# JubSteven/POEM-v2

Hardware: AMD Instinct MI355X
Metric: samples/sec (multi-view frames) POEM-medium 8-view (higher is better)
Workload: dtype f32

## Files before the change

### poem-v2_amd/csrc/decoder.cpp

```cpp
#include "engine.h"

int build_anchor_tables(poem_handle_t h, Plan& p, hipStream_t s, bool at_create) {
  const poem_config_t& c = h->cfg;
  const int C = c.embed, Q = c.nquery;
  const bool ov = !at_create && h->overlap && h->bps_stream && h->knn_stream;
  hipStream_t sk = ov ? h->knn_stream : s;
  if (ov) {
    HIPCHK(hipEventRecord(h->ev_fork0, s));
    HIPCHK(hipStreamWaitEvent(sk, h->ev_fork0, 0));
  }
  const int bb0 = h->block_base(0);
  HIPCHK(poem_launch_canon_xyz(h->tmpl, p.canon_xyz, Q * 3, c.radius, sk));
  for (int k = 0; k < 2; ++k) {
    const int vb = bb0 + (k == 0 ? B_VS : B_VC);
    HIPCHK(poem_launch_vector_attention_tables(p.canon_xyz, h->anchor, h->anchor_idx, h->R(vb + 4), h->R(vb + 5),
                                               h->P(vb + 6), h->R(vb + 7), h->fused[0].w[5 + k], p.tab_g[k], p.tab_p[k],
                                               Q, C, sk));
  }
  if (ov) HIPCHK(hipEventRecord(h->ev_tab, sk));
  h->tables_pending = ov;
  return POEM_OK;
}

namespace {

struct DecoderRun {
  poem_handle_t h;
  Plan& p;
  const poem_config_t& c;
  const float *pt_xyz, *pt_feats;
  float *pose_aa, *betas;
  const int B, C, S, Q, BS, BQ;
  const int SP, BSP;
  const float* pt_xyz_rows;
  const bool ov;
  hipStream_t s, sb, sk;
  const bool tables;
  const bool chain;
  const float* feats;
  const float* hidden;
  int ldh = 0, hidden_mod = 0, q_batch = 0;
  const float* q0 = nullptr;
  const int *idx_s = nullptr, *idx_c = nullptr;
  const float* anchor = nullptr;
  int shared = 0;
  bool knn_issued[9] = {};
  bool wmerge = false;
  int wmask = 0;
  bool side_rest_pending = false;
  bool bps_waited[9] = {}, knn_waited[9] = {};
  bool anchor_from_y3 = false;

  DecoderRun(poem_handle_t h_, Plan& p_, const float* feats_in, const float* pt_xyz_, const float* pt_feats_, int B_, float* pose,
             float* bet, hipStream_t s_, bool template_queries)
      : h(h_), p(p_), c(h_->cfg), pt_xyz(pt_xyz_), pt_feats(pt_feats_), pose_aa(pose), betas(bet), B(B_), C(c.embed), S(c.nsample),
        Q(c.nquery), BS(B_ * c.nsample), BQ(B_ * c.nquery), SP(padded_samples(c)), BSP(B_ * padded_samples(c)), pt_xyz_rows(pt_xyz_), ov(h_->overlap && h_->bps_stream && h_->knn_stream), s(s_),
        sb(ov ? h_->bps_stream : s_), sk(ov ? h_->knn_stream : s_),
        tables(template_queries && h_->anchor_tables && h_->precision == POEM_PRECISION_FP32),
        chain(h_->chains && h_->precision == POEM_PRECISION_FP32 && poem_chain_supported(c.embed) != 0), feats(feats_in),
        hidden(nullptr) {}

  int gemm(const float* X, int ldx, int wi, int bi, const float* res, int ldr, float* Y, int ldy, int M, int N, int K, int act) {
    HIPCHK(poem_launch_gemm(X, ldx, h->P(wi), bi >= 0 ? h->R(bi) : nullptr, res, ldr, Y, ldy, M, N, K, act, s));
    return POEM_OK;
  }
  bool prof_begin() {
    const bool on = h->prof_on && (size_t)(2 * h->prof_used + 1) < h->prof_ev.size();
    if (on && hipEventRecord(h->prof_ev[2 * h->prof_used], s) != hipSuccess) return false;
    return on;
  }
  int prof_end(bool on, int kind) {
    if (on) { HIPCHK(hipEventRecord(h->prof_ev[2 * h->prof_used + 1], s)); h->prof_kind[h->prof_used++] = (char)kind; }
    return POEM_OK;
  }
  ChainArgs chain_args(int kind) const {
    ChainArgs a{};
    a.kind = kind; a.M = BQ; a.tile_p = h->chain_tile; a.eps = c.ln_eps;
    a.native_delta = h->native16 ? (long long)(h->native16 - h->packed_base) : 0;
    return a;
  }

  int fork() {
    if (!ov) return POEM_OK;
    HIPCHK(hipEventRecord(h->ev_fork, s));
    HIPCHK(hipStreamWaitEvent(sb, h->ev_fork, 0));
    HIPCHK(hipStreamWaitEvent(sk, h->ev_fork, 0));
    return POEM_OK;
  }
  int join() {
    if (!ov) return POEM_OK;
    HIPCHK(hipEventRecord(h->ev_join_bps, sb));
    HIPCHK(hipEventRecord(h->ev_join_knn, sk));
    HIPCHK(hipStreamWaitEvent(s, h->ev_join_bps, 0));
    HIPCHK(hipStreamWaitEvent(s, h->ev_join_knn, 0));
    return POEM_OK;
  }

  int basis_point_side(int i) {
    const auto& f = h->fused[i];
    const size_t seg = (size_t)BSP * C;
    float* outs[6] = {p.y1[i], p.y1[i] + seg, p.y1[i] + 2 * seg, p.y1[i] + 3 * seg, p.y1[i] + 4 * seg, p.y1[i] + 5 * seg};
    const int modes[6] = {1, 2, 1, 2, 0, 0};
    h->kv_presplit[i] = poem_gemm_split_applies(f.w[0], BSP, C, C) != 0;
    const bool anchored = tables && i == 0;
    if (!anchored && h->f1_split && C % 128 == 0) {
      HIPCHK(poem_launch_gemm_segs(pt_feats, C, f.w[0], f.b[0], BSP, C, POEM_ACT_NONE, C, 4, outs, modes, sb));
      HIPCHK(poem_launch_gemm_segs(pt_feats, C, (const float*)f.w[0] + (size_t)4 * C * C, f.b[0] + 4 * C, BSP, C, POEM_ACT_NONE, C, 2, outs + 4,
                                   modes + 4, sb));
    } else {
      HIPCHK(poem_launch_gemm_segs(pt_feats, C, f.w[0], f.b[0], BSP, C, POEM_ACT_NONE, C, anchored ? 4 : 6, outs, modes, sb));
    }
    if (ov) HIPCHK(hipEventRecord(h->ev_bps[i], sb));
    if (anchored && !side_rest_pending) return basis_point_anchor_rows(f);
    return POEM_OK;
  }
  int basis_point_anchor_rows(const poem_handle_s::Fused& f) {
    {
      HIPCHK(poem_launch_gather_anchor_rows(pt_feats, C, h->anchor_idx, SP, p.anch_x[1], B, C, p.ident, sb));
      HIPCHK(poem_launch_gemm(p.anch_x[1], C, (const float*)f.w[0] + (size_t)4 * C * C, f.b[0] + 4 * C, nullptr, 0,
                              p.anch_kv[1], 2 * C, B * 32, 2 * C, C, POEM_ACT_NONE, sb));
      if (ov) HIPCHK(hipEventRecord(h->ev_xyz[0], sb));
    }
    return POEM_OK;
  }

  bool merge_in_attention() const { return h->xattn_merge >= 0 ? h->xattn_merge != 0 : B <= 2; }

  int defer_at() const {
    return (ov && chain) ? h->bps_defer : 0;
  }
  int deferred_basis_point_side(int i, int at) {
    if (defer_at() != at || i + 1 >= c.nblocks) return POEM_OK;
    HIPCHK(hipEventRecord(h->ev_def[i], s));
    HIPCHK(hipStreamWaitEvent(sb, h->ev_def[i], 0));
    return basis_point_side(i + 1);
  }

  int neighbour_searches(int i, bool recorded = false) {
    if (knn_issued[i]) return POEM_OK;
    if (ov) {
      if (!recorded) HIPCHK(hipEventRecord(h->ev_xyz[i], s));
      HIPCHK(hipStreamWaitEvent(sk, h->ev_xyz[i], 0));
    }
    if (p.idx_ld == 32) {
      HIPCHK(poem_launch_knn(p.xyz[i], pt_xyz, p.idx_cross[i], B, Q, S, h->knn_fma, sk));
      HIPCHK(poem_launch_knn(p.xyz[i], p.xyz[i], p.idx_self[i], B, Q, Q, h->knn_fma, sk));
    } else {
      HIPCHK(poem_launch_knn_k(p.xyz[i], pt_xyz, p.idx_cross[i], B, Q, S, c.knn, p.idx_ld, h->knn_fma, sk));
      HIPCHK(poem_launch_knn_k(p.xyz[i], p.xyz[i], p.idx_self[i], B, Q, Q, h->knn_query ? h->knn_query : c.knn, p.idx_ld, h->knn_fma, sk));
    }
    if (ov) HIPCHK(hipEventRecord(h->ev_knn[i], sk));
    knn_issued[i] = true;
    return POEM_OK;
  }

  int query_projection(int i) {
    hidden = p.qeqp;
    ldh = 2 * C; hidden_mod = 0; q_batch = Q;
    q0 = p.qeqp + C;
    if (tables && i == 0) {
      const float* qe0 = p.qeqp0;
      if (h->tables_cached && h->c_qeqp0 && h->precision == POEM_PRECISION_FP32)
        qe0 = h->c_qeqp0;
      else
        HIPCHK(poem_launch_gemm_split(h->R(T_QEMB), C, h->fused[i].w[1], h->fused[i].b[1], nullptr, 0, p.qeqp0, 2 * C, Q, 2 * C, C,
                                      POEM_ACT_NONE, 2 * C, POEM_ACT_NONE, s));
      if (chain) {
        hidden = qe0; hidden_mod = Q; q0 = qe0 + C; q_batch = 0;
      } else {
        HIPCHK(poem_launch_broadcast(qe0, p.qeqp, (long)Q * 2 * C, B, s));
      }
    } else if (!(chain && i > 0)) {
      HIPCHK(poem_launch_gemm_split(feats, C, h->fused[i].w[1], h->fused[i].b[1], nullptr, 0, p.qeqp, 2 * C, BQ, 2 * C, C,
                                    POEM_ACT_NONE, 2 * C, POEM_ACT_NONE, s));
    }
    return POEM_OK;
  }

  int anchor_rows_f3(int i) {
    HIPCHK(poem_launch_gather_anchor_rows(hidden, C, h->anchor_idx, Q, p.anch_x[0], B, C, nullptr, s));
    HIPCHK(poem_launch_gemm(p.anch_x[0], C, (const float*)h->fused[i].w[2] + (size_t)C * C, h->fused[i].b[2] + C, nullptr, 0,
                            p.anch_kv[0], 2 * C, B * 32, 2 * C, C, POEM_ACT_NONE, s));
    return POEM_OK;
  }

  int cross_attentions(int i) {
    const int bb = h->block_base(i);
    if (chain) {
      const int a1 = bb + B_A1, a2 = bb + B_A2;
      if (ov && !bps_waited[i]) HIPCHK(hipStreamWaitEvent(s, h->ev_bps[i], 0));
      if (ov && (wmask & 4) && h->knn_early && i > 0 && knn_issued[i] && !knn_waited[i]) {
        HIPCHK(hipStreamWaitEvent(s, h->ev_knn[i], 0));
        knn_waited[i] = true;
      }
      const void *part_o = nullptr, *part_ml = nullptr;
      int pchunks = 0;
      float pkc2 = 0.f;
      poem_cross_attention_partials(B, Q, S, C, c.heads, p.attn_scratch, &part_o, &part_ml, &pchunks, &pkc2);
      const bool merged = merge_in_attention() && poem_cross_attention_merges(S, C, c.heads) != 0;
      const bool comb = !merged && h->chain_combine && poem_chain_combines(C, c.heads, pchunks) != 0;
      auto attention = [&](const float* q, int ldq, int qb, const float* kimg, const float* vimg) -> hipError_t {
        if (merged) return poem_launch_cross_attention_merged(q, ldq, qb, kimg, vimg, p.ctx, B, Q, S, C, c.heads, s);
        return poem_launch_cross_attention_imgq(q, ldq, qb, kimg, vimg, comb ? nullptr : p.ctx, B, Q, S, C, c.heads, p.attn_scratch, s);
      };
      auto from_partials = [&](ChainArgs& a) {
        if (!comb) return;
        a.x = nullptr; a.part_o = (const float4*)part_o; a.part_ml = (const float2*)part_ml;
        a.pc_heads = c.heads; a.pc_chunks = pchunks; a.pc_nq = Q; a.pc_kc2 = pkc2;
      };
      HIPCHK(attention(q0, 2 * C, q_batch, p.y1[i], p.y1[i] + (size_t)BSP * C));
      if (side_rest_pending) {
        side_rest_pending = false;
        if (tables && i == 0)
          if (const int rc = basis_point_anchor_rows(h->fused[0]); rc != POEM_OK) return rc;
        for (int k = 1; k < c.nblocks; ++k)
          if (const int rc = basis_point_side(k); rc != POEM_OK) return rc;
      }
      if (const int rc = deferred_basis_point_side(i, 1); rc != POEM_OK) return rc;
      ChainArgs ca = chain_args(0);
      ca.x = p.ctx; ca.ldx = C;
      from_partials(ca);
      ca.w1 = (const float4*)h->P(a1 + 6); ca.b1 = h->R(a1 + 7); ca.res = hidden; ca.ldres = ldh; ca.res_mod = hidden_mod;
      ca.ln_g = h->R(a1 + 8); ca.ln_b = h->R(a1 + 9); ca.y1 = p.h_attn; ca.ldy1 = C;
      ca.w2 = (const float4*)h->P(a2 + 0); ca.b2 = h->R(a2 + 1); ca.n2 = 1; ca.y2 = p.qp; ca.ldy2 = C;
      HIPCHK(poem_launch_chain(&ca, C, s));
      HIPCHK(attention(p.qp, C, Q, p.y1[i] + (size_t)2 * BSP * C, p.y1[i] + (size_t)3 * BSP * C));
      if (const int rc = deferred_basis_point_side(i, 2); rc != POEM_OK) return rc;
      ChainArgs cb = chain_args(0);
      cb.x = p.ctx; cb.ldx = C;
      from_partials(cb);
      cb.w1 = (const float4*)h->P(a2 + 6); cb.b1 = h->R(a2 + 7); cb.res = p.h_attn; cb.ldres = C; cb.res_mod = 0;
      cb.ln_g = h->R(a2 + 8); cb.ln_b = h->R(a2 + 9); cb.y1 = p.h_cross[i]; cb.ldy1 = C;
      anchor_from_y3 = tables && i == 0 && (h->small_batch & 2) && (long)BQ <= 16L * poem_device_cu_count();
      cb.w2 = (const float4*)h->fused[i].w[2]; cb.b2 = h->fused[i].b[2]; cb.n2 = (tables && i == 0 && !anchor_from_y3) ? 1 : 3; cb.y2 = p.y3; cb.ldy2 = 3 * C;
      HIPCHK(poem_launch_chain(&cb, C, s));
// ... 16 lines not shown
      }
      if (ov && a == 0) HIPCHK(hipStreamWaitEvent(s, h->ev_bps[i], 0));
      if (h->precision == POEM_PRECISION_SPLIT_F16X3_ALL) poem_cross_attention_split(h->kv_presplit[i] ? 2 : 1);
      if (h->precision == POEM_PRECISION_FP32 && merge_in_attention() && poem_cross_attention_merges(S, C, c.heads))
        HIPCHK(poem_launch_cross_attention_merged(qptr, ldq, Q, p.y1[i] + (size_t)(2 * a) * BSP * C, p.y1[i] + (size_t)(2 * a + 1) * BSP * C,
                                                  p.ctx, B, Q, S, C, c.heads, s));
      else
        HIPCHK(poem_launch_cross_attention_img(qptr, ldq, p.y1[i] + (size_t)(2 * a) * BSP * C, p.y1[i] + (size_t)(2 * a + 1) * BSP * C,
                                               p.ctx, B, Q, S, C, c.heads, p.attn_scratch, s));
      const int rc = gemm(p.ctx, C, ab + 6, ab + 7, hidden, ldh, p.att, C, BQ, C, C, POEM_ACT_NONE);
      if (rc != POEM_OK) return rc;
      HIPCHK(poem_launch_layernorm(p.att, h->R(ab + 8), h->R(ab + 9), hout, BQ, C, c.ln_eps, s));
      hidden = hout;
      ldh = C;
    }
    if (tables && i == 0) {
      HIPCHK(poem_launch_gemm(hidden, C, h->fused[i].w[2], h->fused[i].b[2], nullptr, 0, p.y3, 3 * C, BQ, C, C, POEM_ACT_NONE, s));
      return anchor_rows_f3(i);
    }
    HIPCHK(poem_launch_gemm_split(hidden, C, h->fused[i].w[2], h->fused[i].b[2], nullptr, 0, p.y3, 3 * C, BQ, 3 * C, C, POEM_ACT_NONE,
                                  3 * C, POEM_ACT_NONE, s));
    return POEM_OK;
  }

  int vector_self(int i) {
    const int vsb = h->block_base(i) + B_VS;
    const float* xyz = p.xyz[i];
    if (ov && i > 0 && !knn_waited[i]) HIPCHK(hipStreamWaitEvent(s, h->ev_knn[i], 0));
    const bool prof = prof_begin();
    const int kq = shared ? 32 : (h->knn_query ? h->knn_query : c.knn);
    if (h->precision != POEM_PRECISION_FP32) {
      if (kq != 32) return POEM_E_UNSUPPORTED;
      const auto& sw = h->split[2 * i];
      HIPCHK(poem_launch_vector_attention_split(xyz, xyz, anchor, idx_s, shared, p.y3, p.y3 + C, p.y3 + 2 * C, Q, h->R(vsb + 4),
                                                h->R(vsb + 5), sw.w[0], h->R(vsb + 7), sw.w[1], sw.w[2], sw.scales, p.rs, B, Q, C,
                                                3 * C, 3 * C, 3 * C, s));
    } else if (tables && i == 0) {
      if (ov && h->tables_pending) HIPCHK(hipStreamWaitEvent(s, h->ev_tab, 0));
      if (anchor_from_y3)
        HIPCHK(poem_launch_vector_attention_anchored(h->anchor_idx, p.y3, p.y3 + C, p.y3 + 2 * C, Q, h->P(vsb + 10), p.tab_g[0], p.tab_p[0],
                                                     p.rs, B, Q, C, 3 * C, 3 * C, 3 * C, s));
      else {
      if (ov) HIPCHK(hipStreamWaitEvent(s, h->ev_xyz[0], 0));
      HIPCHK(poem_launch_vector_attention_anchored(p.ident, p.y3, p.anch_kv[0], p.anch_kv[0] + C, 32, h->P(vsb + 10), p.tab_g[0],
                                                   p.tab_p[0], p.rs, B, Q, C, 3 * C, 2 * C, 2 * C, s));
      }
    } else if (!shared && p.idx_ld != 32) {
      HIPCHK(poem_launch_vector_attention_k(xyz, xyz, idx_s, kq, p.idx_ld, p.y3, p.y3 + C, p.y3 + 2 * C, Q, h->R(vsb + 4), h->R(vsb + 5),
                                            h->P(vsb + 6), h->R(vsb + 7), h->fused[i].w[5], h->R(vsb + 9), h->P(vsb + 10), h->R(vsb + 11),
                                            p.rs, B, Q, C, 3 * C, 3 * C, 3 * C, 1, s));
    } else {
      poem_vecattn_one_query_blocks(h->va_p1);
      poem_vecattn_valid_neighbours(kq);
      const hipError_t ve = poem_launch_vector_attention(xyz, xyz, anchor, idx_s, shared, p.y3, p.y3 + C, p.y3 + 2 * C, Q, h->R(vsb + 4),
                                                         h->R(vsb + 5), h->P(vsb + 6), h->R(vsb + 7), h->fused[i].w[5], h->R(vsb + 9),
                                                         h->P(vsb + 10), h->R(vsb + 11), p.rs, B, Q, C, 3 * C, 3 * C, 3 * C, 1, s);
      poem_vecattn_valid_neighbours(32);
      poem_vecattn_one_query_blocks(0);
      HIPCHK(ve);
    }
    if (const int rc = prof_end(prof, tables && i == 0 ? 1 : 0); rc != POEM_OK) return rc;
    if (chain) {
      ChainArgs cc = chain_args(1);
      cc.x = p.rs; cc.ldx = C;
      cc.w1 = (const float4*)h->P(vsb + 2); cc.b1 = h->R(vsb + 3); cc.res = hidden; cc.ldres = C; cc.res_mod = 0;
      cc.y1 = p.f_self[i]; cc.ldy1 = C;
      cc.w2 = (const float4*)h->fused[i].w[4]; cc.b2 = h->fused[i].b[4]; cc.n2 = 1; cc.y2 = p.qc; cc.ldy2 = C;
      HIPCHK(poem_launch_chain(&cc, C, s));
      return POEM_OK;
    }
    if (const int rc = gemm(p.rs, C, vsb + 2, vsb + 3, hidden, C, p.f_self[i], C, BQ, C, C, POEM_ACT_NONE); rc != POEM_OK) return rc;
    HIPCHK(poem_launch_gemm(p.f_self[i], C, h->fused[i].w[4], h->fused[i].b[4], nullptr, 0, p.qc, C, BQ, C, C, POEM_ACT_NONE, s));
    return POEM_OK;
  }

  int vector_cross(int i) {
    const int vcb = h->block_base(i) + B_VC;
    const float* xyz = p.xyz[i];
    if (ov && (wmask & 2) && i == 0 && defer_at() == 0)
      for (int k = 1; k < c.nblocks; ++k) {
        HIPCHK(hipStreamWaitEvent(s, h->ev_bps[k], 0));
        bps_waited[k] = true;
      }
    const bool prof = prof_begin();
    const int kc = shared ? 32 : c.knn;
    if (h->precision != POEM_PRECISION_FP32) {
      if (kc != 32) return POEM_E_UNSUPPORTED;
      const auto& sw = h->split[2 * i + 1];
      HIPCHK(poem_launch_vector_attention_split(xyz, pt_xyz_rows, anchor, idx_c, shared, p.qc, p.y1[i] + 4 * (size_t)BSP * C,
                                                p.y1[i] + 5 * (size_t)BSP * C, SP, h->R(vcb + 4), h->R(vcb + 5), sw.w[0],
                                                h->R(vcb + 7), sw.w[1], sw.w[2], sw.scales, p.rc, B, Q, C, C, C, C, s));
    } else if (tables && i == 0) {
      if (ov) HIPCHK(hipStreamWaitEvent(s, h->ev_xyz[0], 0));
      HIPCHK(poem_launch_vector_attention_anchored(p.ident, p.qc, p.anch_kv[1], p.anch_kv[1] + C, 32, h->P(vcb + 10), p.tab_g[1],
                                                   p.tab_p[1], p.rc, B, Q, C, C, 2 * C, 2 * C, s));
    } else if (!shared && p.idx_ld != 32) {
      HIPCHK(poem_launch_vector_attention_k(xyz, pt_xyz_rows, idx_c, kc, p.idx_ld, p.qc, p.y1[i] + 4 * (size_t)BSP * C, p.y1[i] + 5 * (size_t)BSP * C,
                                            SP, h->R(vcb + 4), h->R(vcb + 5), h->P(vcb + 6), h->R(vcb + 7), h->fused[i].w[6], h->R(vcb + 9),
                                            h->P(vcb + 10), h->R(vcb + 11), p.rc, B, Q, C, C, C, C, 1, s));
    } else {
      poem_vecattn_one_query_blocks(h->va_p1);
      poem_vecattn_valid_neighbours(kc);
      const hipError_t ve = poem_launch_vector_attention(xyz, pt_xyz_rows, anchor, idx_c, shared, p.qc, p.y1[i] + 4 * (size_t)BSP * C,
                                                         p.y1[i] + 5 * (size_t)BSP * C, SP, h->R(vcb + 4), h->R(vcb + 5), h->P(vcb + 6),
                                                         h->R(vcb + 7), h->fused[i].w[6], h->R(vcb + 9), h->P(vcb + 10), h->R(vcb + 11), p.rc, B,
                                                         Q, C, C, C, C, 1, s);
      poem_vecattn_valid_neighbours(32);
      poem_vecattn_one_query_blocks(0);
      HIPCHK(ve);
    }
    return prof_end(prof, tables && i == 0 ? 1 : 0);
  }

  int parametric_tail(int i) {
    const int bb = h->block_base(i);
    HIPCHK(poem_launch_q3_flatten(feats, h->R(bb + B_FLAT_W), h->R(bb + B_FLAT_B), p.q3t, B, Q, C, s));
    HIPCHK(poem_launch_narrow_linear(p.q3t, C, h->R(bb + B_MANO_W), h->R(bb + B_MANO_B), nullptr, p.par, B, C, 106, s));
    HIPCHK(poem_launch_rot6d_to_aa(p.par, pose_aa, betas, B, s));
    if (h->mano_table) HIPCHK(poem_launch_mano_lbs(pose_aa, betas, h->mano_table, p.mano_verts, p.mano_joints, B, h->mano_center, s));
    return POEM_OK;
  }

  int tail(int i, bool* done) {
    const int bb = h->block_base(i), vcb = bb + B_VC;
    const float* xyz = p.xyz[i];
    const bool last = i == c.nblocks - 1;
    const bool feats_dead = last && !c.parametric && !h->taps;
    *done = feats_dead;
    if (chain) {
      ChainArgs cd = chain_args(2);
      cd.x = p.rc; cd.ldx = C;
      cd.w1 = (const float4*)h->P(vcb + 2); cd.b1 = h->R(vcb + 3); cd.res = p.f_self[i]; cd.ldres = C; cd.res_mod = 0;
      cd.y1 = p.f_cross[i]; cd.ldy1 = C;
      cd.wf4 = (const float4*)h->fused[i].w[3]; cd.bf4 = h->fused[i].b[3];
      cd.wreg2 = h->R(bb + B_REG2_W); cd.breg2 = h->R(bb + B_REG2_B); cd.xyz_in = xyz; cd.xyz_out = p.xyz[i + 1];
      HIPCHK(poem_launch_chain(&cd, C, s));
      if (feats_dead) return POEM_OK;
      const bool early = ov && h->knn_early && !last;
      const bool d2_first = early && h->d2_first != 0;
      if (early && d2_first) HIPCHK(hipEventRecord(h->ev_xyz[i + 1], s));
      if (early && !d2_first)
        if (const int rc = neighbour_searches(i + 1); rc != POEM_OK) return rc;
      ChainArgs ce = chain_args(3);
      ce.x = p.f_cross[i]; ce.ldx = C;
      ce.wf4 = (const float4*)h->fused[i].w[3]; ce.bf4 = h->fused[i].b[3];
      ce.wout = (const float4*)h->P(bb + B_OUT_W); ce.bout = h->R(bb + B_OUT_B);
      ce.ln2_g = h->R(bb + B_LN_W); ce.ln2_b = h->R(bb + B_LN_B); ce.y3 = p.feats[i]; ce.ldy3 = C;
      if (!last) {
        ce.w2 = (const float4*)h->fused[i + 1].w[1]; ce.b2 = h->fused[i + 1].b[1]; ce.n2 = 2; ce.y2 = p.qeqp; ce.ldy2 = 2 * C;
      }
      HIPCHK(poem_launch_chain(&ce, C, s));
      if (early && d2_first)
        if (const int rc = neighbour_searches(i + 1, true); rc != POEM_OK) return rc;
      feats = p.feats[i];
      return c.parametric && last ? parametric_tail(i) : POEM_OK;
    }
    if (const int rc = gemm(p.rc, C, vcb + 2, vcb + 3, p.f_self[i], C, p.f_cross[i], C, BQ, C, C, POEM_ACT_NONE); rc != POEM_OK) return rc;
    if (feats_dead) {
      HIPCHK(poem_launch_gemm(p.f_cross[i], C, h->fused[i].w[3], h->fused[i].b[3], nullptr, 0, p.y4, 5 * C, BQ, C, C, POEM_ACT_RELU, s));
      HIPCHK(poem_launch_narrow_linear(p.y4, 5 * C, h->R(bb + B_REG2_W), h->R(bb + B_REG2_B), xyz, p.xyz[i + 1], BQ, C, 3, s));
      return POEM_OK;
    }
    HIPCHK(poem_launch_gemm_split(p.f_cross[i], C, h->fused[i].w[3], h->fused[i].b[3], nullptr, 0, p.y4, 5 * C, BQ, 5 * C, C,
                                  POEM_ACT_RELU, C, POEM_ACT_GELU, s));
    HIPCHK(poem_launch_narrow_linear(p.y4, 5 * C, h->R(bb + B_REG2_W), h->R(bb + B_REG2_B), xyz, p.xyz[i + 1], BQ, C, 3, s));
    if (const int rc = gemm(p.y4 + C, 5 * C, bb + B_OUT_W, bb + B_OUT_B, p.f_cross[i], C, p.ffo, C, BQ, C, 4 * C, POEM_ACT_NONE); rc != POEM_OK)
      return rc;
    HIPCHK(poem_launch_layernorm(p.ffo, h->R(bb + B_LN_W), h->R(bb + B_LN_B), p.feats[i], BQ, C, c.ln_eps, s));
    feats = p.feats[i];
    return c.parametric && last ? parametric_tail(i) : POEM_OK;
  }

  int run() {
    if (SP != S) {
      if (h->precision != POEM_PRECISION_FP32) return POEM_E_UNSUPPORTED;
      HIPCHK(poem_launch_pad_rows(pt_feats, p.feat_pad, B, S, SP, C, s));
      HIPCHK(poem_launch_pad_rows(pt_xyz, p.xyz_pad, B, S, SP, 3, s));
      pt_feats = p.feat_pad;
      pt_xyz_rows = p.xyz_pad;
    }
    int rc = fork();
    if (rc != POEM_OK) return rc;
    wmask = (ov && chain) ? (h->wait_merge >= 0 ? h->wait_merge : 3) : 0;
    wmerge = wmask != 0;
    side_rest_pending = (wmask & 1) && defer_at() == 0;
    if (ov)
      for (int i = 0; i < ((defer_at() || side_rest_pending) ? 1 : c.nblocks); ++i)
        if ((rc = basis_point_side(i)) != POEM_OK) return rc;
    for (int i = 0; i < c.nblocks; ++i) {
      idx_s = idx_c = h->anchor_idx;
      anchor = h->anchor;
      shared = 1;
      if (i > 0) {
        if ((rc = neighbour_searches(i)) != POEM_OK) return rc;
        idx_s = p.idx_self[i]; idx_c = p.idx_cross[i]; anchor = nullptr; shared = 0;
      }
      if (!ov && (rc = basis_point_side(i)) != POEM_OK) return rc;
      bool done = false;
      if ((rc = query_projection(i)) != POEM_OK || (rc = cross_attentions(i)) != POEM_OK || (rc = vector_self(i)) != POEM_OK ||
          (rc = vector_cross(i)) != POEM_OK || (rc = tail(i, &done)) != POEM_OK)
        return rc;
      if (done) break;
    }
    return join();
  }
};

}

int run_decoder(poem_handle_t h, Plan& p, const float* feats_in, const float* pt_xyz, const float* pt_feats, int B, float* pose_aa,
                float* betas, hipStream_t s, bool template_queries) {
  DecoderRun run(h, p, feats_in, pt_xyz, pt_feats, B, pose_aa, betas, s, template_queries);
  return run.run();
}
```

### poem-v2_amd/csrc/engine.h

```cpp
#pragma once
#include "../../include/poem_hip.h"
#include "launchers.h"

#include <hip/hip_runtime.h>

#include <algorithm>
#include <cstdio>
#include <cstdlib>
#include <cstring>
#include <map>
#include <string>
#include <vector>

extern thread_local int g_last_hip_error;

#define HIPCHK(expr)                                 \
  do {                                               \
    (void)hipGetLastError();                         \
    hipError_t e_ = (expr);                          \
    if (e_ != hipSuccess) {                          \
      g_last_hip_error = (int)e_;                    \
      return POEM_E_LAUNCH;                          \
    }                                                \
  } while (0)
// ... 15 lines not shown
enum {
  T_INPROJ_W = 0, T_INPROJ_B, T_ADAPT_W, T_ADAPT_B, T_M00_W, T_M00_B, T_M02_W, T_M02_B, T_M10_W, T_M10_B, T_M12_W,
  T_M12_B, T_QEMB, T_HEAD_COUNT
};
enum {
  B_EMB_W = 0, B_EMB_B,
  B_A1 = 2,
  B_A2 = 12,
  B_VS = 22,
  B_VC = 37,
  B_REG0_W = 52, B_REG0_B, B_REG2_W, B_REG2_B, B_INT_W, B_INT_B, B_OUT_W, B_OUT_B, B_LN_W, B_LN_B,
  B_COUNT = 62,
  B_FLAT_W = 62, B_FLAT_B, B_MANO_W, B_MANO_B, B_COUNT_PARAM = 66
};

static inline int petr_slot(const poem_config_t& c) { return T_HEAD_COUNT + c.nblocks * (c.parametric ? B_COUNT_PARAM : B_COUNT); }
static inline size_t pe_views(int max_views) { return (size_t)max_views * (max_views + 1) / 2; }
std::vector<TensorSpec> tensor_table(const poem_config_t& c);
int check_config(const poem_config_t* c);

struct poem_handle_s {
  poem_config_t cfg;
  std::vector<TensorSpec> specs;
  std::vector<const float*> raw;
  std::vector<const void*> packed;
  const float* bps = nullptr;
  const float* anchor = nullptr;
  const int32_t* anchor_idx = nullptr;
  const float* tmpl = nullptr;
  float* pe_table = nullptr;
  struct Fused { const void* w[7]; const float* b[7]; };
  std::vector<Fused> fused;
  struct SplitW { const void* w[3]; const float* scales; };
  std::vector<SplitW> split;
  void* split_mem = nullptr;
  int precision = 0;
  bool kv_presplit[8] = {};
  const char* packed_base = nullptr;
  size_t packed_size = 0;
  char* native16 = nullptr;
  char* gemm_split = nullptr;
  float* gemm_scales = nullptr;
  bool taps = false;
  struct Tap { const void* p; int64_t elems; };
  std::map<std::string, Tap> tapmap;
  std::vector<hipEvent_t> prof_ev;
  int prof_used = 0;
  std::vector<char> prof_kind;
  bool prof_on = false;
  hipStream_t bps_stream = nullptr, knn_stream = nullptr;
  hipEvent_t ev_fork = nullptr, ev_join_bps = nullptr, ev_join_knn = nullptr, ev_tab = nullptr, ev_fork0 = nullptr;
  bool anchor_tables = true;
  bool chains = true;
  bool fused_sampling = true;
  bool tables_first = true;
  bool chain_combine = true;
  int xattn_merge = -1;
  bool knn_early = true;
  bool graphs = true;
  bool graph_broken = false;
  hipStream_t cap_stream = nullptr;
  int stream_device = 0;
  struct GraphEntry { std::vector<int64_t> key; hipGraphExec_t exec; uint64_t stamp; uint64_t shape; hipStream_t last_stream = nullptr; bool launched = false; };
  std::vector<GraphEntry> graph_cache;
  std::vector<std::vector<int64_t>> graph_seen;
  bool graph_eager = false;
  uint64_t graph_clock = 0;
  static constexpr size_t GRAPH_CAP = 12;
  int64_t graph_captures = 0, graph_instantiations = 0, graph_replays = 0, plain_forwards = 0, layout_uploads = 0;
  int small_batch = 3;
  int group_xcd = 1;
  int group_min_views = 0;
  const float* mano_table = nullptr;
  int mano_center = 9;
  int knn_query = 0;
  int knn_fma = 0;
  int chain_tile = 0;
  bool tables_cached = true;
  bool tables_pending = false;
  float* tab_mem = nullptr;
  float *c_canon_xyz = nullptr, *c_tab_g[2] = {}, *c_tab_p[2] = {};
  float* c_qeqp0 = nullptr;
  hipEvent_t ev_bps[8] = {}, ev_xyz[8] = {}, ev_knn[8] = {}, ev_def[8] = {};
  int bps_defer = 0;
  bool f1_split = true;
  int va_p1 = -1;
  int d2_first = 1;
  int wait_merge = -1;
  bool overlap = true;
  static constexpr int IDX_CAP = 32768;
  int32_t* idx_dev = nullptr;
  std::vector<int32_t> idx_host;
  int block_base(int b) const { return T_HEAD_COUNT + b * (cfg.parametric ? B_COUNT_PARAM : B_COUNT); }
  const float* R(int idx) const { return raw[idx]; }
  const void* P(int idx) const { return packed[idx]; }
};

struct Arena {
  char* base;
  size_t off = 0;
  explicit Arena(void* b) : base((char*)b) {}
  template <typename T>
  T* take(size_t n) {
    off = align_up(off, 256);
    T* p = base ? (T*)(base + off) : nullptr;
    off += n * sizeof(T);
    return p;
  }
};

struct Plan {
  int32_t *offs, *view_sample, *pe_index, *idx_self[8], *idx_cross[8];
  float *x, *uv, *g, *h1, *h2, *mm, *mh, *y, *bps_feat, *centre, *pt_xyz, *xyz[9];
  float *xt, *ptab, *q1;
  float *petr_f, *petr_h, *petr_tab;
  float *feats0, *qp, *ctx, *att, *h_attn, *y3, *rs, *qc, *rc, *y4, *ffo;
  float *y1[8];
  float *qeqp;
  float *h_cross[8], *f_self[8], *f_cross[8], *feats[8];
  float *q3t, *par, *attn_scratch, *g_pose, *g_betas;
  float *mano_verts, *mano_joints;
  float *canon_xyz, *tab_g[2], *tab_p[2];
  float *anch_x[2], *anch_kv[2], *qeqp0;
  int32_t* ident;
  float *feat_pad, *xyz_pad;
  int idx_ld;
  size_t bytes;
};

inline int padded_samples(const poem_config_t& c) { return (c.nsample + 31) / 32 * 32; }

inline int neighbour_ld(const poem_config_t& c, int knn_query) { return (c.knn > 32 || knn_query > 32) ? 64 : 32; }

Plan make_plan(const poem_config_t& c, int B, int BN, void* base, int idx_ld);
void register_taps(poem_handle_t h, const Plan& p, int B, int BN, bool sampling);

int poem_process_switches();
void poem_park_graph_exec(hipGraphExec_t e, uint64_t shape, int device, hipStream_t last_stream, bool launched);
hipGraphExec_t poem_reuse_graph_exec(hipGraph_t graph, uint64_t shape, int device);

int build_anchor_tables(poem_handle_t h, Plan& p, hipStream_t s, bool at_create = false);
int run_decoder(poem_handle_t h, Plan& p, const float* feats_in, const float* pt_xyz, const float* pt_feats, int B, float* pose_aa,
                float* betas, hipStream_t s, bool template_queries = false);
```

### poem-v2_amd/csrc/forward.cpp

```cpp
#include "engine.h"

namespace {

struct SplitContext {
  bool set = false;
  explicit SplitContext(poem_handle_t h) {
    if (h->precision != POEM_PRECISION_SPLIT_F16X3_ALL) return;
    set = true;
    poem_gemm_split_context(h->packed_base, h->packed_size, h->gemm_split, h->gemm_scales);
    poem_cross_attention_split(1);
    const int dh = h->cfg.embed / h->cfg.heads;
    poem_gemm_split_images(dh == 32 || dh == 64);
  }
  ~SplitContext() {
    if (!set) return;
    poem_gemm_split_context(nullptr, 0, nullptr, nullptr);
    poem_cross_attention_split(0);
    poem_gemm_split_images(0);
  }
};

struct HeadRun {
  poem_handle_t h;
  const poem_config_t& c;
// ... 76 lines not shown
      const int ps = petr_slot(c), K0 = 3 * c.depth_num;
      HIPCHK(poem_launch_frustum_features(cam_intr, cam_extr, p.petr_f, BN, c.feat_h, c.feat_w, c.depth_num, c.lid != 0, c.depth_start,
                                          c.depth_end, c.position_range, img_w, img_h, s));
      HIPCHK(poem_launch_conv1x1_ex(p.petr_f, h->P(ps), h->R(ps + 1), nullptr, nullptr, p.petr_h, nullptr, BN, K0, 2 * C, HW, 1, s));
      HIPCHK(poem_launch_conv1x1_ex(p.petr_h, h->P(ps + 2), h->R(ps + 3), h->pe_table, p.pe_index, p.petr_tab, nullptr, BN, 2 * C, C, HW, 0, s));
      table = p.petr_tab;
      table_index = nullptr;
    }
    HIPCHK(poem_launch_conv1x1(mlvl_feat, h->P(T_INPROJ_W), h->R(T_INPROJ_B), table, table_index,
                               (fused_fe && !h->taps) ? nullptr : p.x, fused_fe ? p.xt : nullptr, BN, c.in_channels, C, HW, s));
    if (fused_fe && (h->small_batch & 1)) {
      HIPCHK(poem_launch_input_tables(h->bps, reference_joints, h->tmpl, p.view_sample, cam_intr, cam_extr, p.ptab, p.ptab + (size_t)plan_views * S * 4, p.centre, p.pt_xyz,
                                      p.xyz[0], BN, B, S, Q, c.feat_h, c.feat_w, img_w, img_h, c.radius, s));
      return POEM_OK;
    }
    HIPCHK(poem_launch_prep_xyz(reference_joints, h->bps, h->tmpl, p.centre, p.pt_xyz, p.xyz[0], B, S, Q, c.radius, s));
    if (fused_fe) {
      float* inv = p.uv + (size_t)BN * S * 2;
      HIPCHK(poem_launch_invert_extr(cam_extr, inv, BN, s));
      HIPCHK(poem_launch_project_table(h->bps, p.centre, p.view_sample, cam_intr, inv, p.ptab, p.ptab + (size_t)plan_views * S * 4, nullptr, BN, C, c.feat_h, c.feat_w, S,
                                       img_w, img_h, s));
    } else {
      HIPCHK(poem_launch_project_uv(h->bps, p.centre, p.view_sample, cam_intr, cam_extr, p.uv + (size_t)BN * S * 2, p.uv, BN, c.feat_h,
                                    c.feat_w, S, img_w, img_h, s));
    }
    return POEM_OK;
  }

  int sampling(hipStream_t st) {
    if (fused_fe) {
      SampleMergeArgs sm{};
      sm.xt = p.xt; sm.tab = (const float4*)p.ptab; sm.tabo = (const uint2*)(p.ptab + (size_t)plan_views * S * 4);
      sm.view_sample = p.view_sample; sm.offs = p.offs;
      sm.w0 = (const float4*)h->P(T_M00_W); sm.b0 = h->R(T_M00_B); sm.w1 = (const float4*)h->P(T_M02_W); sm.b1 = h->R(T_M02_B);
      sm.h2 = p.h2; sm.q1 = p.q1; sm.S = S; sm.hw = HW; sm.h2_tiled = 1;
      sm.views = plan_views; sm.B = B; sm.views_dev = p.offs + B;
      const bool group_ok = h->group_min_views >= 0 && (S / C) % 8 == 0;
      sm.group_min_views = group_ok ? (h->group_min_views > 0 ? h->group_min_views : 2 * poem_device_cu_count() / ((C / (C == 512 ? 32 : 64)) * (S / C / 8)))
                                    : 0x7fffffff;
      if (h->tables_first && h->tables_pending) HIPCHK(hipStreamWaitEvent(st, h->ev_tab, 0));
      MergeTailArgs mt{};
      mt.h2 = p.h2; mt.q1 = p.q1; mt.offs = p.offs;
      mt.w0 = (const float4*)h->P(T_M10_W); mt.b0 = h->R(T_M10_B); mt.w1 = (const float4*)h->P(T_M12_W); mt.b1 = h->R(T_M12_B);
      mt.out = p.bps_feat; mt.B = B; mt.S = S; mt.h2_tiled = 1;
      mt.group_min_views = sm.group_min_views; mt.views_dev = sm.views_dev; mt.views = sm.views;
      sm.xcd_order = h->group_xcd;
      if (group_ok && plan_views >= sm.group_min_views) {
        SampleGroupArgs sg{};
        sg.sm = sm; sg.w2 = mt.w0; sg.b2 = mt.b0; sg.w3 = mt.w1; sg.b3 = mt.b1; sg.out = p.bps_feat;
        HIPCHK(poem_launch_sample_group(&sg, C, st));
      }
      HIPCHK(poem_launch_sample_merge(&sm, C, st));
      HIPCHK(poem_launch_merge_tail(&mt, C, st));
      return POEM_OK;
    }
    auto gemm = [&](const float* X, int ldx, int wi, int bi, float* Y, int ldy, int M, int N, int K, int act) -> int {
      HIPCHK(poem_launch_gemm(X, ldx, h->P(wi), h->R(bi), nullptr, 0, Y, ldy, M, N, K, act, st));
      return POEM_OK;
    };
    HIPCHK(poem_launch_grid_sample(p.x, p.uv, p.g, BN, C, c.feat_h, c.feat_w, S, st));
    int rc = gemm(p.g, C, T_M00_W, T_M00_B, p.h1, C, BN * S, C, C, POEM_ACT_RELU);
    if (rc == POEM_OK) rc = gemm(p.h1, C, T_M02_W, T_M02_B, p.h2, C / 2, BN * S, C / 2, C, POEM_ACT_NONE);
    if (rc != POEM_OK) return rc;
    HIPCHK(poem_launch_merge_reduce(p.h2, p.offs, p.mm, B, S, C / 2, st));
    rc = gemm(p.mm, C / 2, T_M10_W, T_M10_B, p.mh, C / 2, BS, C / 2, C / 2, POEM_ACT_RELU);
    if (rc == POEM_OK) rc = gemm(p.mh, C / 2, T_M12_W, T_M12_B, p.y, C, BS, C, C / 2, POEM_ACT_NONE);
    if (rc != POEM_OK) return rc;
    HIPCHK(poem_launch_merge_finalize(p.g, p.y, p.offs, p.bps_feat, B, S, C, st));
    return POEM_OK;
  }

  int body(hipStream_t st, float* pose_dst, float* betas_dst) {
    if (const int rc = sampling(st); rc != POEM_OK) return rc;
    if (prof_fe) HIPCHK(hipEventRecord(h->prof_ev[2 * prof_slot + 1], st));
    if (!(h->anchor_tables && h->precision == POEM_PRECISION_FP32 && (h->small_batch & 1)))
      HIPCHK(poem_launch_broadcast(h->R(T_QEMB), p.feats0, (long)Q * C, B, st));
    return run_decoder(h, p, p.feats0, p.pt_xyz, p.bps_feat, B, pose_dst, betas_dst, st, true);
  }

  int replay(void* workspace, float* pose_aa, float* betas) {
    if (!h->graphs || h->graph_broken || h->prof_on || h->tables_pending || !h->cap_stream) return 0;
    const std::vector<int64_t> key = {B, plan_views, fused_fe ? -1 : BN, (int64_t)(uintptr_t)workspace, h->precision, h->anchor_tables, h->chains,
                                      h->fused_sampling, h->tables_first, h->chain_combine, h->knn_early, h->overlap, h->chain_tile,
                                      h->tables_cached, h->knn_fma, h->knn_query, h->taps, c.parametric, h->xattn_merge, h->small_batch, h->bps_defer, poem_process_switches(), h->f1_split, h->va_p1, h->group_min_views, h->group_xcd, h->d2_first, h->wait_merge,
                                      (int64_t)(uintptr_t)h->mano_table, h->mano_center};
    poem_handle_s::GraphEntry* hit = nullptr;
    for (auto& g : h->graph_cache)
      if (g.key == key) { hit = &g; break; }
    if (!hit) {
      if (!h->graph_eager) {
        bool seen = false;
        for (auto& k : h->graph_seen) seen = seen || k == key;
        if (!seen) {
          if (h->graph_seen.size() >= 64) h->graph_seen.erase(h->graph_seen.begin());
          h->graph_seen.push_back(key);
          return 0;
        }
      }
      hipGraph_t graph = nullptr;
      hipGraphExec_t exec = nullptr;
      POEM_TRACE("capture begin h=%p B=%d cached=%zu", (void*)h, B, h->graph_cache.size());
      bool ok = hipStreamBeginCapture(h->cap_stream, hipStreamCaptureModeRelaxed) == hipSuccess;
      if (ok) {
        const int rc = body(h->cap_stream, p.g_pose, p.g_betas);
        POEM_TRACE("capture body rc=%d", rc);
        const hipError_t e = hipStreamEndCapture(h->cap_stream, &graph);
        POEM_TRACE("capture end e=%d graph=%p", (int)e, (void*)graph);
        ok = rc == POEM_OK && e == hipSuccess && graph != nullptr;
      }
      ++h->graph_captures;
      if (ok) {
        exec = poem_reuse_graph_exec(graph, graph_shape_of(c, key), h->stream_device);
        if (!exec) {
          ok = hipGraphInstantiate(&exec, graph, nullptr, nullptr, 0) == hipSuccess;
          ++h->graph_instantiations;
        }
      }
      POEM_TRACE("instantiate ok=%d exec=%p", (int)ok, (void*)exec);
      if (graph) (void)hipGraphDestroy(graph);
      POEM_TRACE("graph destroyed");
      if (!ok) {
        (void)hipGetLastError();
        h->graph_broken = true;
        return 0;
      }
      if (h->graph_cache.size() >= poem_handle_s::GRAPH_CAP) {
        size_t lru = 0;
        for (size_t i = 1; i < h->graph_cache.size(); ++i)
          if (h->graph_cache[i].stamp < h->graph_cache[lru].stamp) lru = i;
        poem_park_graph_exec(h->graph_cache[lru].exec, h->graph_cache[lru].shape, h->stream_device, h->graph_cache[lru].last_stream,
                             h->graph_cache[lru].launched);
        h->graph_cache.erase(h->graph_cache.begin() + lru);
      }
      h->graph_cache.push_back({key, exec, 0, graph_shape_of(c, key), nullptr, false});
      hit = &h->graph_cache.back();
    }
    hit->stamp = ++h->graph_clock;
    POEM_TRACE("graph launch exec=%p", (void*)hit->exec);
    HIPCHK(hipGraphLaunch(hit->exec, s));
    hit->last_stream = s; hit->launched = true;
    ++h->graph_replays;
    POEM_TRACE("graph launched");
    if (c.parametric) {
      HIPCHK(hipMemcpyAsync(pose_aa, p.g_pose, (size_t)B * 48 * sizeof(float), hipMemcpyDeviceToDevice, s));
      HIPCHK(hipMemcpyAsync(betas, p.g_betas, (size_t)B * 10 * sizeof(float), hipMemcpyDeviceToDevice, s));
    }
    return 1;
  }

  static uint64_t graph_shape_of(const poem_config_t& c, const std::vector<int64_t>& key) {
    uint64_t v = 1469598103934665603ull;
    auto mix = [&](uint64_t x) { v = (v ^ x) * 1099511628211ull; };
    mix((uint64_t)c.embed); mix((uint64_t)c.nblocks); mix((uint64_t)c.heads); mix((uint64_t)c.nsample); mix((uint64_t)c.nquery);
    mix((uint64_t)c.in_channels); mix((uint64_t)c.feat_h * 65536u + (uint64_t)c.feat_w); mix((uint64_t)c.max_views);
    for (size_t i = 0; i < key.size(); ++i)
      if (i != 3) mix((uint64_t)key[i]);
    return v ? v : 1;
  }
};

}

extern "C" {

int poem_head_forward(poem_handle_t h, const float* mlvl_feat, const float* cam_intr, const float* cam_extr,
                      const int32_t* view_offsets_host, int batch, const float* reference_joints, int img_w, int img_h,
                      float* out_xyz, float* pose_aa, float* betas, void* workspace, size_t workspace_bytes,
// ... 71 lines not shown
```

### poem-v2_amd/csrc/gemm.hip

```cpp
#include "common.h"
#include <algorithm>
#include <cstdlib>

typedef _Float16 h8 __attribute__((ext_vector_type(8)));
#ifndef POEM_GS_WAVES
#define POEM_GS_WAVES 12
#endif
#define POEM_GEMM_SX 16.0f
__global__ __launch_bounds__(256) void pack_split_tiles_kernel(const float* __restrict__ W, int N, int K,
                                                              h8* __restrict__ img, float* __restrict__ scales,
                                                              int scale_stride) {
  __shared__ float red[256];
  const int nt = blockIdx.x, KC = K / 16;
  float m = 0.f;
  for (int i = threadIdx.x; i < 32 * K; i += 256) {
    const int row = 32 * nt + i / K;
    if (row < N) m = fmaxf(m, fabsf(W[(size_t)row * K + i % K]));
  }
  red[threadIdx.x] = m;
  __syncthreads();
  for (int o = 128; o > 0; o >>= 1) {
    if ((int)threadIdx.x < o) red[threadIdx.x] = fmaxf(red[threadIdx.x], red[threadIdx.x + o]);
    __syncthreads();
  }
// ... 160 lines not shown
      float4* yp = reinterpret_cast<float4*>(Y) + (size_t)(mt0 + i) * KCO * 64 + lane;
      const float4* rp = reinterpret_cast<const float4*>(R) + (size_t)(mt0 + i) * KCO * 64 + lane;
#pragma unroll
      for (int n = 0; n < NT; ++n) {
#pragma unroll
        for (int g = 0; g < 4; ++g) {
          const int c0 = (cg * NT + n) * 32 + 8 * g + 4 * h;
          const int kco = (cg * NT + n) * 4 + g;
          float4 v = make_float4(acc[i][n][4 * g], acc[i][n][4 * g + 1], acc[i][n][4 * g + 2], acc[i][n][4 * g + 3]);
          if (bias) {
            const float4 bb = *reinterpret_cast<const float4*>(bias + c0);
            v.x += bb.x; v.y += bb.y; v.z += bb.z; v.w += bb.w;
          }
          if (act == 1) { v.x = relu_nan(v.x); v.y = relu_nan(v.y); v.z = relu_nan(v.z); v.w = relu_nan(v.w); }
          if (act == 2) { v.x = gelu_erf(v.x); v.y = gelu_erf(v.y); v.z = gelu_erf(v.z); v.w = gelu_erf(v.w); }
          if (R) {
            const float4 rr = rp[(size_t)kco * 64];
            v.x += rr.x; v.y += rr.y; v.z += rr.z; v.w += rr.w;
          }
          yp[(size_t)kco * 64] = v;
        }
      }
    }
  } else {
#pragma unroll
    for (int n = 0; n < NT; ++n) {
      const int col = (cg * NT + n) * 32 + r;
      if (col >= N) continue;
      const float bv = bias ? bias[col] : 0.f;
#pragma unroll
      for (int i = 0; i < MT; ++i) {
#pragma unroll
        for (int e = 0; e < 16; ++e) {
          const int row = (mt0 + i) * 32 + mfma_row(e, h);
          if (row < M) {
            float v = acc[i][n][e] + bv;
            if (act == 1) v = relu_nan(v);
            if (act == 2) v = gelu_erf(v);
            if (R) v += R[(size_t)row * ldr + col];
            Y[(size_t)row * ldy + col] = v;
          }
        }
      }
    }
  }
}

template <int MT, int NT>
static hipError_t launch_gemm2_t(const float* X, int ldx, const void* Wp, const float* bias, const float* R, int ldr,
                                 float* Y, int ldy, int M, int N, int K, int act, int in_pa, int out_pa, hipStream_t s) {
  const int ntiles = (N + 31) / 32, mtiles = (M + 31) / 32;
  const int rgroups = (mtiles + MT - 1) / MT;
  dim3 grid((unsigned)((rgroups + 3) / 4), (unsigned)(ntiles / NT)), block(256);
#define POEM_G2(IP, OP)                                                                                              \
  hipLaunchKernelGGL((gemm2_kernel<MT, NT, IP, OP>), grid, block, 0, s, X, ldx, (const float4*)Wp, bias, R, ldr, Y, \
                     ldy, M, N, K, act)
  if (in_pa && out_pa) POEM_G2(true, true);
  else if (in_pa) POEM_G2(true, false);
  else if (out_pa) POEM_G2(false, true);
  else POEM_G2(false, false);
#undef POEM_G2
  return hipGetLastError();
}

extern "C" hipError_t poem_launch_gemm2(const float* X, int ldx, const void* Wp, const float* bias, const float* R,
                                        int ldr, float* Y, int ldy, int M, int N, int K, int act, int in_pa, int out_pa,
                                        hipStream_t s) {
  const int ntiles = (N + 31) / 32, mtiles = (M + 31) / 32;
  const bool big = (long)((mtiles + 1) / 2) * (ntiles / 4) >= 768;
  if (ntiles % 4 == 0) {
    if (big) return launch_gemm2_t<2, 4>(X, ldx, Wp, bias, R, ldr, Y, ldy, M, N, K, act, in_pa, out_pa, s);
    return launch_gemm2_t<1, 2>(X, ldx, Wp, bias, R, ldr, Y, ldy, M, N, K, act, in_pa, out_pa, s);
  }
  if (ntiles % 2 == 0) return launch_gemm2_t<1, 2>(X, ldx, Wp, bias, R, ldr, Y, ldy, M, N, K, act, in_pa, out_pa, s);
  return launch_gemm2_t<1, 1>(X, ldx, Wp, bias, R, ldr, Y, ldy, M, N, K, act, in_pa, out_pa, s);
}

struct PanelSegs {
  float* ptr[6];
  int mode[6];
  int seg_cols;
  int split_images;
  int xcd_map;
};

template <int MT, int NT, int SKC, int OMODE>
__device__ __forceinline__ void kslab_body(const float* __restrict__ X, int ldx, const float4* __restrict__ Wp,
                                           const float* __restrict__ bias, const float* __restrict__ R, int ldr,
                                           float* __restrict__ Y, int ldy, int M, int K, int pact, int cb, int rb, int ycol0) {
  constexpr int FRAGS = NT * SKC;
  constexpr int PER = FRAGS / 8;
  static_assert(FRAGS % 8 == 0, "a slab is dealt to the eight waves");
  extern __shared__ __attribute__((aligned(16))) float4 ws[];
  const int tid = threadIdx.x, lane = tid & 63, wv = tid >> 6, r = lane & 31, h = lane >> 5;
  const int KC = K >> 3, nslab = KC / SKC;
  const int mt0 = (rb * 8 + wv) * MT;
  const float4* wsrc = Wp + (size_t)(cb * NT) * KC * 64 + lane;
  const __amdgpu_buffer_rsrc_t xrs = frag_rsrc(X, 0xffffffffu);
  unsigned xo[MT];
#pragma unroll
  for (int i = 0; i < MT; ++i) xo[i] = (unsigned)min((mt0 + i) * 32 + r, M - 1) * (unsigned)(ldx * 4) + 16u * h;
  f32x16 acc[MT][NT];
#pragma unroll
  for (int i = 0; i < MT; ++i)
#pragma unroll
    for (int n = 0; n < NT; ++n) acc[i][n] = zero16();

  float4 stage[PER];
#define KS_FETCH(SL)                                                                                     \
  _Pragma("unroll") for (int j = 0; j < PER; ++j) {                                                      \
    const int f_ = wv * PER + j;                                                                         \
    stage[j] = wsrc[((size_t)(f_ / SKC) * KC + (size_t)(SL) * SKC + f_ % SKC) * 64];                      \
  }
#define KS_COMMIT(BUF)                                                                                   \
  _Pragma("unroll") for (int j = 0; j < PER; ++j) ws[((BUF) * FRAGS + wv * PER + j) * 64 + lane] = stage[j];
  KS_FETCH(0)
  KS_COMMIT(0)
  __syncthreads();
  float4 a0[MT], a1[MT], a2[MT], a3[MT];
#define KS_LOADA(A, KCI) { const int kq_ = min((KCI), KC - 1); _Pragma("unroll") for (int i = 0; i < MT; ++i) A[i] = frag_load(xrs, (int)xo[i], kq_ * 32); }
#define KS_MMA(A, WB, KL)                                                                                \
  {                                                                                                      \
    float4 b_[NT];                                                                                       \
    _Pragma("unroll") for (int n = 0; n < NT; ++n) b_[n] = (WB)[(n * SKC + (KL)) * 64 + lane];            \
    _Pragma("unroll") for (int t = 0; t < 4; ++t)                                                        \
      _Pragma("unroll") for (int n = 0; n < NT; ++n)                                                     \
        _Pragma("unroll") for (int i = 0; i < MT; ++i)                                                   \
          acc[i][n] = OMODE == 1 ? mfma32((&b_[n].x)[t], (&A[i].x)[t], acc[i][n]) : mfma32((&A[i].x)[t], (&b_[n].x)[t], acc[i][n]); \
  }
  KS_LOADA(a0, 0) KS_LOADA(a1, 1) KS_LOADA(a2, 2)
  static_assert(SKC % 4 == 0, "the ring is unrolled by four");
  for (int sl = 0; sl < nslab; ++sl) {
    const float4* wb = ws + (sl & 1) * FRAGS * 64;
    KS_FETCH(min(sl + 1, nslab - 1))
    __builtin_amdgcn_sched_barrier(0);
    const int kc0 = sl * SKC;
    for (int kl = 0; kl < SKC; kl += 4) {
      KS_LOADA(a3, kc0 + kl + 3)
      __builtin_amdgcn_sched_barrier(0);
      KS_MMA(a0, wb, kl)
      __builtin_amdgcn_sched_barrier(0);
      KS_LOADA(a0, kc0 + kl + 4)
      __builtin_amdgcn_sched_barrier(0);
      KS_MMA(a1, wb, kl + 1)
      __builtin_amdgcn_sched_barrier(0);
      KS_LOADA(a1, kc0 + kl + 5)
      __builtin_amdgcn_sched_barrier(0);
      KS_MMA(a2, wb, kl + 2)
      __builtin_amdgcn_sched_barrier(0);
      KS_LOADA(a2, kc0 + kl + 6)
      __builtin_amdgcn_sched_barrier(0);
      KS_MMA(a3, wb, kl + 3)
      __builtin_amdgcn_sched_barrier(0);
    }
    if (sl + 1 < nslab) { KS_COMMIT((sl + 1) & 1) }
    __syncthreads();
  }
#undef KS_FETCH
#undef KS_COMMIT
#undef KS_LOADA
#undef KS_MMA
  const int col0 = cb * NT * 32;
  if (OMODE == 1) {
#pragma unroll
    for (int i = 0; i < MT; ++i) {
      if ((mt0 + i) * 32 >= M) break;
// ... 36 lines not shown
    const int col = col0 + n * 32 + r, ycol = ycol0 + n * 32 + r;
    const float bv = bias ? bias[col] : 0.f;
#pragma unroll
    for (int i = 0; i < MT; ++i) {
      const int row0 = (mt0 + i) * 32 + 4 * h;
      if (row0 >= M) continue;
      float v[16];
#pragma unroll
      for (int e = 0; e < 16; ++e) {
        v[e] = acc[i][n][e] + bv;
        if (pact == 1) v[e] = relu_nan(v[e]);
        if (pact == 2) v[e] = gelu_erf(v[e]);
      }
      if (row0 + 28 < M) {
        float* yl = Y + (size_t)row0 * ldy + ycol;
        if (R) {
          const float* rl = R + (size_t)row0 * ldr + col;
          float rr[16];
#pragma unroll
          for (int e = 0; e < 16; ++e) rr[e] = rl[(size_t)((e & 3) + 8 * (e >> 2)) * ldr];
#pragma unroll
          for (int e = 0; e < 16; ++e) yl[(size_t)((e & 3) + 8 * (e >> 2)) * ldy] = v[e] + rr[e];
        } else {
#pragma unroll
          for (int e = 0; e < 16; ++e) yl[(size_t)((e & 3) + 8 * (e >> 2)) * ldy] = v[e];
        }
      } else {
#pragma unroll
        for (int e = 0; e < 16; ++e) {
          const int row = row0 + (e & 3) + 8 * (e >> 2);
          if (row < M) Y[(size_t)row * ldy + ycol] = v[e] + (R ? R[(size_t)row * ldr + col] : 0.f);
        }
      }
    }
  }
}

template <int MT, int NT, int SKC>
__global__ __launch_bounds__(512, 2) void gemm_kslab_kernel(const float* __restrict__ X, int ldx, const float4* __restrict__ Wp,
                                                            const float* __restrict__ bias, const float* __restrict__ R, int ldr,
                                                            float* __restrict__ Y, int ldy, int M, int N, int K, int act,
                                                            int act_split, int act2, PanelSegs segs) {
  const int ncb = N / (32 * NT);
  const int nb = (int)gridDim.x;
  const int lb = (nb & 7) == 0 ? (int)(blockIdx.x & 7) * (nb >> 3) + (int)(blockIdx.x >> 3) : (int)blockIdx.x;
  const int cb = lb % ncb, rb = lb / ncb;
  const int col0 = cb * NT * 32;
  const int pact = (col0 >= act_split) ? act2 : act;
  if (segs.seg_cols == 0) {
    kslab_body<MT, NT, SKC, 0>(X, ldx, Wp, bias, R, ldr, Y, ldy, M, K, pact, cb, rb, col0);
    return;
  }
  const int sidx = col0 / segs.seg_cols, ycol0 = col0 - sidx * segs.seg_cols, mode = segs.mode[sidx];
  float* ys = segs.ptr[sidx];
  if (mode == 1) kslab_body<MT, NT, SKC, 1>(X, ldx, Wp, bias, nullptr, 0, ys, segs.seg_cols, M, K, pact, cb, rb, ycol0);
  else if (mode == 2) kslab_body<MT, NT, SKC, 2>(X, ldx, Wp, bias, nullptr, 0, ys, segs.seg_cols, M, K, pact, cb, rb, ycol0);
  else kslab_body<MT, NT, SKC, 0>(X, ldx, Wp, bias, nullptr, 0, ys, segs.seg_cols, M, K, pact, cb, rb, ycol0);
}

static bool kslab_applies(const float* X, int ldx, int M, int N, int K, int act_split) {
  return K >= 512 && K % 128 == 0 && N % 64 == 0 && (act_split >= N || act_split % 64 == 0) && !((uintptr_t)X & 15) && ldx % 4 == 0 &&
         (unsigned long long)M * ldx * 4ull < (1ull << 32) && M >= 512;
}

static hipError_t launch_gemm_kslab(const float* X, int ldx, const void* Wp, const float* bias, const float* R, int ldr, float* Y,
                                    int ldy, int M, int N, int K, int act, int act_split, int act2, const PanelSegs& segs, hipStream_t s) {
  constexpr int NT = 2, SKC = 16;
  const int mtiles = (M + 31) / 32, ncb = N / (32 * NT);
  const bool mt2 = (long)((mtiles + 15) / 16) * ncb >= 2 * poem_device_cus();
  const size_t lds = (size_t)2 * NT * SKC * 1024;
  if (mt2) {
    auto kern = gemm_kslab_kernel<2, NT, SKC>;
    hipLaunchKernelGGL(kern, dim3((unsigned)(((mtiles + 15) / 16) * ncb)), dim3(512), lds, s, X, ldx, (const float4*)Wp, bias, R, ldr, Y, ldy,
                       M, N, K, act, act_split, act2, segs);
  } else {
    auto kern = gemm_kslab_kernel<1, NT, SKC>;
    hipLaunchKernelGGL(kern, dim3((unsigned)(((mtiles + 7) / 8) * ncb)), dim3(512), lds, s, X, ldx, (const float4*)Wp, bias, R, ldr, Y, ldy,
                       M, N, K, act, act_split, act2, segs);
  }
  return hipGetLastError();
}


template <int NT, int MT, bool GELU, int OMODE, bool SPLIT = false>
__device__ __forceinline__ void panel_rows(const float* __restrict__ X, int ldx, const float4* __restrict__ wl,
                                           const float* __restrict__ bias, const float* __restrict__ R, int ldr,
                                           float* __restrict__ Y, int ldy, int M, int K, int pact, int col0, int ycol0,
                                           int bip, int blocks_in_panel, const float* __restrict__ tile_scales = nullptr,
                                           int scale_stride = 0, int split_images = 0, int part = 0, int nparts = 1) {
  constexpr int NWV = (SPLIT && !GELU) ? POEM_GS_WAVES : 8;
  const int KC = K >> 3;
  const int tid = threadIdx.x, lane = tid & 63, wv = tid >> 6, r = lane & 31, h = lane >> 5;
  const int mtiles = (M + 31) / 32;
  const int rgroups = (mtiles + MT - 1) / MT;
  const __amdgpu_buffer_rsrc_t xrs = frag_rsrc(X, 0xffffffffu);
  float bv[NT];
#pragma unroll
  for (int n = 0; n < NT; ++n) bv[n] = (bias && OMODE != 1) ? bias[col0 + n * 32 + r] : 0.f;
  const size_t lane_yo = (size_t)(4 * h) * ldy + r, lane_ro = (size_t)(4 * h) * ldr + r;
  const int rg_lo = (int)((long)rgroups * part / nparts), rg_hi = (int)((long)rgroups * (part + 1) / nparts);
#ifndef POEM_PANEL_LAB
#define POEM_PANEL_LAB 0
#endif
#ifdef POEM_PANEL_SKEW
  if (wv >= NWV / 2) { const long long t0_ = wall_clock64(); while (wall_clock64() - t0_ < POEM_PANEL_SKEW) __builtin_amdgcn_s_sleep(32); }
#endif
  for (int rg = rg_lo + bip * NWV + wv; rg < rg_hi; rg += blocks_in_panel * NWV) {
#if POEM_PANEL_LAB & 4
    __builtin_amdgcn_s_setprio(0);
#endif
    const int mt0 = rg * MT;
    unsigned xo[MT];
#pragma unroll
    for (int i = 0; i < MT; ++i) xo[i] = (unsigned)min((mt0 + i) * 32 + r, M - 1) * (unsigned)(ldx * 4) + 16u * h;
    f32x16 acc[MT][NT];
#pragma unroll
    for (int i = 0; i < MT; ++i)
#pragma unroll
      for (int n = 0; n < NT; ++n) acc[i][n] = zero16();
    if constexpr (SPLIT) {
      const int KC16 = K >> 4;
      const h8* wl8 = reinterpret_cast<const h8*>(wl);
      unsigned xo8[MT];
#pragma unroll
      for (int i = 0; i < MT; ++i) xo8[i] = (unsigned)min((mt0 + i) * 32 + r, M - 1) * (unsigned)(ldx * 4) + 32u * h;
      float4 ra[2][MT][2];
#define POEM_LOADA8(S, KCI) { const int kq_ = min((KCI), KC16 - 1); _Pragma("unroll") for (int i = 0; i < MT; ++i) { \
        ra[S][i][0] = frag_load(xrs, (int)xo8[i], kq_ * 64); ra[S][i][1] = frag_load(xrs, (int)xo8[i], kq_ * 64 + 16); } }
      POEM_LOADA8(0, 0)
      h8 bh_next = wl8[lane], bl_next = wl8[64 + lane];
      for (int kc = 0; kc < KC16; ++kc) {
        const int cur = kc & 1;
        if (cur == 0) { POEM_LOADA8(1, kc + 1) } else { POEM_LOADA8(0, kc + 1) }
        h8 ah[MT], al[MT];
#pragma unroll
        for (int i = 0; i < MT; ++i) {
          const float4 lo4 = cur == 0 ? ra[0][i][0] : ra[1][i][0], hi4 = cur == 0 ? ra[0][i][1] : ra[1][i][1];
          const float xv[8] = {lo4.x, lo4.y, lo4.z, lo4.w, hi4.x, hi4.y, hi4.z, hi4.w};
#pragma unroll
          for (int t = 0; t < 8; ++t) {
#if defined(POEM_GS_LAB) && POEM_GS_LAB == 1
            ah[i][t] = __builtin_bit_cast(_Float16, (unsigned short)__float_as_uint(xv[t]));
            al[i][t] = ah[i][t];
#else
            const float v = __builtin_amdgcn_fmed3f(xv[t] * POEM_GEMM_SX, -60000.f, 60000.f);
            ah[i][t] = (_Float16)v;
            al[i][t] = (_Float16)(v - (float)ah[i][t]);
#endif
          }
        }
        __builtin_amdgcn_sched_barrier(0);
#pragma unroll
        for (int n = 0; n < NT; ++n) {
          const int nn = n + 1 < NT ? n + 1 : 0, kn = n + 1 < NT ? kc : min(kc + 1, KC16 - 1);
          const h8 bh = bh_next, bl = bl_next;
          bh_next = wl8[((size_t)(nn * KC16 + kn) * 2 + 0) * 64 + lane];
          bl_next = wl8[((size_t)(nn * KC16 + kn) * 2 + 1) * 64 + lane];
          __builtin_amdgcn_sched_barrier(0);
#define POEM_MMA8(XA, WB)                                                                                      \
          _Pragma("unroll") for (int i = 0; i < MT; ++i)                                                       \
            acc[i][n] = OMODE == 1 ? __builtin_amdgcn_mfma_f32_32x32x16_f16(WB, XA[i], acc[i][n], 0, 0, 0)     \
                                   : __builtin_amdgcn_mfma_f32_32x32x16_f16(XA[i], WB, acc[i][n], 0, 0, 0);
#if defined(POEM_GS_LAB) && POEM_GS_LAB == 2
#pragma unroll
          for (int i = 0; i < MT; ++i) acc[i][n][0] += (float)al[i][0] * (float)bh[0] + (float)ah[i][1] * (float)bl[1];
#else
          POEM_MMA8(al, bh) POEM_MMA8(ah, bh) POEM_MMA8(ah, bl)
#endif
#undef POEM_MMA8
          __builtin_amdgcn_sched_barrier(0);
        }
      }
#undef POEM_LOADA8
#pragma unroll
      for (int n = 0; n < NT; ++n) {
        const float inv = 1.0f / (tile_scales[(size_t)(col0 / 32 + n) * scale_stride] * POEM_GEMM_SX);
#pragma unroll
        for (int i = 0; i < MT; ++i)
#pragma unroll
          for (int e = 0; e < 16; ++e) acc[i][n][e] *= inv;
      }
    } else {
    float4 a0[MT], a1[MT], b0[NT], b1[NT];
#define POEM_LOADA(A, KCI) { const int kq_ = min((KCI), KC - 1); _Pragma("unroll") for (int i = 0; i < MT; ++i) A[i] = frag_load(xrs, (int)xo[i], kq_ * 32); }
#define POEM_LOADB(B, KCI) { const int kq_ = min((KCI), KC - 1); _Pragma("unroll") for (int n = 0; n < NT; ++n) B[n] = wl[(n * KC + kq_) * 64 + lane]; }
#define POEM_MMA(A, B)                                                          \
  _Pragma("unroll") for (int t = 0; t < 4; ++t) {                               \
    _Pragma("unroll") for (int n = 0; n < NT; ++n) {                            \
      const float bw = (&B[n].x)[t];                                            \
      _Pragma("unroll") for (int i = 0; i < MT; ++i)                            \
        acc[i][n] = OMODE == 1 ? mfma32(bw, (&A[i].x)[t], acc[i][n]) : mfma32((&A[i].x)[t], bw, acc[i][n]); \
    }                                                                           \
  }
    POEM_LOADA(a0, 0) POEM_LOADB(b0, 0)
    int kc = 0;
    for (; kc + 1 < KC; kc += 2) {
      POEM_LOADA(a1, kc + 1) POEM_LOADB(b1, kc + 1)
// ... 41 lines not shown
              vprev = v;
            } else {
#if POEM_PANEL_LAB & 1
              asm volatile("" :: "v"(v.x), "v"(v.y), "v"(v.z), "v"(v.w));
#else
              yp[(size_t)(n * 4 + g) * 64] = v;
#endif
            }
          }
      }
      continue;
    }
#pragma unroll
    for (int i = 0; i < MT; ++i) {
      const int trow0 = (mt0 + i) * 32;
      if (trow0 >= M) break;
      float* yl = Y + (size_t)trow0 * ldy + (size_t)ycol0 + lane_yo;
      const float* rl = R ? R + (size_t)trow0 * ldr + (size_t)col0 + lane_ro : nullptr;
      const bool full = trow0 + 32 <= M;
#pragma unroll
      for (int n = 0; n < NT; ++n) {
        float v[16];
        if (GELU && pact == 2) {
#pragma unroll
          for (int e = 0; e < 16; ++e) v[e] = gelu_erf(acc[i][n][e] + bv[n]);
        } else if (pact == 1) {
#pragma unroll
          for (int e = 0; e < 16; e += 2) {
            const f32x2 t = f32x2{acc[i][n][e], acc[i][n][e + 1]} + f32x2{bv[n], bv[n]};
            v[e] = relu_nan(t[0]); v[e + 1] = relu_nan(t[1]);
          }
        } else {
#pragma unroll
          for (int e = 0; e < 16; e += 2) {
            const f32x2 t = f32x2{acc[i][n][e], acc[i][n][e + 1]} + f32x2{bv[n], bv[n]};
            v[e] = t[0]; v[e + 1] = t[1];
          }
        }
        if (OMODE == 2) {
          float4* yp = reinterpret_cast<float4*>(Y) + ((size_t)(mt0 + i) * (ldy >> 5) + (ycol0 >> 5) + n) * 256 + lane;
          if (SPLIT && split_images) {
#pragma unroll
            for (int c = 0; c < 2; ++c) {
              h8 hi, lo;
              split_pair(make_float4(v[8 * c], v[8 * c + 1], v[8 * c + 2], v[8 * c + 3]),
                         make_float4(v[8 * c + 4], v[8 * c + 5], v[8 * c + 6], v[8 * c + 7]), hi, lo);
              yp[(size_t)(2 * c) * 64] = __builtin_bit_cast(float4, hi);
              yp[(size_t)(2 * c + 1) * 64] = __builtin_bit_cast(float4, lo);
            }
          } else {
#pragma unroll
          for (int g = 0; g < 4; ++g) {
#if POEM_PANEL_LAB & 1
            asm volatile("" :: "v"(v[4 * g]), "v"(v[4 * g + 1]), "v"(v[4 * g + 2]), "v"(v[4 * g + 3]));
#else
            yp[(size_t)g * 64] = make_float4(v[4 * g], v[4 * g + 1], v[4 * g + 2], v[4 * g + 3]);
#endif
          }
          }
        } else if (full) {
          if (rl) {
            float rr[16];
#pragma unroll
            for (int e = 0; e < 16; ++e) rr[e] = rl[(size_t)((e & 3) + 8 * (e >> 2)) * ldr + n * 32];
            __builtin_amdgcn_sched_barrier(0);
#pragma unroll
            for (int e = 0; e < 16; ++e) yl[(size_t)((e & 3) + 8 * (e >> 2)) * ldy + n * 32] = v[e] + rr[e];
          } else {
#pragma unroll
            for (int e = 0; e < 16; ++e) yl[(size_t)((e & 3) + 8 * (e >> 2)) * ldy + n * 32] = v[e];
          }
        } else {
#pragma unroll
          for (int e = 0; e < 16; ++e) {
            const int ro = (e & 3) + 8 * (e >> 2);
            if (trow0 + ro + 4 * h < M) yl[(size_t)ro * ldy + n * 32] = v[e] + (rl ? rl[(size_t)ro * ldr + n * 32] : 0.f);
          }
        }
      }
    }
  }
}

template <int NT, int MT, bool GELU, bool SPLIT = false>
__global__ __launch_bounds__((SPLIT && !GELU) ? POEM_GS_WAVES * 64 : 512, 2) void gemm_panel_kernel(const float* __restrict__ X, int ldx,
                                                            const float4* __restrict__ Wp, const float* __restrict__ bias,
                                                            const float* __restrict__ R, int ldr, float* __restrict__ Y,
                                                            int ldy, int M, int N, int K, int act, int act_split, int act2,
                                                            PanelSegs segs, const float* __restrict__ tile_scales = nullptr,
                                                            int scale_stride = 0) {
  constexpr int NWV = (SPLIT && !GELU) ? POEM_GS_WAVES : 8;
  const int KC = K >> 3;
  extern __shared__ __attribute__((aligned(16))) float4 wl[];
  const int tid = threadIdx.x;
  const int panels = N / (32 * NT);
  const int xm = segs.xcd_map;
  const int lb = xm ? (int)(blockIdx.x >> 3) : (int)blockIdx.x;
  const int panel = lb % panels, bip = lb / panels;
  const int blocks_in_panel = xm ? (int)(gridDim.x >> 3) / panels : ((int)gridDim.x - panel + panels - 1) / panels;
  const int part = xm ? (int)(blockIdx.x & 7) : 0, nparts = xm ? 8 : 1;
  {
    const float4* src = Wp + (size_t)panel * NT * KC * 64;
    for (int i = tid; i < NT * KC * 64; i += NWV * 64) wl[i] = src[i];
    float* lb = reinterpret_cast<float*>(wl + NT * KC * 64);
    if (tid < NT * 32) lb[tid] = bias ? bias[panel * NT * 32 + tid] : 0.f;
  }
  __syncthreads();
  const int col0 = panel * NT * 32;
  const int pact = (col0 >= act_split) ? act2 : act;
  if (segs.seg_cols == 0) {
    panel_rows<NT, MT, GELU, 0, SPLIT>(X, ldx, wl, bias, R, ldr, Y, ldy, M, K, pact, col0, col0, bip, blocks_in_panel,
                                       tile_scales, scale_stride, 0, part, nparts);
    return;
  }
  const int sidx = col0 / segs.seg_cols;
  const int ycol0 = col0 - sidx * segs.seg_cols;
  float* ys = segs.ptr[sidx];
  const int mode = segs.mode[sidx];
  if (!GELU && mode == 1)
    panel_rows<NT, MT, false, 1, SPLIT>(X, ldx, wl, bias, nullptr, 0, ys, segs.seg_cols, M, K, pact, col0, ycol0, bip,
                                        blocks_in_panel, tile_scales, scale_stride, segs.split_images, part, nparts);
  else if (!GELU && mode == 2)
    panel_rows<NT, MT, false, 2, SPLIT>(X, ldx, wl, bias, nullptr, 0, ys, segs.seg_cols, M, K, pact, col0, ycol0, bip,
                                        blocks_in_panel, tile_scales, scale_stride, segs.split_images, part, nparts);
  else
    panel_rows<NT, MT, GELU, 0, SPLIT>(X, ldx, wl, bias, nullptr, 0, ys, segs.seg_cols, M, K, pact, col0, ycol0, bip,
                                       blocks_in_panel, tile_scales, scale_stride, 0, part, nparts);
}

static int poem_num_cus() { return poem_device_cus(); }
static std::atomic<int> g_kslab{1};
extern "C" void poem_gemm_kslab(int on) { g_kslab = on; }
static std::atomic<int> g_panel_narrow{1};
extern "C" void poem_gemm_panel_narrow(int on) { g_panel_narrow = on; }
static std::atomic<int> g_panel_xcd_map{1};
extern "C" void poem_gemm_xcd_map(int on) { g_panel_xcd_map = on; }

template <int NT, int MT, bool GELU, bool SPLIT = false>
static hipError_t launch_panel_t(const float* X, int ldx, const void* Wp, const float* bias, const float* R, int ldr,
                                 float* Y, int ldy, int M, int N, int K, int act, int act_split, int act2,
                                 const PanelSegs& segs, hipStream_t s, const float* tile_scales = nullptr,
                                 int scale_stride = 0) {
  const size_t lds = (size_t)NT * (K / 8) * 64 * 16 + (size_t)NT * 32 * sizeof(float);
  auto kern = gemm_panel_kernel<NT, MT, GELU, SPLIT>;
  static std::atomic<unsigned long long> optin{0};
  if (hipError_t e = poem_optin_lds(reinterpret_cast<const void*>(kern), 128 * 1024 + 512, optin); e != hipSuccess) return e;
  const int panels = N / (32 * NT);
  const int grid = std::max(poem_num_cus(), panels);
  PanelSegs sg = segs;
  const int mtiles = (M + 31) / 32;
  sg.xcd_map = g_panel_xcd_map && grid % 8 == 0 && (grid / 8) % panels == 0 && mtiles >= 8 * ((grid / 8) / panels) * 8 * MT;
  hipLaunchKernelGGL(kern, dim3(grid), dim3((SPLIT && !GELU) ? POEM_GS_WAVES * 64 : 512), lds, s, X, ldx, (const float4*)Wp, bias, R,
                     ldr, Y, ldy, M, N, K, act, act_split, act2, sg, tile_scales, scale_stride);
  return hipGetLastError();
}

static hipError_t launch_gemm_split_impl(const float* X, int ldx, const void* Wp, const float* bias, const float* R,
                                         int ldr, float* Y, int ldy, int M, int N, int K, int act, int act_split,
                                         int act2, const PanelSegs& segs, hipStream_t s) {
  const bool seg = segs.seg_cols > 0;
  const bool in_split_mode = g_explicit_split.img || (g_split_ctx.packed && (const char*)Wp >= g_split_ctx.packed &&
                                                      (const char*)Wp < g_split_ctx.packed + g_split_ctx.bytes);
  int NT = 0;
  const long wave_slots = 8L * poem_num_cus(), row_tiles = (M + 31) / 32;
  for (int c : {4, 2, 1})
    if (N % (32 * c) == 0 && (size_t)c * K * 128 <= 128 * 1024 && (act_split >= N || act_split % (32 * c) == 0) &&
        (!seg || segs.seg_cols % (32 * c) == 0)) {
      NT = c;
      if (row_tiles * (N / (32 * c)) >= wave_slots || !g_panel_narrow || K > 256 || in_split_mode) break;
    }
  const bool split_mode = in_split_mode;
  if (NT <= 1 && !split_mode && g_kslab && kslab_applies(X, ldx, M, N, K, act_split) && (!seg || (segs.seg_cols % 64 == 0 && M % 32 == 0)))
    return launch_gemm_kslab(X, ldx, Wp, bias, R, ldr, Y, ldy, M, N, K, act, act_split, act2, segs, s);
  if (!seg && NT == 1 && N >= 64 && K >= 512 && !(act_split < N && act2 != act)) NT = 0;
  if (NT == 0 || K % 8 || ((uintptr_t)X & 15) || ldx % 4 || (unsigned long long)M * ldx * 4ull >= (1ull << 32)) {
    if (seg || (act_split < N && act2 != act) || g_explicit_split.img) return hipErrorInvalidValue;
    return poem_launch_gemm2(X, ldx, Wp, bias, R, ldr, Y, ldy, M, N, K, act, 0, 0, s);
  }
  const int mtiles = (M + 31) / 32, panels = N / (32 * NT);
  const int wpp = std::max(1, std::max(poem_num_cus(), panels) / panels) * 8;
  auto cost = [&](int mt) { return (long)(((mtiles + mt - 1) / mt + wpp - 1) / wpp) * mt; };
  const bool mt2_default = 5 * cost(2) <= 6 * cost(1);
  const bool mt2 = mt2_default;
  const bool gelu = act == 2 || (act_split < N && act2 == 2);
  if (seg && gelu) return hipErrorInvalidValue;
  const float* tsc = nullptr;
  int tstride = 0;
  const void* Wsplit = nullptr;
  if (g_explicit_split.img) {
    Wsplit = g_explicit_split.img; tsc = g_explicit_split.scales; tstride = 1;
  } else if (g_split_ctx.packed && (const char*)Wp >= g_split_ctx.packed && (const char*)Wp < g_split_ctx.packed + g_split_ctx.bytes) {
    const size_t off = (const char*)Wp - g_split_ctx.packed;
    Wsplit = g_split_ctx.split + off; tsc = g_split_ctx.scales + off / 256; tstride = K / 2;
  }
  if (g_explicit_split.img && K % 16) return hipErrorInvalidValue;
  if (Wsplit && K % 16 == 0 && (unsigned long long)M * ldx * 4ull + 64ull < (1ull << 32)) {
#ifdef POEM_LAB
    static const int force_mt = getenv("POEM_GS_MT") ? atoi(getenv("POEM_GS_MT")) : 1;
#else
    constexpr int force_mt = 1;
#endif
    const bool mt2 = force_mt == 2;
    (void)mt2_default;
#define POEM_PANEL_S(NTV)                                                                                                \
    if (gelu)                                                                                                            \
      return mt2 ? launch_panel_t<NTV, 2, true, true>(X, ldx, Wsplit, bias, R, ldr, Y, ldy, M, N, K, act, act_split, act2, segs, s, tsc, tstride)   \
                 : launch_panel_t<NTV, 1, true, true>(X, ldx, Wsplit, bias, R, ldr, Y, ldy, M, N, K, act, act_split, act2, segs, s, tsc, tstride);  \
    return mt2 ? launch_panel_t<NTV, 2, false, true>(X, ldx, Wsplit, bias, R, ldr, Y, ldy, M, N, K, act, act_split, act2, segs, s, tsc, tstride)    \
               : launch_panel_t<NTV, 1, false, true>(X, ldx, Wsplit, bias, R, ldr, Y, ldy, M, N, K, act, act_split, act2, segs, s, tsc, tstride)
    if (NT == 4) { POEM_PANEL_S(4); }
    if (NT == 2) { POEM_PANEL_S(2); }
    POEM_PANEL_S(1);
#undef POEM_PANEL_S
  }
#define POEM_PANEL(NTV)                                                                                                  \
  if (gelu)                                                                                                              \
    return mt2 ? launch_panel_t<NTV, 2, true>(X, ldx, Wp, bias, R, ldr, Y, ldy, M, N, K, act, act_split, act2, segs, s)   \
               : launch_panel_t<NTV, 1, true>(X, ldx, Wp, bias, R, ldr, Y, ldy, M, N, K, act, act_split, act2, segs, s);  \
  return mt2 ? launch_panel_t<NTV, 2, false>(X, ldx, Wp, bias, R, ldr, Y, ldy, M, N, K, act, act_split, act2, segs, s)    \
             : launch_panel_t<NTV, 1, false>(X, ldx, Wp, bias, R, ldr, Y, ldy, M, N, K, act, act_split, act2, segs, s)
  if (NT == 4) { POEM_PANEL(4); }
  if (NT == 2) { POEM_PANEL(2); }
  POEM_PANEL(1);
#undef POEM_PANEL
}

extern "C" hipError_t poem_launch_gemm_split(const float* X, int ldx, const void* Wp, const float* bias, const float* R,
                                             int ldr, float* Y, int ldy, int M, int N, int K, int act, int act_split,
                                             int act2, hipStream_t s) {
  PanelSegs none{};
  return launch_gemm_split_impl(X, ldx, Wp, bias, R, ldr, Y, ldy, M, N, K, act, act_split, act2, none, s);
}

extern "C" hipError_t poem_launch_gemm_segs(const float* X, int ldx, const void* Wp, const float* bias, int M, int K,
                                            int act, int seg_cols, int nsegs, float* const* outs, const int* modes,
                                            hipStream_t s) {
  if (nsegs < 1 || nsegs > 6 || seg_cols % 32 || M % 32) return hipErrorInvalidValue;
  PanelSegs segs{};
  segs.seg_cols = seg_cols;
  segs.split_images = g_split_images;
  for (int i = 0; i < nsegs; ++i) { segs.ptr[i] = outs[i]; segs.mode[i] = modes[i]; }
  const int N = seg_cols * nsegs;
  return launch_gemm_split_impl(X, ldx, Wp, bias, nullptr, 0, nullptr, 0, M, N, K, act, N, act, segs, s);
}

extern "C" hipError_t poem_launch_gemm(const float* X, int ldx, const void* Wp, const float* bias, const float* R,
                                       int ldr, float* Y, int ldy, int M, int N, int K, int act, hipStream_t s) {
  return poem_launch_gemm_split(X, ldx, Wp, bias, R, ldr, Y, ldy, M, N, K, act, N, act, s);
}

__global__ __launch_bounds__(256) void layernorm_kernel(const float* __restrict__ x, const float* __restrict__ g,
                                                        const float* __restrict__ b, float* __restrict__ y, int rows,
                                                        int cols, float eps) {
  const int lane = threadIdx.x & 63;
  const int row = blockIdx.x * 4 + (threadIdx.x >> 6);
  if (row >= rows) return;
  const float* xr = x + (size_t)row * cols;
  float s = 0.f;
  for (int c = lane; c < cols; c += 64) s += xr[c];
#pragma unroll
  for (int o = 32; o > 0; o >>= 1) s += __shfl_xor(s, o, 64);
  const float mean = s / (float)cols;
  float v = 0.f;
  for (int c = lane; c < cols; c += 64) { float d = xr[c] - mean; v += d * d; }
#pragma unroll
  for (int o = 32; o > 0; o >>= 1) v += __shfl_xor(v, o, 64);
  const float rstd = 1.0f / sqrtf(v / (float)cols + eps);
  float* yr = y + (size_t)row * cols;
  for (int c = lane; c < cols; c += 64) yr[c] = (xr[c] - mean) * rstd * g[c] + b[c];
}

extern "C" hipError_t poem_launch_layernorm(const float* x, const float* g, const float* b, float* y, int rows,
                                            int cols, float eps, hipStream_t s) {
  hipLaunchKernelGGL(layernorm_kernel, dim3((rows + 3) / 4), dim3(256), 0, s, x, g, b, y, rows, cols, eps);
  return hipGetLastError();
}

__global__ __launch_bounds__(256) void narrow_linear_kernel(const float* __restrict__ x, int ldx,
                                                            const float* __restrict__ w, const float* __restrict__ b,
                                                            const float* __restrict__ base, float* __restrict__ out,
                                                            int rows, int K, int N, int npb) {
  const int lane = threadIdx.x & 63;
  const int row = blockIdx.x * 4 + (threadIdx.x >> 6);
  if (row >= rows) return;
  const float* xr = x + (size_t)row * ldx;
  for (int n = blockIdx.y * npb, ne = min(N, n + npb); n < ne; ++n) {
    float s = 0.f;
    for (int c = lane; c < K; c += 64) s = fmaf(xr[c], w[(size_t)n * K + c], s);
#pragma unroll
    for (int o = 32; o > 0; o >>= 1) s += __shfl_xor(s, o, 64);
    if (lane == 0) out[(size_t)row * N + n] = (base ? base[(size_t)row * N + n] : 0.f) + (s + (b ? b[n] : 0.f));
  }
}

extern "C" hipError_t poem_launch_narrow_linear(const float* x, int ldx, const float* w, const float* b,
                                                const float* base, float* out, int rows, int K, int N,
                                                hipStream_t s) {
  const int npb = (long)((rows + 3) / 4) * N <= 65535 && (rows + 3) / 4 < 2048 ? 1 : N;
  hipLaunchKernelGGL(narrow_linear_kernel, dim3((rows + 3) / 4, (N + npb - 1) / npb), dim3(256), 0, s, x, ldx, w, b, base, out, rows, K, N, npb);
  return hipGetLastError();
}
```

### poem-v2_amd/csrc/handle.cpp

```cpp
#include "engine.h"

#include <atomic>
thread_local int g_last_hip_error = 0;

static std::atomic<int> g_proc_switches{15};
int poem_process_switches() { return g_proc_switches.load(); }

#include <mutex>
namespace {
struct CaptureKit {
  hipStream_t cap = nullptr, bps = nullptr, knn = nullptr;
  hipEvent_t ev[5 + 32] = {};
};
std::mutex g_pool_mutex;
std::map<int, std::vector<CaptureKit>> g_kit_pool;
struct ParkedExec { hipGraphExec_t exec; uint64_t shape; int device; hipEvent_t done; };
std::vector<ParkedExec> g_parked_execs;
std::map<int, std::vector<hipEvent_t>> g_idle_done_events;
int64_t g_exec_reuses = 0, g_exec_update_failures = 0, g_exec_busy_skips = 0;

hipEvent_t done_event_locked(hipStream_t last_stream, bool launched, int device, bool* ok) {
  *ok = true;
  if (!launched) return nullptr;
  int cur = -1;
  const bool switched = hipGetDevice(&cur) == hipSuccess && cur != device && hipSetDevice(device) == hipSuccess;
  hipEvent_t ev = nullptr;
  auto& idle = g_idle_done_events[device];
  if (!idle.empty()) { ev = idle.back(); idle.pop_back(); }
  else if (hipEventCreateWithFlags(&ev, hipEventDisableTiming) != hipSuccess) { (void)hipGetLastError(); ev = nullptr; }
  if (ev && hipEventRecord(ev, last_stream) != hipSuccess) {
    (void)hipGetLastError();
    idle.push_back(ev);
    ev = nullptr;
  }
  if (!ev) {
    *ok = hipDeviceSynchronize() == hipSuccess;
    (void)hipGetLastError();
  }
  if (switched) (void)hipSetDevice(cur);
  return ev;
}

hipEvent_t** kit_event_slots(poem_handle_t h, hipEvent_t** out) {
  int n = 0;
  out[n++] = &h->ev_fork; out[n++] = &h->ev_join_bps; out[n++] = &h->ev_join_knn; out[n++] = &h->ev_tab; out[n++] = &h->ev_fork0;
  for (int i = 0; i < 8; ++i) { out[n++] = &h->ev_bps[i]; out[n++] = &h->ev_xyz[i]; out[n++] = &h->ev_knn[i]; out[n++] = &h->ev_def[i]; }
  return out;
}

bool take_kit(poem_handle_t h) {
  int dev = 0;
  if (hipGetDevice(&dev) != hipSuccess) return false;
  h->stream_device = dev;
  hipEvent_t* slots[5 + 32];
  kit_event_slots(h, slots);
  {
    std::lock_guard<std::mutex> lock(g_pool_mutex);
    auto& pool = g_kit_pool[dev];
    if (!pool.empty()) {
      const CaptureKit k = pool.back();
      pool.pop_back();
      h->cap_stream = k.cap; h->bps_stream = k.bps; h->knn_stream = k.knn;
      for (int i = 0; i < 5 + 32; ++i) *slots[i] = k.ev[i];
      return true;
    }
  }
  bool ok = hipStreamCreateWithFlags(&h->bps_stream, hipStreamNonBlocking) == hipSuccess &&
            hipStreamCreateWithFlags(&h->knn_stream, hipStreamNonBlocking) == hipSuccess &&
            hipStreamCreateWithFlags(&h->cap_stream, hipStreamNonBlocking) == hipSuccess;
  for (int i = 0; i < 5 + 32; ++i) ok = ok && hipEventCreateWithFlags(slots[i], hipEventDisableTiming) == hipSuccess;
  return ok;
}

void return_kit(poem_handle_t h) {
  hipEvent_t* slots[5 + 32];
  kit_event_slots(h, slots);
  bool whole = h->cap_stream && h->bps_stream && h->knn_stream;
  for (int i = 0; i < 5 + 32; ++i) whole = whole && *slots[i] != nullptr;
  if (!whole) {
    if (h->cap_stream) (void)hipStreamDestroy(h->cap_stream);
    if (h->bps_stream) (void)hipStreamDestroy(h->bps_stream);
    if (h->knn_stream) (void)hipStreamDestroy(h->knn_stream);
    for (int i = 0; i < 5 + 32; ++i) if (*slots[i]) (void)hipEventDestroy(*slots[i]);
  } else {
    CaptureKit k;
    k.cap = h->cap_stream; k.bps = h->bps_stream; k.knn = h->knn_stream;
    for (int i = 0; i < 5 + 32; ++i) k.ev[i] = *slots[i];
    std::lock_guard<std::mutex> lock(g_pool_mutex);
    g_kit_pool[h->stream_device].push_back(k);
  }
  h->cap_stream = h->bps_stream = h->knn_stream = nullptr;
  for (int i = 0; i < 5 + 32; ++i) *slots[i] = nullptr;
}

void park_execs(poem_handle_t h) {
  std::lock_guard<std::mutex> lock(g_pool_mutex);
  for (auto& g : h->graph_cache) {
    bool ok = true;
    hipEvent_t ev = done_event_locked(g.last_stream, g.launched, h->stream_device, &ok);
    g_parked_execs.push_back({g.exec, ok ? g.shape : 0, h->stream_device, ev});
  }
  h->graph_cache.clear();
}
}

void poem_park_graph_exec(hipGraphExec_t e, uint64_t shape, int device, hipStream_t last_stream, bool launched) {
  std::lock_guard<std::mutex> lock(g_pool_mutex);
  bool ok = true;
  hipEvent_t ev = done_event_locked(last_stream, launched, device, &ok);
  g_parked_execs.push_back({e, ok ? shape : 0, device, ev});
}

hipGraphExec_t poem_reuse_graph_exec(hipGraph_t graph, uint64_t shape, int device) {
  ParkedExec cand{nullptr, 0, 0, nullptr};
  {
    std::lock_guard<std::mutex> lock(g_pool_mutex);
    for (size_t i = g_parked_execs.size(); i-- > 0;) {
      ParkedExec& pe = g_parked_execs[i];
      if (pe.shape != shape || pe.device != device) continue;
      if (pe.done) {
        if (hipEventQuery(pe.done) != hipSuccess) { (void)hipGetLastError(); ++g_exec_busy_skips; continue; }
        g_idle_done_events[pe.device].push_back(pe.done);
        pe.done = nullptr;
      }
      cand = pe;
      g_parked_execs.erase(g_parked_execs.begin() + i);
      break;
    }
  }
  if (!cand.exec) return nullptr;
  hipGraphNode_t err_node = nullptr;
  hipGraphExecUpdateResult res = hipGraphExecUpdateSuccess;
  const hipError_t e = hipGraphExecUpdate(cand.exec, graph, &err_node, &res);
  std::lock_guard<std::mutex> lock(g_pool_mutex);
  if (e == hipSuccess && res == hipGraphExecUpdateSuccess) {
    ++g_exec_reuses;
    return cand.exec;
  }
  (void)hipGetLastError();
  POEM_TRACE("exec update refused e=%d res=%d", (int)e, (int)res);
  ++g_exec_update_failures;
  g_parked_execs.insert(g_parked_execs.begin(), {cand.exec, 0, cand.device, nullptr});
  return nullptr;
}

std::vector<TensorSpec> tensor_table(const poem_config_t& c) {
  const int C = c.embed, Q = c.nquery;
  std::vector<TensorSpec> t;
  auto lin = [&](int o, int i, bool pack, bool bias = true) {
    t.push_back({o, i, pack});
    if (bias) t.push_back({o, 1, false});
  };
  lin(C, c.in_channels, true);
  lin(C, 3 * C / 2, true);
  lin(C, C, true);
  lin(C / 2, C, true);
  lin(C / 2, C / 2, true);
  lin(C, C / 2, true);
  t.push_back({Q, C, false});
  for (int b = 0; b < c.nblocks; ++b) {
    lin(C, C, true);
    for (int a = 0; a < 2; ++a) {
      lin(C, C, true); lin(C, C, true); lin(C, C, true); lin(C, C, true);
      t.push_back({C, 1, false}); t.push_back({C, 1, false});
    }
    for (int a = 0; a < 2; ++a) {
      lin(C, C, true); lin(C, C, true);
      lin(C, 3, false);
      lin(C, C, true); lin(C, C, true); lin(C, C, true);
      lin(C, C, true, false); lin(C, C, true, false); lin(C, C, true, false);
    }
    lin(C, C, true);
    lin(3, C, false);
    lin(4 * C, C, true);
    lin(C, 4 * C, true);
// ... 245 lines not shown
  h->pe_table = (float*)cur;
  cur += align_up(pe_views(cfg->max_views) * C * hw * 4, 256);
  float* sine = (float*)cur;
  rc = poem_pe_table_ex(h->P(T_ADAPT_W), h->R(T_ADAPT_B), C, cfg->feat_h, cfg->feat_w, cfg->max_views, cfg->pe_normalize != 0, sine,
                        h->pe_table, stream);
  if (rc != POEM_OK) { poem_destroy(h); return rc; }
  {
    if (!take_kit(h)) { poem_destroy(h); return POEM_E_LAUNCH; }
  }
  {
    const size_t tf = poem_vector_attention_table_floats(cfg->nquery, C);
    const size_t cx = align_up((size_t)cfg->nquery * 3, 64);
    const size_t qf = align_up((size_t)cfg->nquery * 2 * C, 64);
    if (hipMalloc((void**)&h->tab_mem, (cx + 4 * tf + qf) * sizeof(float)) != hipSuccess) {
      g_last_hip_error = (int)hipGetLastError(); poem_destroy(h); return POEM_E_LAUNCH;
    }
    h->c_canon_xyz = h->tab_mem;
    Plan tp{};
    tp.canon_xyz = h->c_canon_xyz;
    for (int k = 0; k < 2; ++k) {
      tp.tab_g[k] = h->c_tab_g[k] = h->tab_mem + cx + (size_t)(2 * k) * tf;
      tp.tab_p[k] = h->c_tab_p[k] = h->tab_mem + cx + (size_t)(2 * k + 1) * tf;
    }
    rc = build_anchor_tables(h, tp, s, true);
    if (rc != POEM_OK) { poem_destroy(h); return rc; }
    h->c_qeqp0 = h->tab_mem + cx + 4 * tf;
    if (poem_launch_gemm_split(h->R(T_QEMB), C, h->fused[0].w[1], h->fused[0].b[1], nullptr, 0, h->c_qeqp0, 2 * C, cfg->nquery, 2 * C, C,
                               POEM_ACT_NONE, 2 * C, POEM_ACT_NONE, s) != hipSuccess) {
      g_last_hip_error = (int)hipGetLastError(); poem_destroy(h); return POEM_E_LAUNCH;
    }
  }
  *out = h;
  return POEM_OK;
}

void poem_destroy(poem_handle_t h) {
  if (!h) return;
  POEM_TRACE("destroy h=%p graphs=%zu", (void*)h, h->graph_cache.size());
  for (auto e : h->prof_ev) (void)hipEventDestroy(e);
  if (h->tab_mem) (void)hipFree(h->tab_mem);
  if (h->split_mem) (void)hipFree(h->split_mem);
  if (h->gemm_split) (void)hipFree(h->gemm_split);
  if (h->native16) (void)hipFree(h->native16);
  if (h->gemm_scales) (void)hipFree(h->gemm_scales);
  park_execs(h);
  return_kit(h);
  delete h;
}

int poem_set_overlap(poem_handle_t h, int enable) {
  if (!h) return POEM_E_ARG;
  h->overlap = enable != 0;
  return POEM_OK;
}

int poem_set_chains(poem_handle_t h, int enable) {
  if (!h) return POEM_E_ARG;
  h->chains = enable != 0;
  return POEM_OK;
}

int poem_set_option(poem_handle_t h, const char* name, int value) {
  if (!h || !name) return POEM_E_ARG;
  const std::string k(name);
  if (k == "overlap") h->overlap = value != 0;
  else if (k == "anchor_tables") h->anchor_tables = value != 0;
  else if (k == "chains") h->chains = value != 0;
  else if (k == "knn_early") h->knn_early = value != 0;
  else if (k == "fused_sampling") h->fused_sampling = value != 0;
  else if (k == "chain_combine") h->chain_combine = value != 0;
  else if (k == "xattn_merge") { if (value < -1 || value > 1) return POEM_E_ARG; h->xattn_merge = value; }
  else if (k == "tables_first") h->tables_first = value != 0;
  else if (k == "tables_cached") h->tables_cached = value != 0;
  else if (k == "knn_fma") h->knn_fma = value != 0;
  else if (k == "knn_query") {
    if (value < 0 || value > 64 || value > h->cfg.nquery) return POEM_E_ARG;
    if (h->precision != POEM_PRECISION_FP32 && value != 0 && value != 32) return POEM_E_UNSUPPORTED;
    h->knn_query = value;
  }
  else if (k == "graphs") h->graphs = value != 0;
  else if (k == "graph_eager") h->graph_eager = value != 0;
  else if (k == "gemm_xcd_map") { poem_gemm_xcd_map(value != 0); g_proc_switches.fetch_and(~1); g_proc_switches.fetch_or(value ? 1 : 0); }
  else if (k == "f1_split") h->f1_split = value != 0;
  else if (k == "xattn_half") { poem_cross_attention_half(value != 0); g_proc_switches.fetch_and(~4); g_proc_switches.fetch_or(value ? 4 : 0); }
  else if (k == "xattn_tail") { poem_cross_attention_tail_halves(value != 0); g_proc_switches.fetch_and(~8); g_proc_switches.fetch_or(value ? 8 : 0); }
  else if (k == "wait_merge") { if (value < -1 || value > 7) return POEM_E_ARG; h->wait_merge = value; }
  else if (k == "d2_first") { if (value < 0 || value > 1) return POEM_E_ARG; h->d2_first = value; }
  else if (k == "va_p1") { if (value < -1 || value > 2) return POEM_E_ARG; h->va_p1 = value; }
  else if (k == "gemm_kslab") { poem_gemm_kslab(value != 0); g_proc_switches.fetch_and(~2); g_proc_switches.fetch_or(value ? 2 : 0); }
  else if (k == "small_batch") h->small_batch = value;
  else if (k == "group_xcd") h->group_xcd = value != 0;
  else if (k == "group_min_views") { if (value < -1) return POEM_E_ARG; h->group_min_views = value; }
  else if (k == "bps_defer") { if (value < 0 || value > 3) return POEM_E_ARG; h->bps_defer = value; }
  else if (k == "chain_tile") { if (value < 0 || value > 3) return POEM_E_ARG; h->chain_tile = value; }
  else return POEM_E_ARG;
  return POEM_OK;
}

int poem_graph_stats(poem_handle_t h, int64_t* out, int n) {
  if (!h || !out || n < 9) return POEM_E_ARG;
  out[0] = (int64_t)h->graph_cache.size();
  out[1] = h->graph_captures; out[2] = h->graph_instantiations; out[3] = h->graph_replays; out[4] = h->plain_forwards;
  out[5] = h->layout_uploads;
  std::lock_guard<std::mutex> lock(g_pool_mutex);
  out[6] = (int64_t)g_parked_execs.size(); out[7] = g_exec_reuses; out[8] = g_exec_update_failures;
  if (n >= 10) out[9] = g_exec_busy_skips;
  return POEM_OK;
}

int poem_attach_mano(poem_handle_t h, const void* table, int center_idx) {
  if (!h || center_idx < -1 || center_idx > 20) return POEM_E_ARG;
  if (table && !h->cfg.parametric) return POEM_E_UNSUPPORTED;
  h->mano_table = (const float*)table;
  h->mano_center = center_idx;
  return POEM_OK;
}

int poem_set_anchor_tables(poem_handle_t h, int enable) {
  if (!h) return POEM_E_ARG;
  h->anchor_tables = enable != 0;
  return POEM_OK;
}

int poem_set_precision(poem_handle_t h, int mode) {
  if (!h || mode < POEM_PRECISION_FP32 || mode > POEM_PRECISION_SPLIT_F16X3_ALL) return POEM_E_ARG;
  if (mode != POEM_PRECISION_FP32 && (!h->split_mem || !h->gemm_split)) return POEM_E_UNSUPPORTED;
  if (mode != POEM_PRECISION_FP32 && (h->cfg.knn != 32 || (h->knn_query && h->knn_query != 32)))
    return POEM_E_UNSUPPORTED;
  if (mode != POEM_PRECISION_FP32 && h->cfg.nsample % 32)
    return POEM_E_UNSUPPORTED;
  h->precision = mode;
  return POEM_OK;
}

int poem_enable_taps(poem_handle_t h, int enable) {
  if (!h) return POEM_E_ARG;
  h->taps = enable != 0;
  return POEM_OK;
}

int64_t poem_tap(poem_handle_t h, const char* name, void* dst, int64_t dst_elems, void* stream) {
  if (!h || !name) return POEM_E_ARG;
  auto it = h->tapmap.find(name);
  if (it == h->tapmap.end()) return POEM_E_ARG;
  if (dst) {
    if (dst_elems < it->second.elems) return POEM_E_ARG;
    HIPCHK(hipMemcpyAsync(dst, it->second.p, (size_t)it->second.elems * 4, hipMemcpyDeviceToDevice, (hipStream_t)stream));
  }
  return it->second.elems;
}
int poem_profile_enable(poem_handle_t h, int max_launches) {
  if (!h || max_launches < 0) return POEM_E_ARG;
  for (auto e : h->prof_ev) (void)hipEventDestroy(e);
  h->prof_ev.clear();
  h->prof_used = 0;
  h->prof_on = max_launches > 0;
  h->prof_kind.assign((size_t)max_launches, 0);
  for (int i = 0; i < 2 * max_launches; ++i) {
    hipEvent_t e;
    HIPCHK(hipEventCreate(&e));
    h->prof_ev.push_back(e);
  }
  return POEM_OK;
}

static int profile_sum(poem_handle_t h, int kind, int* launches, float* total_ms) {
// ... 33 lines not shown
```

### poem-v2_amd/csrc/knn.hip

```cpp
#include "common.h"
#include <algorithm>

#define POEM_KNN_SURV_CAP 128
#define POEM_KNN_SURV_CAP_K 256

namespace {

typedef float knn2 __attribute__((ext_vector_type(2)));

template <bool FMA>
__device__ __forceinline__ knn2 knn_dist2(knn2 qx, knn2 qy, knn2 qz, knn2 sx, knn2 sy, knn2 sz) {
#pragma clang fp contract(off)
  const knn2 dx = qx - sx, dy = qy - sy, dz = qz - sz;
  const knn2 xx = dx * dx;
  if (FMA) return __builtin_elementwise_fma(dz, dz, __builtin_elementwise_fma(dy, dy, xx));
  const knn2 yy = dy * dy, zz = dz * dz;
  return (xx + yy) + zz;
}
template <bool FMA>
__device__ __forceinline__ float knn_dist(float qx, float qy, float qz, float sx, float sy, float sz) {
  const knn2 d = knn_dist2<FMA>(knn2{qx, qx}, knn2{qy, qy}, knn2{qz, qz}, knn2{sx, sx}, knn2{sy, sy}, knn2{sz, sz});
  return d[0];
}

// ... 104 lines not shown

}

template <int QPB, bool FMA, bool WIDE>
__device__ __forceinline__ void knn_block(const float* qxyz, const float* sxyz, int* idx, int NQ, int NS, int G, int K, int ld) {
  constexpr int CAP = WIDE ? POEM_KNN_SURV_CAP_K : POEM_KNN_SURV_CAP, LM = WIDE ? 128 : 64;
  extern __shared__ __attribute__((aligned(16))) float sp[];
  const int NSP = (NS + 127) & ~127, pairs = NSP >> 7;
  const int lane = threadIdx.x & 63, wv = threadIdx.x >> 6;
  const int b = blockIdx.x / G, g = blockIdx.x % G;
  float *px = sp, *py = sp + NSP, *pz = sp + 2 * NSP;
  float2* surv = reinterpret_cast<float2*>(sp + 3 * NSP) + wv * CAP;
  float* lmin = sp + 3 * NSP + QPB * CAP * 2 + wv * LM;
  int* counter = reinterpret_cast<int*>(sp + 3 * NSP + QPB * CAP * 2 + QPB * LM);
  {
    const float* src = sxyz + (size_t)b * NS * 3;
    for (int i = threadIdx.x; i < NS * 3; i += QPB * 64) {
      const int c = i / 3, k = i - 3 * c;
      sp[k * NSP + c] = src[i];
    }
    for (int i = NS + threadIdx.x; i < NSP; i += QPB * 64) px[i] = py[i] = pz[i] = INFINITY;
    if (threadIdx.x == 0) *counter = 0;
  }
  __syncthreads();
  const int q_lo = g * NQ / G, q_hi = (g + 1) * NQ / G;
  for (;;) {
    int qi = 0;
    if (lane == 0) qi = atomicAdd(counter, 1);
    qi = q_lo + __builtin_amdgcn_readfirstlane(qi);
    if (qi >= q_hi) break;
    const long wid = (long)b * NQ + qi;
    const float* qp = qxyz + wid * 3;
    const float qx = qp[0], qy = qp[1], qz = qp[2];
    knn_query<FMA, WIDE>(px, py, pz, surv, lmin, qx, qy, qz, pairs, NS, lane, idx + wid * ld, K);
  }
}

template <int QPB, bool FMA>
__global__ __launch_bounds__(QPB * 64) void knn_kernel(const float* __restrict__ qxyz, const float* __restrict__ sxyz,
                                                       int* __restrict__ idx, int B, int NQ, int NS, int G) {
  knn_block<QPB, FMA, false>(qxyz, sxyz, idx, NQ, NS, G, 32, 32);
}
template <int QPB, bool FMA>
__global__ __launch_bounds__(QPB * 64) void knn_kernel_k(const float* __restrict__ qxyz, const float* __restrict__ sxyz,
                                                         int* __restrict__ idx, int B, int NQ, int NS, int G, int K, int ld) {
  knn_block<QPB, FMA, true>(qxyz, sxyz, idx, NQ, NS, G, K, ld);
}

template <bool WIDE>
static hipError_t knn_launch(const float* qxyz, const float* sxyz, int* idx, int B, int NQ, int NS, int K, int ld, int fma,
                             hipStream_t s) {
  constexpr int QPB = 16, CAP = WIDE ? POEM_KNN_SURV_CAP_K : POEM_KNN_SURV_CAP, LM = WIDE ? 128 : 64;
  if (B <= 0 || NQ <= 0 || NS <= 0) return hipErrorInvalidValue;
  const int NSP = (NS + 127) & ~127;
  const size_t lds = ((size_t)3 * NSP + (size_t)QPB * CAP * 2 + QPB * LM + 4) * sizeof(float);
  if (lds > 160 * 1024) return hipErrorInvalidValue;
  auto kern = [fma] {
    if constexpr (WIDE) return fma ? knn_kernel_k<QPB, true> : knn_kernel_k<QPB, false>;
    else return fma ? knn_kernel<QPB, true> : knn_kernel<QPB, false>;
  }();
  static std::atomic<unsigned long long> optin[2];
  if (lds > 64 * 1024)
    if (hipError_t e = poem_optin_lds(reinterpret_cast<const void*>(kern), 160 * 1024, optin[fma ? 1 : 0]); e != hipSuccess) return e;
  const int cus = poem_device_cus();
  int G = (cus + B - 1) / B;
  G = std::max(1, std::min(G, (NQ + QPB - 1) / QPB));
  if ((long)G * NQ >= (1l << 31)) return hipErrorInvalidValue;
  const dim3 grid((unsigned)(B * G)), block(QPB * 64);
  if constexpr (WIDE) hipLaunchKernelGGL(kern, grid, block, lds, s, qxyz, sxyz, idx, B, NQ, NS, G, K, ld);
  else hipLaunchKernelGGL(kern, grid, block, lds, s, qxyz, sxyz, idx, B, NQ, NS, G);
  return hipGetLastError();
}

extern "C" hipError_t poem_launch_knn(const float* qxyz, const float* sxyz, int* idx, int B, int NQ, int NS, int fma,
                                      hipStream_t s) {
  return knn_launch<false>(qxyz, sxyz, idx, B, NQ, NS, 32, 32, fma, s);
}
extern "C" hipError_t poem_launch_knn_k(const float* qxyz, const float* sxyz, int* idx, int B, int NQ, int NS, int K, int ld,
                                        int fma, hipStream_t s) {
  if (K < 1 || K > 64 || K > NS || ld < K) return hipErrorInvalidValue;
  return K == 32 && ld == 32 ? knn_launch<false>(qxyz, sxyz, idx, B, NQ, NS, 32, 32, fma, s)
                             : knn_launch<true>(qxyz, sxyz, idx, B, NQ, NS, K, ld, fma, s);
}
```

### poem-v2_amd/csrc/launchers.h

```cpp
#pragma once
#include <hip/hip_runtime.h>

#include "chain.h"
#include "loss.h"
#include "merge.h"

extern "C" {
hipError_t poem_launch_pack_linear(const float* w, int N, int K, void* out, hipStream_t s);
hipError_t poem_launch_gemm(const float* X, int ldx, const void* Wp, const float* bias, const float* R, int ldr,
                            float* Y, int ldy, int M, int N, int K, int act, hipStream_t s);
hipError_t poem_launch_gemm2(const float* X, int ldx, const void* Wp, const float* bias, const float* R, int ldr,
                             float* Y, int ldy, int M, int N, int K, int act, int in_pa, int out_pa, hipStream_t s);
hipError_t poem_launch_unpack_rows(const void* pa, int N, int K, float* out, hipStream_t s);
hipError_t poem_launch_layernorm(const float* x, const float* g, const float* b, float* y, int rows, int cols,
                                 float eps, hipStream_t s);
hipError_t poem_launch_narrow_linear(const float* x, int ldx, const float* w, const float* b, const float* base,
                                     float* out, int rows, int K, int N, hipStream_t s);
hipError_t poem_launch_sine_pe(float* out, int F, int H, int W, int max_views, int normalize, hipStream_t s);
hipError_t poem_launch_frustum_features(const float* intr, const float* extr, float* out, int views, int H, int W, int D, int lid,
                                        double depth_start, double depth_end, const double* position_range, int img0, int img1,
                                        hipStream_t s);
hipError_t poem_launch_conv1x1_ex(const float* feat, const void* Wp, const float* bias, const float* table, const int* pe_index,
                                  float* x, float* xt, int views, int K, int C, int hw, int relu, hipStream_t s);
int poem_sample_merge_supported(int C, int S, int hw);
hipError_t poem_launch_project_table(const float* bps, const float* centre, const int* view_sample, const float* intr,
                                     const float* inv_extr, void* tabw, void* tabo, float* uv, int views, int C, int fh, int fw, int S,
                                     int img_w, int img_h, hipStream_t s);
hipError_t poem_launch_view_layout(const ViewLayoutArgs* a, hipStream_t s);
hipError_t poem_launch_input_tables(const float* bps, const float* ref_joints, const float* tmpl, const int* view_sample,
                                    const float* intr, const float* extr, void* tabw, void* tabo, float* centre, float* pt_xyz, float* query_xyz,
                                    int views, int B, int S, int Q, int fh, int fw, int img_w, int img_h, float radius, hipStream_t s);
hipError_t poem_launch_sample_merge(const SampleMergeArgs* a, int C, hipStream_t s);
hipError_t poem_launch_sample_group(const SampleGroupArgs* a, int C, hipStream_t s);
int poem_device_cu_count(void);
hipError_t poem_launch_merge_tail(const MergeTailArgs* a, int C, hipStream_t s);
hipError_t poem_launch_invert_extr(const float* extr, float* inv, int views, hipStream_t s);
hipError_t poem_launch_conv1x1(const float* feat, const void* Wp, const float* bias, const float* table,
                               const int* pe_index, float* x, float* xt, int views, int K, int C, int hw, hipStream_t s);
hipError_t poem_launch_project_sample(const float* x, const float* bps, const float* centre, const int* view_sample,
                                      const float* intr, const float* extr, float* inv_scratch, float* uv, float* g,
                                      int views, int C, int fh, int fw, int S, int img_w, int img_h, hipStream_t s);
hipError_t poem_launch_project_uv(const float* bps, const float* centre, const int* view_sample, const float* intr,
                                  const float* extr, float* inv_scratch, float* uv, int views, int fh, int fw, int S, int img_w,
                                  int img_h, hipStream_t s);
hipError_t poem_launch_grid_sample(const float* x, const float* uv, float* g, int views, int C, int fh, int fw, int S, hipStream_t s);
hipError_t poem_launch_grid_sample_ex(const float* x, const float* uv, float* g, int views, int C, int fh, int fw, int S, int staged,
                                      hipStream_t s);
hipError_t poem_launch_merge_reduce(const float* h2, const int* offs, float* m, int B, int S, int HALF, hipStream_t s);
hipError_t poem_launch_merge_finalize(const float* g, const float* y, const int* offs, float* out, int B, int S, int C,
                                      hipStream_t s);
hipError_t poem_launch_cross_attention(const float* q, const float* k, const float* v, float* ctx, int B, int NQ, int NK,
                                       int C, int heads, int ldkv, float* scratch, hipStream_t s);
size_t poem_cross_attention_scratch_floats(int B, int NQ, int NK, int C, int heads, int with_images);
hipError_t poem_launch_cross_attention_img(const float* q, int ldq, const void* kimg, const void* vimg, float* ctx, int B,
                                           int NQ, int NK, int C, int heads, float* scratch, hipStream_t s);
hipError_t poem_launch_gemm_segs(const float* X, int ldx, const void* Wp, const float* bias, int M, int K, int act,
                                 int seg_cols, int nsegs, float* const* outs, const int* modes, hipStream_t s);
hipError_t poem_launch_cross_attention_imgq(const float* q, int ldq, int q_batch_rows, const void* kimg, const void* vimg,
                                            float* ctx, int B, int NQ, int NK, int C, int heads, float* scratch, hipStream_t s);
int poem_chain_supported(int C);
int poem_chain_combines(int C, int heads, int chunks);
void poem_cross_attention_partials(int B, int NQ, int NK, int C, int heads, float* scratch, const void** part_o,
                                   const void** part_ml, int* chunks, float* kc2);
hipError_t poem_launch_chain(const ChainArgs* a, int C, hipStream_t s);
hipError_t poem_launch_native16(const void* packed, void* native, size_t bytes, hipStream_t s);
int poem_chain16_wants_native(int C);
hipError_t poem_launch_knn(const float* qxyz, const float* sxyz, int* idx, int B, int NQ, int NS, int fma, hipStream_t s);
hipError_t poem_launch_knn_k(const float* qxyz, const float* sxyz, int* idx, int B, int NQ, int NS, int K, int ld, int fma,
                             hipStream_t s);
hipError_t poem_launch_vector_attention(const float* query_xyz, const float* src_xyz, const float* anchor_xyz,
                                        const int* idx, int shared_idx, const float* q, const float* k, const float* v,
                                        int nsrc, const float* wd1, const float* bd1, const void* wd2, const float* bd2,
                                        const void* wg1, const float* bg1, const void* wg2, const float* bg2, float* out,
                                        int B, int Q, int C, int ldq, int ldk, int ldv, int composed, hipStream_t s);
hipError_t poem_launch_vector_attention_k(const float* query_xyz, const float* src_xyz, const int* idx, int K, int ld,
                                          const float* q, const float* k, const float* v, int nsrc, const float* wd1,
                                          const float* bd1, const void* wd2, const float* bd2, const void* wg1, const float* bg1,
                                          const void* wg2, const float* bg2, float* out, int B, int Q, int C, int ldq, int ldk,
                                          int ldv, int composed, hipStream_t s);
size_t poem_vector_attention_table_floats(int Q, int C);
hipError_t poem_launch_vector_attention_tables(const float* query_xyz, const float* anchor_xyz, const int* idx,
                                               const float* wd1, const float* bd1, const void* wd2, const float* bd2,
                                               const void* wg1d2, float* tab_g, float* tab_p, int Q, int C, hipStream_t s);
hipError_t poem_launch_vector_attention_anchored(const int* idx, const float* qg, const float* kg, const float* v, int nsrc,
                                                 const void* wg2, const float* tab_g, const float* tab_p, float* out, int B,
                                                 int Q, int C, int ldq, int ldk, int ldv, hipStream_t s);
hipError_t poem_launch_gather_anchor_rows(const float* src, int ld, const int* idx, int NS, float* dst, int B, int C,
                                          int* ident, hipStream_t s);
hipError_t poem_launch_pad_rows(const float* src, float* dst, int B, int S, int SP, int W, hipStream_t s);
hipError_t poem_launch_canon_xyz(const float* tmpl, float* out, int n, float radius, hipStream_t s);
hipError_t poem_launch_pack_split(const float* w, int C, void* img, float* scale_out, hipStream_t s);
hipError_t poem_launch_pack_split_tiles(const float* w, int N, int K, void* img, float* scales, int scale_stride, hipStream_t s);
void poem_gemm_split_context(const void* packed, size_t bytes, const void* split, const float* scales);
void poem_gemm_split_explicit(const void* img, const float* scales);
void poem_cross_attention_split(int on);
void poem_cross_attention_masked_form(int on);
void poem_cross_attention_half(int on);
void poem_cross_attention_tail_halves(int on);
int poem_cross_attention_merges(int NK, int C, int heads);
int poem_cross_attention_fits(int B, int NK, int C);
hipError_t poem_launch_cross_attention_merged_rm(const float* q, const float* k, const float* v, float* ctx, int B, int NQ, int NK,
                                                 int C, int heads, float* scratch, hipStream_t s);
hipError_t poem_launch_cross_attention_merged(const float* q, int ldq, int q_batch_rows, const void* kimg, const void* vimg, float* ctx,
                                              int B, int NQ, int NK, int C, int heads, hipStream_t s);
int poem_gemm_split_applies(const void* Wp, int M, int ldx, int K);
void poem_gemm_split_images(int on);
void poem_gemm_xcd_map(int on);
void poem_gemm_kslab(int on);
void poem_vecattn_one_query_blocks(int on);
void poem_vecattn_valid_neighbours(int k);
hipError_t poem_launch_vector_attention_split(const float* query_xyz, const float* src_xyz, const float* anchor_xyz,
                                              const int* idx, int shared_idx, const float* q, const float* k,
                                              const float* v, int nsrc, const float* wd1, const float* bd1,
                                              const void* wd2, const float* bd2, const void* wg1, const void* wg2,
                                              const float* scales, float* out, int B, int Q, int C, int ldq,
                                              int ldk, int ldv, hipStream_t s);
hipError_t poem_launch_dlt(const float* uv, const float* intr, const float* mat, const int* offs, float* out, int B, int J,
                           int invert, hipStream_t s);
hipError_t poem_launch_dlt_confidence(const float* uv, const float* conf, const float* intr, const float* mat,
                                      const int* offs, float* out, int* sel_count, int B, int J, int invert, int mode,
                                      double threshold, hipStream_t s);
hipError_t poem_launch_pa_epe(const float* pred, const float* gt, float* out, int B, int P, hipStream_t s);
hipError_t poem_launch_pck_accumulate(const float* pred, const float* gt, int B, int P, double vmin, double vmax, int steps,
                                      unsigned int* counts, double* sum, unsigned int* n, float* dist_out, hipStream_t s);
hipError_t poem_launch_mano_to_openpose(const float* jreg, const float* verts, float* joints, int B, int nverts,
                                        hipStream_t s);
hipError_t poem_launch_warp_affine(const unsigned char* src, const long long* src_off, const int* src_hw,
                                   const double* minv, const double* gain, float* out_f32, unsigned char* out_u8, int views,
                                   int OH, int OW, hipStream_t s);
hipError_t poem_launch_heatmap_uv(const float* hmap, float* uv, int maps, int hh, int hw, float img_w, float img_h,
                                  hipStream_t s);
hipError_t poem_launch_heatmap_uv_conf(const float* hmap, float* uv, float* conf, int maps, int hh, int hw, float img_w,
                                       float img_h, hipStream_t s);
size_t poem_conv3x3_packed_floats(int Cout, int Cin);
hipError_t poem_launch_upcat_conv3x3(const float* a_half, int Ca, const float* b_full, int Cb, const void* wp, const float* scale,
                                     const float* shift, float* out, int views, int Cout, int H, int W, int relu, long out_ns,
                                     int out_cs, int out_rs, int out_off, hipStream_t s);
hipError_t poem_launch_pack_conv3x3(const float* w, int Cout, int Cin, void* out, hipStream_t s);
hipError_t poem_launch_conv3x3(const float* in, const void* wp, const float* scale, const float* shift, const float* res,
                               float* out, int views, int Cin, int Cout, int H, int W, int stride, int relu, long out_ns,
                               int out_cs, int out_rs, int out_off, hipStream_t s);
hipError_t poem_launch_conv3x3_ex(const float* in, const void* wp, const float* scale, const float* shift, const float* res,
                                  long res_ns, int res_cs, int res_rs, int res_off, int res_pre, float* out, int views, int Cin,
                                  int Cout, int H, int W, int stride, int relu, long out_ns, int out_cs, int out_rs, int out_off,
                                  hipStream_t s);
size_t poem_conv1x1_packed_floats(int Cout, int Cin);
hipError_t poem_launch_pack_conv1x1(const float* w, int Cout, int Cin, void* out, hipStream_t s);
hipError_t poem_launch_conv1x1_nchw(const float* in, long in_ns, int in_cs, int in_rs, int in_off, const void* wp,
                                    const float* shift, const float* res, long res_ns, int res_cs, int res_rs, int res_off,
                                    float* out, long out_ns, int out_cs, int out_rs, int out_off, int views, int Cin, int Cout,
                                    int H, int W, int relu, hipStream_t s);
hipError_t poem_launch_hrnet_fuse(const float* const* ptrs, const long* ns, const int* cs, const int* rs, const int* off,
// ... 50 lines not shown
```

### poem-v2_amd/csrc/plan.cpp

```cpp
#include "engine.h"

Plan make_plan(const poem_config_t& c, int B, int BN, void* base, int idx_ld) {
  Plan p{};
  p.idx_ld = idx_ld;
  Arena a(base);
  const size_t C = c.embed, S = c.nsample, Q = c.nquery, HW = (size_t)c.feat_h * c.feat_w;
  const size_t BS = (size_t)B * S, BQ = (size_t)B * Q, VS = (size_t)BN * S;
  const size_t SP = (size_t)padded_samples(c), BSP = (size_t)B * SP;
  p.offs = a.take<int32_t>(B + 1);
  p.view_sample = a.take<int32_t>(BN);
  p.pe_index = a.take<int32_t>(BN);
  p.x = a.take<float>((size_t)BN * C * HW);
  p.uv = a.take<float>(VS * 2 + (size_t)BN * 16);
  p.h2 = a.take<float>(VS * C / 2);
  p.bps_feat = a.take<float>(BS * C);
  const size_t front = a.off;
  p.g = a.take<float>(VS * C);
  p.h1 = a.take<float>(VS * C);
  p.mm = a.take<float>(BS * C / 2);
  p.mh = a.take<float>(BS * C / 2);
  p.y = a.take<float>(BS * C);
  const size_t end_ops = a.off;
  a.off = front;
  p.xt = a.take<float>((size_t)BN * C * HW);
  p.ptab = a.take<float>(VS * 8);
  p.q1 = a.take<float>(BS * C);
  a.off = std::max(a.off, end_ops);
  p.centre = a.take<float>((size_t)B * 3);
  p.pt_xyz = a.take<float>(BS * 3);
  for (int i = 0; i <= c.nblocks; ++i) p.xyz[i] = nullptr;
  float* xyz_all = a.take<float>((size_t)(c.nblocks + 1) * BQ * 3);
  for (int i = 0; i <= c.nblocks; ++i) p.xyz[i] = xyz_all ? xyz_all + (size_t)i * BQ * 3 : nullptr;
  p.feats0 = a.take<float>(BQ * C);
  p.qeqp = a.take<float>(BQ * C * 2);
  p.qp = a.take<float>(BQ * C);
  p.ctx = a.take<float>(BQ * C);
  p.att = a.take<float>(BQ * C);
  p.h_attn = a.take<float>(BQ * C);
  p.y3 = a.take<float>(BQ * C * 3);
  p.rs = a.take<float>(BQ * C);
  p.qc = a.take<float>(BQ * C);
  p.rc = a.take<float>(BQ * C);
  p.y4 = a.take<float>(BQ * C * 5);
  p.ffo = a.take<float>(BQ * C);
  for (int i = 0; i < c.nblocks; ++i) {
    p.h_cross[i] = a.take<float>(BQ * C);
    p.f_self[i] = a.take<float>(BQ * C);
    p.f_cross[i] = a.take<float>(BQ * C);
    p.feats[i] = a.take<float>(BQ * C);
    p.idx_self[i] = a.take<int32_t>(BQ * idx_ld);
    p.idx_cross[i] = a.take<int32_t>(BQ * idx_ld);
    p.y1[i] = a.take<float>(BSP * C * 6);
  }
  p.q3t = a.take<float>((size_t)B * C);
  p.par = a.take<float>((size_t)B * 106);
  p.g_pose = a.take<float>((size_t)B * 48);
  p.g_betas = a.take<float>((size_t)B * 10);
  p.mano_verts = a.take<float>((size_t)B * 778 * 3);
  p.mano_joints = a.take<float>((size_t)B * 21 * 3);
  p.attn_scratch = a.take<float>(poem_cross_attention_scratch_floats(B, (int)Q, (int)S, (int)C, c.heads, 0) + 4);
  p.canon_xyz = a.take<float>(Q * 3);
  for (int k = 0; k < 2; ++k) {
    p.anch_x[k] = a.take<float>((size_t)B * 32 * C);
    p.anch_kv[k] = a.take<float>((size_t)B * 32 * C * 2);
  }
  p.qeqp0 = a.take<float>(Q * C * 2);
  p.ident = a.take<int32_t>(32);
  for (int k = 0; k < 2; ++k) {
    p.tab_g[k] = a.take<float>(poem_vector_attention_table_floats((int)Q, (int)C));
    p.tab_p[k] = a.take<float>(poem_vector_attention_table_floats((int)Q, (int)C));
  }
  if (c.petr_embedding) {
    p.petr_f = a.take<float>((size_t)BN * 3 * c.depth_num * HW);
    p.petr_h = a.take<float>((size_t)BN * 2 * C * HW);
    p.petr_tab = a.take<float>((size_t)BN * C * HW);
  }
  p.feat_pad = p.xyz_pad = nullptr;
  if (SP != S) {
    p.feat_pad = a.take<float>(BSP * C);
    p.xyz_pad = a.take<float>(BSP * 3);
  }
  p.bytes = align_up(a.off, 256);
  return p;
}
void register_taps(poem_handle_t h, const Plan& p, int B, int BN, bool sampling) {
  const poem_config_t& c = h->cfg;
  const int64_t C = c.embed, S = c.nsample, Q = c.nquery, HW = c.feat_h * c.feat_w;
  const int64_t BS = B * S, BQ = B * Q;
  h->tapmap.clear();
  if (!h->taps) return;
  auto put = [&](const std::string& k, const void* ptr, int64_t n) { h->tapmap[k] = {ptr, n}; };
  if (sampling) {
    put("x", p.x, (int64_t)BN * C * HW);
    if (!(h->fused_sampling && h->precision == POEM_PRECISION_FP32 && poem_sample_merge_supported((int)C, (int)S, (int)HW)))
      put("g", p.g, (int64_t)BN * C * S);
    put("bps_feat", p.bps_feat, BS * C);
    put("pt_xyz", p.pt_xyz, BS * 3);
  }
  put("query_xyz", p.xyz[0], BQ * 3);
  for (int i = 0; i < c.nblocks; ++i) {
    const std::string pre = "b" + std::to_string(i) + ".";
    put(pre + "h_cross", p.h_cross[i], BQ * C);
    put(pre + "f_self", p.f_self[i], BQ * C);
    put(pre + "f_cross", p.f_cross[i], BQ * C);
    put(pre + "feats", p.feats[i], BQ * C);
    put(pre + "xyz", p.xyz[i + 1], BQ * 3);
    if (i > 0) {
      put(pre + "idx_self", p.idx_self[i], BQ * p.idx_ld);
      put(pre + "idx_cross", p.idx_cross[i], BQ * p.idx_ld);
    }
  }
}

extern "C" {

size_t poem_workspace_bytes(poem_handle_t h, int batch, int total_views) {
  if (!h || batch <= 0 || total_views < batch || h->cfg.nblocks > 8) return 0;
  return make_plan(h->cfg, batch, total_views, nullptr, neighbour_ld(h->cfg, h->knn_query)).bytes;
}
}
```

### poem-v2_amd/csrc/vecattn.hip

```cpp
#include "common.h"
#ifndef POEM_VA_XCD_SAMPLES
#define POEM_VA_XCD_SAMPLES 1
#endif
#include <algorithm>
#include <cstdlib>

#ifdef POEM_VA_DBG
__device__ long long va_dbg[64 * 4 * 8];
#define VA_STAMP(k) do { if (item >= 6000 && item < 6064 && lane == 0) va_dbg[((item - 6000) * 4 + wv) * 8 + (k)] = clock64(); } while (0)
#else
#define VA_STAMP(k) do { } while (0)
#endif

struct VecAttnArgs {
  const float* query_xyz;
  const float* src_xyz;
  const float* anchor_xyz;
  const int* idx;
  int shared_idx;
  const float* q;
  const float* k;
  const float* v;
  int NS;
  const float* wd1;
  const float* bd1;
  const float4* wd2;
  const float* bd2;
  const float4* wg1;
  const float* bg1;
  const float4* wg2;
  const float* bg2;
  float* out;
  int B, Q;
  int ldq, ldk, ldv;
  int stagger;
  int composed;
  float4* tab_g;
  float4* tab_p;
  int kvalid;
  int ldidx;
};

__device__ unsigned int va_cu_slot[8 * 256];

template <int C, int P, int NW, int TPW, bool FLIP, bool INIT0 = true>
__device__ __forceinline__ void chain_gemm(const float4* __restrict__ Wp, const float* __restrict__ X,
                                           f32x16 (&acc)[TPW][P], int wv, int lane) {
  constexpr int KC = C / 8;
  constexpr int XS = 32 * P;
  const int j = lane & 31, h = lane >> 5;
  const __amdgpu_buffer_rsrc_t wrs = frag_rsrc(Wp, (unsigned)(C * C * 4));
  const int wbase = __builtin_amdgcn_readfirstlane(wv) * TPW * KC * 1024;
  const int loff = lane * 16;
  const float* xc = X + (4 * h) * XS + j;
  float4 a0[TPW], a1[TPW];
#define VA_LOADW(A, KCI)                                                                  \
  {                                                                                       \
    const int kq_ = min((KCI), KC - 1);                                                   \
    _Pragma("unroll") for (int tp = 0; tp < TPW; ++tp) A[tp] = frag_load(wrs, loff, wbase + (tp * KC + kq_) * 1024); \
  }
#define VA_READX(XR, KCI, T)                                                              \
  {                                                                                       \
    const int kq_ = min((KCI), KC - 1);                                                   \
    _Pragma("unroll") for (int p = 0; p < P; ++p) XR[p] = xc[(kq_ * 8 + (T)) * XS + 32 * p]; \
  }
#define VA_MMA(A, T, XR, INIT)                                                            \
  _Pragma("unroll") for (int tp = 0; tp < TPW; ++tp) {                                    \
    const float av = (&A[tp].x)[T];                                                       \
    _Pragma("unroll") for (int p = 0; p < P; ++p) {                                       \
      const f32x16 c_ = (INIT) ? zero16() : acc[tp][p];                                   \
      acc[tp][p] = FLIP ? mfma32(XR[p], av, c_) : mfma32(av, XR[p], c_);                  \
    }                                                                                     \
  }
  float x0[P], x1[P], x2[P], x3[P];
#define VA_CHUNK4(A, KCI, INIT)                                                             \
  VA_MMA(A, 0, x0, INIT) __builtin_amdgcn_sched_barrier(0); VA_READX(x0, (KCI) + 1, 0) __builtin_amdgcn_sched_barrier(0);  \
  VA_MMA(A, 1, x1, false) __builtin_amdgcn_sched_barrier(0); VA_READX(x1, (KCI) + 1, 1) __builtin_amdgcn_sched_barrier(0); \
  VA_MMA(A, 2, x2, false) __builtin_amdgcn_sched_barrier(0); VA_READX(x2, (KCI) + 1, 2) __builtin_amdgcn_sched_barrier(0); \
  VA_MMA(A, 3, x3, false) __builtin_amdgcn_sched_barrier(0); VA_READX(x3, (KCI) + 1, 3) __builtin_amdgcn_sched_barrier(0);
  if constexpr (TPW <= 2) {
  static_assert(KC % 4 == 0, "C must be a multiple of 32");
  float4 a2[TPW], a3[TPW];
  VA_LOADW(a0, 0)
  VA_READX(x0, 0, 0) VA_READX(x1, 0, 1) VA_READX(x2, 0, 2) VA_READX(x3, 0, 3)
  VA_LOADW(a1, 1)
  VA_LOADW(a2, 2)
  __builtin_amdgcn_sched_barrier(0);
#define VA_GROUP(KC0, INIT)                                                   \
  VA_LOADW(a3, (KC0) + 3) __builtin_amdgcn_sched_barrier(0); VA_CHUNK4(a0, (KC0), INIT)      \
  VA_LOADW(a0, (KC0) + 4) __builtin_amdgcn_sched_barrier(0); VA_CHUNK4(a1, (KC0) + 1, false) \
  VA_LOADW(a1, (KC0) + 5) __builtin_amdgcn_sched_barrier(0); VA_CHUNK4(a2, (KC0) + 2, false) \
  VA_LOADW(a2, (KC0) + 6) __builtin_amdgcn_sched_barrier(0); VA_CHUNK4(a3, (KC0) + 3, false)
  VA_GROUP(0, INIT0)
  for (int kc = 4; kc < KC; kc += 4) { VA_GROUP(kc, false) }
#undef VA_GROUP
  } else {
  VA_LOADW(a0, 0)
  VA_READX(x0, 0, 0) VA_READX(x1, 0, 1) VA_READX(x2, 0, 2) VA_READX(x3, 0, 3)
  VA_LOADW(a1, 1)
  __builtin_amdgcn_sched_barrier(0);
  VA_CHUNK4(a0, 0, INIT0)
  VA_LOADW(a0, 2)
  __builtin_amdgcn_sched_barrier(0);
  VA_CHUNK4(a1, 1, false)
  for (int kc = 2; kc < KC; kc += 2) {
    VA_LOADW(a1, kc + 1)
    __builtin_amdgcn_sched_barrier(0);
    VA_CHUNK4(a0, kc, false)
    VA_LOADW(a0, kc + 2)
    __builtin_amdgcn_sched_barrier(0);
    VA_CHUNK4(a1, kc + 1, false)
  }
  }
#undef VA_CHUNK4
#undef VA_LOADW
#undef VA_READX
#undef VA_MMA
}

template <int C, int P, int NW, int MINW, bool COMP, int MODE = 0>
__global__ __launch_bounds__(NW * 64, MINW) void vecattn_kernel(VecAttnArgs A) {
  static_assert(MODE == 0 || MODE == 4 || COMP, "table modes exist for the composed form only");
  constexpr bool MASK = MODE == 3;
  constexpr bool WIDE = MODE == 4;
  constexpr int NTILE = C / 32;
  constexpr int TPW = C / 32 / NW;
  constexpr int XS = 32 * P;
  constexpr int NT = NW * 64;
  extern __shared__ __attribute__((aligned(16))) float smem[];
  float* X = smem;
  float* dl = smem + C * XS;
  int* sidx = reinterpret_cast<int*>(dl + P * 32 * 3);
  int* voffs = sidx + P * 32;
  float* qs = reinterpret_cast<float*>(voffs + P * 32);

  const int tid = threadIdx.x, lane = tid & 63, wv = tid >> 6, j = lane & 31, h = lane >> 5;
  const int groups = (A.Q + P - 1) / P;
  const int total = A.B * groups;
  const float inv_sqrt_c = 1.0f / sqrtf((float)C);

  if (A.stagger > 0) {
    if (tid == 0) {
      const unsigned hw = __builtin_amdgcn_s_getreg(4 | (0 << 6) | (31 << 11));
      const unsigned xcc = __builtin_amdgcn_s_getreg(20 | (0 << 6) | (3 << 11));
      const unsigned key = ((xcc & 7u) << 8) | ((hw >> 8) & 0xffu);
      sidx[0] = (int)atomicInc(&va_cu_slot[key], 1u);
    }
    __syncthreads();
    if (sidx[0] & 1) {
      const long long t0 = clock64();
      while (clock64() - t0 < (long long)A.stagger) __builtin_amdgcn_s_sleep(64);
    }
  }

  for (int item = blockIdx.x; item < total; item += gridDim.x) {
  int b = item / groups, ig = item % groups;
  if ((MODE == 0 || MODE == 3 || WIDE) && POEM_VA_XCD_SAMPLES && gridDim.x == (unsigned)total && (total & 7) == 0) {
    const int it = (item & 7) * (total >> 3) + (item >> 3);
    b = it / groups; ig = it % groups;
  }
  if (MODE == 2) {
    if (groups % 8 == 0) {
      const int r = item >> 3;
      ig = (r / A.B) * 8 + (item & 7);
      b = r % A.B;
    } else {
      ig = item / A.B;
      b = item % A.B;
    }
  }
  const int i0 = ig * P;
  float wmx[TPW * P], wsum[TPW * P], wres[TPW * P];
  const int nch = WIDE ? (A.kvalid + 31) >> 5 : 1;
  int ch = 0;
va_chunk:
  __syncthreads();

  VA_STAMP(0);
  if (tid < 32 * P) {
    const int p = tid >> 5, jj = tid & 31;
    const int qi = min(i0 + p, A.Q - 1);
#ifdef POEM_VA_NOLOADS0
    const int id = (qi * 37 + jj * 101) % A.NS;
    dl[tid * 3 + 0] = 0.01f * (float)jj; dl[tid * 3 + 1] = 0.02f * (float)(qi & 7); dl[tid * 3 + 2] = 0.03f;
    (void)0;
#else
    const int id = WIDE ? A.idx[((size_t)b * A.Q + qi) * A.ldidx + min(32 * ch + jj, A.kvalid - 1)]
                        : A.shared_idx ? A.idx[jj] : A.idx[((size_t)b * A.Q + qi) * 32 + jj];
    if (MODE != 2) {
      const float* qx = A.query_xyz + ((size_t)b * A.Q + qi) * 3;
      const float* nx = A.anchor_xyz ? A.anchor_xyz + jj * 3 : A.src_xyz + ((size_t)b * A.NS + id) * 3;
      dl[tid * 3 + 0] = qx[0] - nx[0];
      dl[tid * 3 + 1] = qx[1] - nx[1];
      dl[tid * 3 + 2] = qx[2] - nx[2];
    }
#endif
    sidx[tid] = id;
    voffs[tid] = (int)((unsigned)id * (unsigned)(A.ldv * 4));
  }
  if (MODE != 1)
  for (int f = tid; f < P * C / 4; f += NT) {
    const int p = f / (C / 4), c4 = f % (C / 4);
    const int qi = min(i0 + p, A.Q - 1);
    reinterpret_cast<float4*>(qs)[f] = *reinterpret_cast<const float4*>(A.q + ((size_t)b * A.Q + qi) * A.ldq + 4 * c4);
  }
  __syncthreads();
  if (MODE != 2) {
    float db0[P], db1[P];
#pragma unroll
    for (int p = 0; p < P; ++p) {
      db0[p] = dl[(p * 32 + j) * 3 + h];
      db1[p] = h == 0 ? dl[(p * 32 + j) * 3 + 2] : 0.f;
    }
#pragma unroll
    for (int tp = 0; tp < TPW; ++tp) {
      const int crow = (wv * TPW + tp) * 32 + j;
      const float wa0 = A.wd1[crow * 3 + h];
      const float wa1 = h == 0 ? A.wd1[crow * 3 + 2] : 0.f;
      const int cbase = (wv * TPW + tp) * 32 + 4 * h;
#pragma unroll
      for (int p = 0; p < P; ++p) {
        f32x16 hh = zero16();
        hh = mfma32(wa0, db0[p], hh);
        hh = mfma32(wa1, db1[p], hh);
#pragma unroll
        for (int g = 0; g < 4; ++g) {
          const float4 bb = *reinterpret_cast<const float4*>(A.bd1 + cbase + 8 * g);
#pragma unroll
          for (int e = 0; e < 4; e += 2) {
            const int i = 4 * g + e;
            const f32x2 v = f32x2{hh[i], hh[i + 1]} + f32x2{(&bb.x)[e], (&bb.x)[e + 1]};
            X[((wv * TPW + tp) * 32 + mfma_row(i, h)) * XS + 32 * p + j] = fmaxf(v[0], 0.f);
            X[((wv * TPW + tp) * 32 + mfma_row(i + 1, h)) * XS + 32 * p + j] = fmaxf(v[1], 0.f);
          }
        }
      }
    }
    __syncthreads();
  }

  f32x16 acc[TPW][P], pos[TPW][P];

  if (MODE != 1)
#pragma unroll
  for (int tp = 0; tp < TPW; ++tp) {
    const int cbase = (wv * TPW + tp) * 32 + 4 * h;
#pragma unroll
    for (int p = 0; p < P; ++p) {
      const float* krow = A.k + ((size_t)b * A.NS + sidx[p * 32 + j]) * A.ldk + cbase;
#pragma unroll
      for (int g = 0; g < 4; ++g) {
        const float4 kk = *reinterpret_cast<const float4*>(krow + 8 * g);
#pragma unroll
        for (int e = 0; e < 4; ++e) (COMP ? acc : pos)[tp][p][4 * g + e] = (&kk.x)[e];
      }
    }
  }
  __builtin_amdgcn_sched_barrier(0);

  VA_STAMP(1);
  if (MODE == 2) {
    const float4* tg = A.tab_g + ((size_t)ig * NTILE + wv * TPW) * (P * 4 * 64) + lane;
    const float4* tq = A.tab_p + ((size_t)ig * NTILE + wv * TPW) * (P * 4 * 64) + lane;
    float4 gf[TPW][P][4];
#pragma unroll
    for (int tp = 0; tp < TPW; ++tp)
#pragma unroll
      for (int p = 0; p < P; ++p)
#pragma unroll
        for (int g = 0; g < 4; ++g) gf[tp][p][g] = tg[((tp * P + p) * 4 + g) * 64];
#pragma unroll
    for (int tp = 0; tp < TPW; ++tp)
#pragma unroll
      for (int p = 0; p < P; ++p)
#pragma unroll
        for (int g = 0; g < 4; ++g) {
          const float4 t = tq[((tp * P + p) * 4 + g) * 64];
#pragma unroll
          for (int e = 0; e < 4; ++e) pos[tp][p][4 * g + e] = (&t.x)[e];
        }
#pragma unroll
    for (int tp = 0; tp < TPW; ++tp) {
      const int cbase = (wv * TPW + tp) * 32 + 4 * h;
#pragma unroll
      for (int g = 0; g < 4; ++g)
#pragma unroll
        for (int p = 0; p < P; ++p) {
          const float4 qq = *reinterpret_cast<const float4*>(qs + p * C + cbase + 8 * g);
#pragma unroll
          for (int e = 0; e < 4; e += 2) {
            const int i = 4 * g + e;
            const f32x2 tv = (f32x2{(&qq.x)[e], (&qq.x)[e + 1]} - f32x2{acc[tp][p][i], acc[tp][p][i + 1]}) +
                             f32x2{(&gf[tp][p][g].x)[e], (&gf[tp][p][g].x)[e + 1]};
            X[((wv * TPW + tp) * 32 + mfma_row(i, h)) * XS + 32 * p + j] = fmaxf(tv[0], 0.f);
            X[((wv * TPW + tp) * 32 + mfma_row(i + 1, h)) * XS + 32 * p + j] = fmaxf(tv[1], 0.f);
          }
        }
    }
    __syncthreads();
  } else if (COMP) {
    chain_gemm<C, P, NW, TPW, true>(A.wd2, X, pos, wv, lane);
    VA_STAMP(2);
#pragma unroll
    for (int tp = 0; tp < TPW; ++tp) {
      const float bch = A.bd2[(wv * TPW + tp) * 32 + j];
      const f32x2 bb2 = {bch, bch};
#pragma unroll
      for (int p = 0; p < P; ++p)
#pragma unroll
        for (int i = 0; i < 16; i += 2) {
          const f32x2 pv = f32x2{pos[tp][p][i], pos[tp][p][i + 1]} + bb2;
          pos[tp][p][i] = pv[0]; pos[tp][p][i + 1] = pv[1];
        }
    }
    if (MODE != 1) {
#pragma unroll
      for (int tp = 0; tp < TPW; ++tp) {
        const int cbase = (wv * TPW + tp) * 32 + 4 * h;
#pragma unroll
        for (int g = 0; g < 4; ++g)
#pragma unroll
          for (int p = 0; p < P; ++p) {
            const float4 qq = *reinterpret_cast<const float4*>(qs + p * C + cbase + 8 * g);
#pragma unroll
            for (int e = 0; e < 4; e += 2) {
              const int i = 4 * g + e;
              const f32x2 tv = f32x2{(&qq.x)[e], (&qq.x)[e + 1]} - f32x2{acc[tp][p][i], acc[tp][p][i + 1]};
              acc[tp][p][i] = tv[0]; acc[tp][p][i + 1] = tv[1];
            }
          }
      }
    }
// ... 8 lines not shown
      for (int tp = 0; tp < TPW; ++tp)
#pragma unroll
        for (int p = 0; p < P; ++p)
#pragma unroll
          for (int g = 0; g < 4; ++g) {
            tg[((tp * P + p) * 4 + g) * 64] = float4{acc[tp][p][4 * g], acc[tp][p][4 * g + 1], acc[tp][p][4 * g + 2], acc[tp][p][4 * g + 3]};
            tq[((tp * P + p) * 4 + g) * 64] = float4{pos[tp][p][4 * g], pos[tp][p][4 * g + 1], pos[tp][p][4 * g + 2], pos[tp][p][4 * g + 3]};
          }
      continue;
    }
#pragma unroll
    for (int tp = 0; tp < TPW; ++tp)
#pragma unroll
      for (int p = 0; p < P; ++p)
#pragma unroll
        for (int i = 0; i < 16; ++i)
          X[((wv * TPW + tp) * 32 + mfma_row(i, h)) * XS + 32 * p + j] = fmaxf(acc[tp][p][i], 0.f);
    __syncthreads();
  } else {
  chain_gemm<C, P, NW, TPW, false>(A.wd2, X, acc, wv, lane);
  VA_STAMP(2);
#pragma unroll
  for (int tp = 0; tp < TPW; ++tp) {
    const int cbase = (wv * TPW + tp) * 32 + 4 * h;
#pragma unroll
    for (int g = 0; g < 4; ++g) {
      const float4 bb = *reinterpret_cast<const float4*>(A.bd2 + cbase + 8 * g);
#pragma unroll
      for (int p = 0; p < P; ++p) {
        const float4 qq = *reinterpret_cast<const float4*>(qs + p * C + cbase + 8 * g);
#pragma unroll
        for (int e = 0; e < 4; e += 2) {
          const int i = 4 * g + e;
          const f32x2 pv = f32x2{acc[tp][p][i], acc[tp][p][i + 1]} + f32x2{(&bb.x)[e], (&bb.x)[e + 1]};
          const f32x2 tv = (f32x2{(&qq.x)[e], (&qq.x)[e + 1]} - f32x2{pos[tp][p][i], pos[tp][p][i + 1]}) + pv;
          acc[tp][p][i] = tv[0]; acc[tp][p][i + 1] = tv[1];
          pos[tp][p][i] = pv[0]; pos[tp][p][i + 1] = pv[1];
        }
      }
    }
  }
  __syncthreads();
#pragma unroll
  for (int tp = 0; tp < TPW; ++tp)
#pragma unroll
    for (int p = 0; p < P; ++p)
#pragma unroll
      for (int i = 0; i < 16; ++i) {
        X[((wv * TPW + tp) * 32 + mfma_row(i, h)) * XS + 32 * p + j] = acc[tp][p][i];
      }
  __syncthreads();

  VA_STAMP(3);
  chain_gemm<C, P, NW, TPW, false>(A.wg1, X, acc, wv, lane);
  VA_STAMP(4);
  __syncthreads();
#pragma unroll
  for (int tp = 0; tp < TPW; ++tp) {
    const int cbase = (wv * TPW + tp) * 32 + 4 * h;
#pragma unroll
    for (int g = 0; g < 4; ++g) {
      const float4 bb = *reinterpret_cast<const float4*>(A.bg1 + cbase + 8 * g);
#pragma unroll
      for (int p = 0; p < P; ++p)
#pragma unroll
        for (int e = 0; e < 4; e += 2) {
          const int i = 4 * g + e;
          const f32x2 v = f32x2{acc[tp][p][i], acc[tp][p][i + 1]} + f32x2{(&bb.x)[e], (&bb.x)[e + 1]};
          X[((wv * TPW + tp) * 32 + mfma_row(i, h)) * XS + 32 * p + j] = fmaxf(v[0], 0.f);
          X[((wv * TPW + tp) * 32 + mfma_row(i + 1, h)) * XS + 32 * p + j] = fmaxf(v[1], 0.f);
        }
    }
  }
  __syncthreads();
  }

  VA_STAMP(5);
  chain_gemm<C, P, NW, TPW, true>(A.wg2, X, acc, wv, lane);
  VA_STAMP(6);
  if (!COMP) __syncthreads();

  float* scr = X + wv * (32 * 33);
  const float k2 = inv_sqrt_c * 1.44269504088896340736f;
  const __amdgpu_buffer_rsrc_t vrs = frag_rsrc(A.v + (size_t)b * A.NS * A.ldv, 0xffffffffu);
  float vgb[2][16];
#define VA_GATHER(Q)                                                                                          \
  {                                                                                                           \
    const int tp_ = (Q) / P, p_ = (Q) % P, cch_ = (wv * TPW + tp_) * 32 + j;                                  \
    _Pragma("unroll") for (int i = 0; i < 16; ++i)                                                            \
      vgb[(Q) & 1][i] = __builtin_bit_cast(float, __builtin_amdgcn_raw_buffer_load_b32(vrs, voffs[p_ * 32 + mfma_row(i, h)] + cch_ * 4, 0, 0)); \
  }
  VA_GATHER(0)
#pragma unroll
  for (int q = 0; q < TPW * P; ++q) {
    const int tp = q / P, p = q % P;
    const int cch = (wv * TPW + tp) * 32 + j;
    {
      if (!COMP) {
#pragma unroll
        for (int i = 0; i < 16; ++i) scr[j * 33 + mfma_row(i, h)] = pos[tp][p][i];
      }
      if (q + 1 < TPW * P) VA_GATHER(q + 1)
      __builtin_amdgcn_sched_barrier(0);
      const float (&vg)[16] = vgb[q & 1];
      asm volatile("s_waitcnt lgkmcnt(0)" ::: "memory");
      float pt[16];
#pragma unroll
      for (int i = 0; i < 16; ++i) pt[i] = COMP ? pos[tp][p][i] : scr[mfma_row(i, h) * 33 + j];
      f32x16& a = acc[tp][p];
      if (MASK) {
#pragma unroll
        for (int i = 0; i < 16; ++i)
          if (mfma_row(i, h) >= A.kvalid) a[i] = -INFINITY;
      }
      if (WIDE) {
#pragma unroll
        for (int i = 0; i < 16; ++i)
          if (32 * ch + mfma_row(i, h) >= A.kvalid) a[i] = -INFINITY;
      }
      float mx = fmaxf(fmaxf(a[0], a[1]), a[2]);
#pragma unroll
      for (int i = 3; i < 15; i += 2) mx = fmaxf(fmaxf(mx, a[i]), a[i + 1]);
      mx = half_max(fmaxf(mx, a[15]));
      const float nb = -mx * k2;
      const f32x2 k2v = {k2, k2}, nbv = {nb, nb};
      f32x2 sum2 = {0.f, 0.f}, res2 = {0.f, 0.f};
      asm volatile("s_waitcnt lgkmcnt(0)" ::: "memory");
#pragma unroll
      for (int i = 0; i < 16; i += 2) {
        f32x2 e = __builtin_elementwise_fma(f32x2{a[i], a[i + 1]}, k2v, nbv);
        e[0] = __builtin_amdgcn_exp2f(e[0]);
        e[1] = __builtin_amdgcn_exp2f(e[1]);
        const f32x2 val = f32x2{vg[i], vg[i + 1]} + f32x2{pt[i], pt[i + 1]};
        sum2 += e;
        res2 = __builtin_elementwise_fma(e, val, res2);
      }
      const float sum = half_sum(sum2[0] + sum2[1]);
      const float res = half_sum(res2[0] + res2[1]);
      if (WIDE) {
        if (ch == 0) {
          wmx[q] = mx; wsum[q] = sum; wres[q] = res;
        } else {
          const float m = fmaxf(wmx[q], mx), nm = -m * k2;
          const float so = __builtin_amdgcn_exp2f(__builtin_fmaf(wmx[q], k2, nm)), sn = __builtin_amdgcn_exp2f(__builtin_fmaf(mx, k2, nm));
          wsum[q] = __builtin_fmaf(wsum[q], so, sum * sn);
          wres[q] = __builtin_fmaf(wres[q], so, res * sn);
          wmx[q] = m;
        }
        if (ch == nch - 1 && h == 0 && i0 + p < A.Q) A.out[((size_t)b * A.Q + i0 + p) * C + cch] = wres[q] * __builtin_amdgcn_rcpf(wsum[q]);
      } else if (h == 0 && i0 + p < A.Q) A.out[((size_t)b * A.Q + i0 + p) * C + cch] = res * __builtin_amdgcn_rcpf(sum);
    }
  }
  if constexpr (WIDE)
    if (++ch < nch) goto va_chunk;
#undef VA_GATHER
  VA_STAMP(7);
  }
}

template <int C, int P, int NW, int MINW, bool COMP, int MODE = 0>
static hipError_t launch_va_t(const VecAttnArgs& a, hipStream_t s) {
  const int groups = (a.Q + P - 1) / P;
  size_t lds = (size_t)C * 32 * P * 4 + P * 32 * 3 * 4 + 2 * P * 32 * 4 + (size_t)P * C * 4;
#ifdef POEM_VA_DBG
  if (const char* e = getenv("POEM_VA_LDSPAD")) lds += atoi(e);
#endif
  auto kern = vecattn_kernel<C, P, NW, MINW, COMP, MODE>;
  static std::atomic<unsigned long long> optin{0};
  if (hipError_t e = poem_optin_lds(reinterpret_cast<const void*>(kern), lds, optin); e != hipSuccess) return e;
  unsigned grid = (unsigned)(a.B * groups);
  if (a.stagger > 0) {
    grid = std::min(grid, (unsigned)(2 * poem_device_cus()));
  }
  hipLaunchKernelGGL(kern, dim3(grid), dim3(NW * 64), lds, s, a);
  return hipGetLastError();
}

template <int C, int P, int NW, int MINW>
static hipError_t launch_va(const VecAttnArgs& a, hipStream_t s, int mode = 0) {
  if (mode == 4) return a.composed ? launch_va_t<C, P, NW, MINW, true, 4>(a, s) : launch_va_t<C, P, NW, MINW, false, 4>(a, s);
  if (mode == 1) return launch_va_t<C, P, NW, MINW, true, 1>(a, s);
  if (mode == 2) return launch_va_t<C, P, NW, MINW, true, 2>(a, s);
  if (mode == 3) return a.composed ? launch_va_t<C, P, NW, MINW, true, 3>(a, s) : hipErrorInvalidValue;
  return a.composed ? launch_va_t<C, P, NW, MINW, true>(a, s) : launch_va_t<C, P, NW, MINW, false>(a, s);
}

static thread_local int g_va_kvalid = 32;
extern "C" void poem_vecattn_valid_neighbours(int k) { g_va_kvalid = k; }

static thread_local int g_va_p1 = 0;
extern "C" void poem_vecattn_one_query_blocks(int on) { g_va_p1 = on; }

static int va_group_size(int C) { return C == 128 ? 4 : (C >= 512 ? 1 : 2); }

static hipError_t dispatch_va(const VecAttnArgs& a, int C, hipStream_t s, int mode) {
  if (mode != 1 && (unsigned long long)a.NS * a.ldv * 4 + (unsigned long long)C * 4 > (1ull << 31)) return hipErrorInvalidValue;
  if (mode == 4 && (a.kvalid < 1 || a.kvalid > 64 || a.ldidx < a.kvalid || a.shared_idx || a.anchor_xyz)) return hipErrorInvalidValue;
  if (mode == 0 && a.kvalid != 32) {
    if (a.kvalid < 1 || a.kvalid > 32) return hipErrorInvalidValue;
    mode = 3;
  }
  switch (C) {
    case 32: return launch_va<32, 2, 1, 1>(a, s, mode);
    case 64: return launch_va<64, 2, 2, 1>(a, s, mode);
    case 128: return launch_va<128, 4, 4, 2>(a, s, mode);
    case 256: {
      const int g_va_p1 = ::g_va_p1 >= 0 ? ::g_va_p1 : ((long)a.B * a.Q <= 16L * poem_device_cus() ? 1 : 0);
      if (mode == 0 && g_va_p1 == 1 && a.composed) return launch_va_t<256, 1, 4, 3, true>(a, s);
      if (mode == 0 && g_va_p1 == 2 && a.composed) return launch_va_t<256, 1, 4, 2, true>(a, s);
      return launch_va<256, 2, 4, 2>(a, s, mode);
    }
    case 512: return launch_va<512, 1, 4, 2>(a, s, mode);
    case 1024: return launch_va<1024, 1, 8, 2>(a, s, mode);
    default: return hipErrorInvalidValue;
  }
}

extern "C" size_t poem_vector_attention_table_floats(int Q, int C) {
  const int P = va_group_size(C);
  return (size_t)((Q + P - 1) / P) * P * 32 * C;
}

extern "C" hipError_t poem_launch_vector_attention_tables(const float* query_xyz, const float* anchor_xyz, const int* idx,
                                                          const float* wd1, const float* bd1, const void* wd2,
                                                          const float* bd2, const void* wg1d2, float* tab_g,
                                                          float* tab_p, int Q, int C, hipStream_t s) {
  VecAttnArgs a{query_xyz, nullptr, anchor_xyz, idx, 1, nullptr, nullptr, nullptr, 1, wd1, bd1, (const float4*)wd2, bd2,
                (const float4*)wg1d2, nullptr, nullptr, nullptr, nullptr, 1, Q, 0, 0, 0, 0, 1, (float4*)tab_g, (float4*)tab_p, 32, 32};
  return dispatch_va(a, C, s, 1);
}

extern "C" hipError_t poem_launch_vector_attention_anchored(const int* idx, const float* qg, const float* kg,
                                                            const float* v, int nsrc, const void* wg2,
                                                            const float* tab_g, const float* tab_p, float* out, int B,
                                                            int Q, int C, int ldq, int ldk, int ldv, hipStream_t s) {
  VecAttnArgs a{nullptr, nullptr, nullptr, idx, 1, qg, kg, v, nsrc, nullptr, nullptr, nullptr, nullptr, nullptr, nullptr,
                (const float4*)wg2, nullptr, out, B, Q, ldq, ldk, ldv, 0, 1, (float4*)tab_g, (float4*)tab_p, 32, 32};
  return dispatch_va(a, C, s, 2);
}

extern "C" hipError_t poem_launch_vector_attention(const float* query_xyz, const float* src_xyz, const float* anchor_xyz,
                                                   const int* idx, int shared_idx, const float* q, const float* k,
                                                   const float* v, int nsrc, const float* wd1, const float* bd1,
                                                   const void* wd2, const float* bd2, const void* wg1, const float* bg1,
                                                   const void* wg2, const float* bg2, float* out, int B, int Q, int C,
                                                   int ldq, int ldk, int ldv, int composed, hipStream_t s) {
  VecAttnArgs a{query_xyz, src_xyz, anchor_xyz, idx, shared_idx, q, k, v, nsrc, wd1, bd1, (const float4*)wd2, bd2,
                (const float4*)wg1, bg1, (const float4*)wg2, bg2, out, B, Q, ldq, ldk, ldv, 0, composed, nullptr, nullptr, g_va_kvalid, 32};
#ifdef POEM_LAB
  static const int stagger_env = getenv("POEM_VA_STAGGER") ? atoi(getenv("POEM_VA_STAGGER")) : 0;
  a.stagger = stagger_env;
#endif
#ifdef POEM_VA_DBG
  if (C == 256)
    if (const char* e = getenv("POEM_VA_CFG")) {
      switch (atoi(e)) {
        case 1: return launch_va<256, 1, 4, 4>(a, s);
        case 2: return launch_va<256, 1, 4, 3>(a, s);
        case 3: return launch_va<256, 2, 8, 4>(a, s);
        case 4: return launch_va<256, 1, 8, 4>(a, s);
        case 5: return launch_va<256, 1, 2, 2>(a, s);
        default: break;
      }
    }
#endif
  return dispatch_va(a, C, s, 0);
}

extern "C" hipError_t poem_launch_vector_attention_k(const float* query_xyz, const float* src_xyz, const int* idx, int K, int ld,
                                                     const float* q, const float* k, const float* v, int nsrc, const float* wd1,
                                                     const float* bd1, const void* wd2, const float* bd2, const void* wg1,
                                                     const float* bg1, const void* wg2, const float* bg2, float* out, int B, int Q,
                                                     int C, int ldq, int ldk, int ldv, int composed, hipStream_t s) {
  VecAttnArgs a{query_xyz, src_xyz, nullptr, idx, 0, q, k, v, nsrc, wd1, bd1, (const float4*)wd2, bd2, (const float4*)wg1, bg1,
                (const float4*)wg2, bg2, out, B, Q, ldq, ldk, ldv, 0, composed, nullptr, nullptr, K, ld};
  return dispatch_va(a, C, s, 4);
}
```

Measured before the change: 1476.

## Project only point rows referenced by cross-attention KNN for K/V in later blocks

For decoder blocks after the first, the K/V projection of the basis-point features is no longer computed for every padded sample row. After the cross KNN runs, a mark/compact kernel builds the list of rows actually referenced, and a row-gather panel GEMM on the KNN stream projects only those rows. Vector attention then remaps neighbour indices into the compacted buffer. This trades a full GEMM over all samples for two small index kernels plus a gathered GEMM. It also moves that work after KNN on the side stream, which may lengthen the critical path, and it adds an event and a graph-cache key.

```diff
diff --git a/poem-v2_amd/csrc/decoder.cpp b/poem-v2_amd/csrc/decoder.cpp
--- a/poem-v2_amd/csrc/decoder.cpp
+++ b/poem-v2_amd/csrc/decoder.cpp
@@ -50,6 +50,7 @@
   bool side_rest_pending = false;
   bool bps_waited[9] = {}, knn_waited[9] = {};
   bool anchor_from_y3 = false;
+  bool vc_rows[9] = {};
 
   DecoderRun(poem_handle_t h_, Plan& p_, const float* feats_in, const float* pt_xyz_, const float* pt_feats_, int B_, float* pose,
              float* bet, hipStream_t s_, bool template_queries)
@@ -105,8 +106,9 @@
     const bool anchored = tables && i == 0;
     if (!anchored && h->f1_split && C % 128 == 0) {
       HIPCHK(poem_launch_gemm_segs(pt_feats, C, f.w[0], f.b[0], BSP, C, POEM_ACT_NONE, C, 4, outs, modes, sb));
-      HIPCHK(poem_launch_gemm_segs(pt_feats, C, (const float*)f.w[0] + (size_t)4 * C * C, f.b[0] + 4 * C, BSP, C, POEM_ACT_NONE, C, 2, outs + 4,
-                                   modes + 4, sb));
+      if (!vc_rows[i])
+        HIPCHK(poem_launch_gemm_segs(pt_feats, C, (const float*)f.w[0] + (size_t)4 * C * C, f.b[0] + 4 * C, BSP, C, POEM_ACT_NONE, C, 2, outs + 4,
+                                     modes + 4, sb));
     } else {
       HIPCHK(poem_launch_gemm_segs(pt_feats, C, f.w[0], f.b[0], BSP, C, POEM_ACT_NONE, C, anchored ? 4 : 6, outs, modes, sb));
     }
@@ -151,6 +153,18 @@
     }
     if (ov) HIPCHK(hipEventRecord(h->ev_knn[i], sk));
     knn_issued[i] = true;
+    return vc_rows[i] ? rows_in_use_projection(i) : POEM_OK;
+  }
+
+  int rows_in_use_projection(int i) {
+    const auto& f = h->fused[i];
+    const size_t seg = (size_t)BSP * C;
+    float* outs[2] = {p.y1[i] + 4 * seg, p.y1[i] + 5 * seg};
+    HIPCHK(poem_launch_rows_in_use(p.idx_cross[i], B, Q, p.idx_ld == 32 ? 32 : c.knn, p.idx_ld, S, SP, p.riu_remap[i], p.riu_rows[i],
+                                   p.riu_xrow[i], p.riu_nused[i], p.riu_rowbase[i], p.riu_total[i], sk));
+    HIPCHK(poem_launch_gemm_segs_rows(pt_feats, C, (const float*)f.w[0] + (size_t)4 * C * C, f.b[0] + 4 * C, BSP, C, C, 2, outs,
+                                      p.riu_xrow[i], p.riu_total[i], sk));
+    if (ov) HIPCHK(hipEventRecord(h->ev_vc[i], sk));
     return POEM_OK;
   }
 
@@ -333,6 +347,9 @@
         HIPCHK(hipStreamWaitEvent(s, h->ev_bps[k], 0));
         bps_waited[k] = true;
       }
+    if (ov && vc_rows[i]) HIPCHK(hipStreamWaitEvent(s, h->ev_vc[i], 0));
+    if (vc_rows[i]) poem_vecattn_rows_in_use(p.riu_remap[i], p.riu_rowbase[i]);
+    struct Clear { ~Clear() { poem_vecattn_rows_in_use(nullptr, nullptr); } } clear_rows_in_use;
     const bool prof = prof_begin();
     const int kc = shared ? 32 : c.knn;
     if (h->precision != POEM_PRECISION_FP32) {
@@ -430,6 +447,9 @@
       pt_feats = p.feat_pad;
       pt_xyz_rows = p.xyz_pad;
     }
+    for (int i = 1; i < c.nblocks; ++i)
+      vc_rows[i] = h->vc_rows_in_use && h->precision == POEM_PRECISION_FP32 && h->f1_split && C % 128 == 0 && SP <= 15360 &&
+                   poem_gemm_segs_rows_applies(pt_feats, C, (const float*)h->fused[i].w[0] + (size_t)4 * C * C, BSP, C, C, 2) != 0;
     int rc = fork();
     if (rc != POEM_OK) return rc;
     wmask = (ov && chain) ? (h->wait_merge >= 0 ? h->wait_merge : 3) : 0;
diff --git a/poem-v2_amd/csrc/engine.h b/poem-v2_amd/csrc/engine.h
--- a/poem-v2_amd/csrc/engine.h
+++ b/poem-v2_amd/csrc/engine.h
@@ -121,6 +121,8 @@
   float *c_canon_xyz = nullptr, *c_tab_g[2] = {}, *c_tab_p[2] = {};
   float* c_qeqp0 = nullptr;
   hipEvent_t ev_bps[8] = {}, ev_xyz[8] = {}, ev_knn[8] = {}, ev_def[8] = {};
+  hipEvent_t ev_vc[8] = {};
+  bool vc_rows_in_use = true;
   int bps_defer = 0;
   bool f1_split = true;
   int va_p1 = -1;
@@ -150,6 +152,7 @@
 
 struct Plan {
   int32_t *offs, *view_sample, *pe_index, *idx_self[8], *idx_cross[8];
+  int32_t *riu_remap[8], *riu_rows[8], *riu_xrow[8], *riu_nused[8], *riu_rowbase[8], *riu_total[8];
   float *x, *uv, *g, *h1, *h2, *mm, *mh, *y, *bps_feat, *centre, *pt_xyz, *xyz[9];
   float *xt, *ptab, *q1;
   float *petr_f, *petr_h, *petr_tab;
diff --git a/poem-v2_amd/csrc/forward.cpp b/poem-v2_amd/csrc/forward.cpp
--- a/poem-v2_amd/csrc/forward.cpp
+++ b/poem-v2_amd/csrc/forward.cpp
@@ -182,7 +182,7 @@
     if (!h->graphs || h->graph_broken || h->prof_on || h->tables_pending || !h->cap_stream) return 0;
     const std::vector<int64_t> key = {B, plan_views, fused_fe ? -1 : BN, (int64_t)(uintptr_t)workspace, h->precision, h->anchor_tables, h->chains,
                                       h->fused_sampling, h->tables_first, h->chain_combine, h->knn_early, h->overlap, h->chain_tile,
-                                      h->tables_cached, h->knn_fma, h->knn_query, h->taps, c.parametric, h->xattn_merge, h->small_batch, h->bps_defer, poem_process_switches(), h->f1_split, h->va_p1, h->group_min_views, h->group_xcd, h->d2_first, h->wait_merge,
+                                      h->tables_cached, h->knn_fma, h->knn_query, h->taps, c.parametric, h->xattn_merge, h->small_batch, h->bps_defer, poem_process_switches(), h->f1_split, h->vc_rows_in_use, h->va_p1, h->group_min_views, h->group_xcd, h->d2_first, h->wait_merge,
                                       (int64_t)(uintptr_t)h->mano_table, h->mano_center};
     poem_handle_s::GraphEntry* hit = nullptr;
     for (auto& g : h->graph_cache)
diff --git a/poem-v2_amd/csrc/gemm.hip b/poem-v2_amd/csrc/gemm.hip
--- a/poem-v2_amd/csrc/gemm.hip
+++ b/poem-v2_amd/csrc/gemm.hip
@@ -266,6 +266,8 @@
   int seg_cols;
   int split_images;
   int xcd_map;
+  const int* rows;
+  const int* mrows;
 };
 
 template <int MT, int NT, int SKC, int OMODE>
@@ -468,12 +470,13 @@
 }
 
 
-template <int NT, int MT, bool GELU, int OMODE, bool SPLIT = false>
+template <int NT, int MT, bool GELU, int OMODE, bool SPLIT = false, bool ROWS = false>
 __device__ __forceinline__ void panel_rows(const float* __restrict__ X, int ldx, const float4* __restrict__ wl,
                                            const float* __restrict__ bias, const float* __restrict__ R, int ldr,
                                            float* __restrict__ Y, int ldy, int M, int K, int pact, int col0, int ycol0,
                                            int bip, int blocks_in_panel, const float* __restrict__ tile_scales = nullptr,
-                                           int scale_stride = 0, int split_images = 0, int part = 0, int nparts = 1) {
+                                           int scale_stride = 0, int split_images = 0, int part = 0, int nparts = 1,
+                                           const int* __restrict__ rowlist = nullptr, int xrows = 0) {
   constexpr int NWV = (SPLIT && !GELU) ? POEM_GS_WAVES : 8;
   const int KC = K >> 3;
   const int tid = threadIdx.x, lane = tid & 63, wv = tid >> 6, r = lane & 31, h = lane >> 5;
@@ -491,6 +494,11 @@
 #ifdef POEM_PANEL_SKEW
   if (wv >= NWV / 2) { const long long t0_ = wall_clock64(); while (wall_clock64() - t0_ < POEM_PANEL_SKEW) __builtin_amdgcn_s_sleep(32); }
 #endif
+  int xrow[MT];
+  if constexpr (ROWS) {
+#pragma unroll
+    for (int i = 0; i < MT; ++i) xrow[i] = M > 0 ? rowlist[min(((rg_lo + bip * NWV + wv) * MT + i) * 32 + r, M - 1)] : 0;
+  }
   for (int rg = rg_lo + bip * NWV + wv; rg < rg_hi; rg += blocks_in_panel * NWV) {
 #if POEM_PANEL_LAB & 4
     __builtin_amdgcn_s_setprio(0);
@@ -498,7 +506,11 @@
     const int mt0 = rg * MT;
     unsigned xo[MT];
 #pragma unroll
-    for (int i = 0; i < MT; ++i) xo[i] = (unsigned)min((mt0 + i) * 32 + r, M - 1) * (unsigned)(ldx * 4) + 16u * h;
+    for (int i = 0; i < MT; ++i) xo[i] = (unsigned)(ROWS ? min(max(xrow[i], 0), xrows - 1) : min((mt0 + i) * 32 + r, M - 1)) * (unsigned)(ldx * 4) + 16u * h;
+    if constexpr (ROWS) {
+#pragma unroll
+      for (int i = 0; i < MT; ++i) xrow[i] = rowlist[min(((rg + blocks_in_panel * NWV) * MT + i) * 32 + r, M - 1)];
+    }
     f32x16 acc[MT][NT];
 #pragma unroll
     for (int i = 0; i < MT; ++i)
@@ -706,7 +718,7 @@
   }
 }
 
-template <int NT, int MT, bool GELU, bool SPLIT = false>
+template <int NT, int MT, bool GELU, bool SPLIT = false, bool ROWS = false>
 __global__ __launch_bounds__((SPLIT && !GELU) ? POEM_GS_WAVES * 64 : 512, 2) void gemm_panel_kernel(const float* __restrict__ X, int ldx,
                                                             const float4* __restrict__ Wp, const float* __restrict__ bias,
                                                             const float* __restrict__ R, int ldr, float* __restrict__ Y,
@@ -718,7 +730,12 @@
   extern __shared__ __attribute__((aligned(16))) float4 wl[];
   const int tid = threadIdx.x;
   const int panels = N / (32 * NT);
-  const int xm = segs.xcd_map;
+  int xm = segs.xcd_map;
+  const int xrows = M;
+  if constexpr (ROWS) {
+    M = min(max(*segs.mrows, 0), M);
+    xm = xm && (M + 31) / 32 >= 8 * (((int)gridDim.x >> 3) / panels) * 8 * MT;
+  }
   const int lb = xm ? (int)(blockIdx.x >> 3) : (int)blockIdx.x;
   const int panel = lb % panels, bip = lb / panels;
   const int blocks_in_panel = xm ? (int)(gridDim.x >> 3) / panels : ((int)gridDim.x - panel + panels - 1) / panels;
@@ -735,6 +752,12 @@
   if (segs.seg_cols == 0) {
     panel_rows<NT, MT, GELU, 0, SPLIT>(X, ldx, wl, bias, R, ldr, Y, ldy, M, K, pact, col0, col0, bip, blocks_in_panel,
                                        tile_scales, scale_stride, 0, part, nparts);
+    return;
+  }
+  if constexpr (ROWS) {
+    const int sidx = col0 / segs.seg_cols;
+    panel_rows<NT, MT, false, 0, false, true>(X, ldx, wl, bias, nullptr, 0, segs.ptr[sidx], segs.seg_cols, M, K, pact, col0,
+                                              col0 - sidx * segs.seg_cols, bip, blocks_in_panel, nullptr, 0, 0, part, nparts, segs.rows, xrows);
     return;
   }
   const int sidx = col0 / segs.seg_cols;
@@ -760,20 +783,20 @@
 static std::atomic<int> g_panel_xcd_map{1};
 extern "C" void poem_gemm_xcd_map(int on) { g_panel_xcd_map = on; }
 
-template <int NT, int MT, bool GELU, bool SPLIT = false>
+template <int NT, int MT, bool GELU, bool SPLIT = false, bool ROWS = false>
 static hipError_t launch_panel_t(const float* X, int ldx, const void* Wp, const float* bias, const float* R, int ldr,
                                  float* Y, int ldy, int M, int N, int K, int act, int act_split, int act2,
                                  const PanelSegs& segs, hipStream_t s, const float* tile_scales = nullptr,
                                  int scale_stride = 0) {
   const size_t lds = (size_t)NT * (K / 8) * 64 * 16 + (size_t)NT * 32 * sizeof(float);
-  auto kern = gemm_panel_kernel<NT, MT, GELU, SPLIT>;
+  auto kern = gemm_panel_kernel<NT, MT, GELU, SPLIT, ROWS>;
   static std::atomic<unsigned long long> optin{0};
   if (hipError_t e = poem_optin_lds(reinterpret_cast<const void*>(kern), 128 * 1024 + 512, optin); e != hipSuccess) return e;
   const int panels = N / (32 * NT);
   const int grid = std::max(poem_num_cus(), panels);
   PanelSegs sg = segs;
   const int mtiles = (M + 31) / 32;
-  sg.xcd_map = g_panel_xcd_map && grid % 8 == 0 && (grid / 8) % panels == 0 && mtiles >= 8 * ((grid / 8) / panels) * 8 * MT;
+  sg.xcd_map = g_panel_xcd_map && grid % 8 == 0 && (grid / 8) % panels == 0 && (ROWS || mtiles >= 8 * ((grid / 8) / panels) * 8 * MT);
   hipLaunchKernelGGL(kern, dim3(grid), dim3((SPLIT && !GELU) ? POEM_GS_WAVES * 64 : 512), lds, s, X, ldx, (const float4*)Wp, bias, R,
                      ldr, Y, ldy, M, N, K, act, act_split, act2, sg, tile_scales, scale_stride);
   return hipGetLastError();
@@ -868,6 +891,48 @@
   return launch_gemm_split_impl(X, ldx, Wp, bias, nullptr, 0, nullptr, 0, M, N, K, act, N, act, segs, s);
 }
 
+static int rows_panel_nt(const float* X, int ldx, const void* Wp, int M, int K, int seg_cols, int nsegs) {
+  const bool in_split_mode = g_explicit_split.img || (g_split_ctx.packed && (const char*)Wp >= g_split_ctx.packed &&
+                                                      (const char*)Wp < g_split_ctx.packed + g_split_ctx.bytes);
+  if (in_split_mode || nsegs < 1 || nsegs > 6 || seg_cols % 32 || M < 1 || K % 8 || ((uintptr_t)X & 15) || ldx % 4 ||
+      (unsigned long long)M * ldx * 4ull >= (1ull << 32))
+    return 0;
+  const int N = seg_cols * nsegs;
+  const long wave_slots = 8L * poem_num_cus(), row_tiles = (M + 31) / 32;
+  int NT = 0;
+  for (int c : {4, 2, 1})
+    if (N % (32 * c) == 0 && (size_t)c * K * 128 <= 128 * 1024 && seg_cols % (32 * c) == 0) {
+      NT = c;
+      if (row_tiles * (N / (32 * c)) >= wave_slots || !g_panel_narrow || K > 256) break;
+    }
+  return (NT == 1 && K >= 512) ? 0 : NT;
+}
+extern "C" int poem_gemm_segs_rows_applies(const float* X, int ldx, const void* Wp, int M, int K, int seg_cols, int nsegs) {
+  return rows_panel_nt(X, ldx, Wp, M, K, seg_cols, nsegs) != 0;
+}
+extern "C" hipError_t poem_launch_gemm_segs_rows(const float* X, int ldx, const void* Wp, const float* bias, int M, int K,
+                                                 int seg_cols, int nsegs, float* const* outs, const int* rows, const int* mrows,
+                                                 hipStream_t s) {
+  const int NT = rows_panel_nt(X, ldx, Wp, M, K, seg_cols, nsegs);
+  if (NT == 0 || !rows || !mrows) return hipErrorInvalidValue;
+  PanelSegs segs{};
+  segs.seg_cols = seg_cols;
+  segs.rows = rows;
+  segs.mrows = mrows;
+  for (int i = 0; i < nsegs; ++i) { segs.ptr[i] = outs[i]; segs.mode[i] = 0; }
+  const int N = seg_cols * nsegs, mtiles = (M + 31) / 32, panels = N / (32 * NT);
+  const int wpp = std::max(1, std::max(poem_num_cus(), panels) / panels) * 8;
+  auto cost = [&](int mt) { return (long)(((mtiles + mt - 1) / mt + wpp - 1) / wpp) * mt; };
+  const bool mt2 = 5 * cost(2) <= 6 * cost(1);
+#define POEM_PANEL_R(NTV)                                                                                                        \
+  return mt2 ? launch_panel_t<NTV, 2, false, false, true>(X, ldx, Wp, bias, nullptr, 0, nullptr, 0, M, N, K, 0, N, 0, segs, s)   \
+             : launch_panel_t<NTV, 1, false, false, true>(X, ldx, Wp, bias, nullptr, 0, nullptr, 0, M, N, K, 0, N, 0, segs, s)
+  if (NT == 4) { POEM_PANEL_R(4); }
+  if (NT == 2) { POEM_PANEL_R(2); }
+  POEM_PANEL_R(1);
+#undef POEM_PANEL_R
+}
+
 extern "C" hipError_t poem_launch_gemm(const float* X, int ldx, const void* Wp, const float* bias, const float* R,
                                        int ldr, float* Y, int ldy, int M, int N, int K, int act, hipStream_t s) {
   return poem_launch_gemm_split(X, ldx, Wp, bias, R, ldr, Y, ldy, M, N, K, act, N, act, s);
diff --git a/poem-v2_amd/csrc/handle.cpp b/poem-v2_amd/csrc/handle.cpp
--- a/poem-v2_amd/csrc/handle.cpp
+++ b/poem-v2_amd/csrc/handle.cpp
@@ -10,7 +10,7 @@
 namespace {
 struct CaptureKit {
   hipStream_t cap = nullptr, bps = nullptr, knn = nullptr;
-  hipEvent_t ev[5 + 32] = {};
+  hipEvent_t ev[5 + 40] = {};
 };
 std::mutex g_pool_mutex;
 std::map<int, std::vector<CaptureKit>> g_kit_pool;
@@ -44,7 +44,7 @@
 hipEvent_t** kit_event_slots(poem_handle_t h, hipEvent_t** out) {
   int n = 0;
   out[n++] = &h->ev_fork; out[n++] = &h->ev_join_bps; out[n++] = &h->ev_join_knn; out[n++] = &h->ev_tab; out[n++] = &h->ev_fork0;
-  for (int i = 0; i < 8; ++i) { out[n++] = &h->ev_bps[i]; out[n++] = &h->ev_xyz[i]; out[n++] = &h->ev_knn[i]; out[n++] = &h->ev_def[i]; }
+  for (int i = 0; i < 8; ++i) { out[n++] = &h->ev_bps[i]; out[n++] = &h->ev_xyz[i]; out[n++] = &h->ev_knn[i]; out[n++] = &h->ev_def[i]; out[n++] = &h->ev_vc[i]; }
   return out;
 }
 
@@ -52,7 +52,7 @@
   int dev = 0;
   if (hipGetDevice(&dev) != hipSuccess) return false;
   h->stream_device = dev;
-  hipEvent_t* slots[5 + 32];
+  hipEvent_t* slots[5 + 40];
   kit_event_slots(h, slots);
   {
     std::lock_guard<std::mutex> lock(g_pool_mutex);
@@ -61,36 +61,36 @@
       const CaptureKit k = pool.back();
       pool.pop_back();
       h->cap_stream = k.cap; h->bps_stream = k.bps; h->knn_stream = k.knn;
-      for (int i = 0; i < 5 + 32; ++i) *slots[i] = k.ev[i];
+      for (int i = 0; i < 5 + 40; ++i) *slots[i] = k.ev[i];
       return true;
     }
   }
   bool ok = hipStreamCreateWithFlags(&h->bps_stream, hipStreamNonBlocking) == hipSuccess &&
             hipStreamCreateWithFlags(&h->knn_stream, hipStreamNonBlocking) == hipSuccess &&
             hipStreamCreateWithFlags(&h->cap_stream, hipStreamNonBlocking) == hipSuccess;
-  for (int i = 0; i < 5 + 32; ++i) ok = ok && hipEventCreateWithFlags(slots[i], hipEventDisableTiming) == hipSuccess;
+  for (int i = 0; i < 5 + 40; ++i) ok = ok && hipEventCreateWithFlags(slots[i], hipEventDisableTiming) == hipSuccess;
   return ok;
 }
 
 void return_kit(poem_handle_t h) {
-  hipEvent_t* slots[5 + 32];
+  hipEvent_t* slots[5 + 40];
   kit_event_slots(h, slots);
   bool whole = h->cap_stream && h->bps_stream && h->knn_stream;
-  for (int i = 0; i < 5 + 32; ++i) whole = whole && *slots[i] != nullptr;
+  for (int i = 0; i < 5 + 40; ++i) whole = whole && *slots[i] != nullptr;
   if (!whole) {
     if (h->cap_stream) (void)hipStreamDestroy(h->cap_stream);
     if (h->bps_stream) (void)hipStreamDestroy(h->bps_stream);
     if (h->knn_stream) (void)hipStreamDestroy(h->knn_stream);
-    for (int i = 0; i < 5 + 32; ++i) if (*slots[i]) (void)hipEventDestroy(*slots[i]);
+    for (int i = 0; i < 5 + 40; ++i) if (*slots[i]) (void)hipEventDestroy(*slots[i]);
   } else {
     CaptureKit k;
     k.cap = h->cap_stream; k.bps = h->bps_stream; k.knn = h->knn_stream;
-    for (int i = 0; i < 5 + 32; ++i) k.ev[i] = *slots[i];
+    for (int i = 0; i < 5 + 40; ++i) k.ev[i] = *slots[i];
     std::lock_guard<std::mutex> lock(g_pool_mutex);
     g_kit_pool[h->stream_device].push_back(k);
   }
   h->cap_stream = h->bps_stream = h->knn_stream = nullptr;
-  for (int i = 0; i < 5 + 32; ++i) *slots[i] = nullptr;
+  for (int i = 0; i < 5 + 40; ++i) *slots[i] = nullptr;
 }
 
 void park_execs(poem_handle_t h) {
@@ -502,6 +502,7 @@
   else if (k == "graph_eager") h->graph_eager = value != 0;
   else if (k == "gemm_xcd_map") { poem_gemm_xcd_map(value != 0); g_proc_switches.fetch_and(~1); g_proc_switches.fetch_or(value ? 1 : 0); }
   else if (k == "f1_split") h->f1_split = value != 0;
+  else if (k == "vc_rows_in_use") h->vc_rows_in_use = value != 0;
   else if (k == "xattn_half") { poem_cross_attention_half(value != 0); g_proc_switches.fetch_and(~4); g_proc_switches.fetch_or(value ? 4 : 0); }
   else if (k == "xattn_tail") { poem_cross_attention_tail_halves(value != 0); g_proc_switches.fetch_and(~8); g_proc_switches.fetch_or(value ? 8 : 0); }
   else if (k == "wait_merge") { if (value < -1 || value > 7) return POEM_E_ARG; h->wait_merge = value; }
diff --git a/poem-v2_amd/csrc/knn.hip b/poem-v2_amd/csrc/knn.hip
--- a/poem-v2_amd/csrc/knn.hip
+++ b/poem-v2_amd/csrc/knn.hip
@@ -210,3 +210,75 @@
   return K == 32 && ld == 32 ? knn_launch<false>(qxyz, sxyz, idx, B, NQ, NS, 32, 32, fma, s)
                              : knn_launch<true>(qxyz, sxyz, idx, B, NQ, NS, K, ld, fma, s);
 }
+
+__global__ __launch_bounds__(1024) void rows_in_use_mark_kernel(const int* __restrict__ idx, int NQ, int K, int ld, int NS, int SP,
+                                                                int* __restrict__ remap, int* __restrict__ rows,
+                                                                int* __restrict__ nused) {
+  extern __shared__ int riu_flag[];
+  int* wsum = riu_flag + SP;
+  const int b = blockIdx.x, tid = threadIdx.x, lane = tid & 63, wv = tid >> 6;
+  for (int i = tid; i < SP; i += 1024) riu_flag[i] = 0;
+  __syncthreads();
+  const int* src = idx + (size_t)b * NQ * ld;
+  for (int t = tid; t < NQ * K; t += 1024) {
+    const int id = src[(size_t)(t / K) * ld + t % K];
+    if ((unsigned)id < (unsigned)NS) riu_flag[id] = 1;
+  }
+  __syncthreads();
+  const int per = (SP + 1023) / 1024, lo = min(tid * per, SP), hi = min(lo + per, SP);
+  int cnt = 0;
+  for (int i = lo; i < hi; ++i) cnt += riu_flag[i];
+  int incl = cnt;
+#pragma unroll
+  for (int o = 1; o < 64; o <<= 1) {
+    const int t = __shfl_up(incl, o, 64);
+    if (lane >= o) incl += t;
+  }
+  if (lane == 63) wsum[wv] = incl;
+  __syncthreads();
+  int base = 0, all = 0;
+  for (int w = 0; w < 16; ++w) {
+    if (w < wv) base += wsum[w];
+    all += wsum[w];
+  }
+  int rank = base + incl - cnt;
+  for (int i = lo; i < hi; ++i) {
+    const bool used = riu_flag[i] != 0;
+    remap[(size_t)b * SP + i] = used ? rank : -1;
+    if (used) rows[(size_t)b * SP + rank++] = i;
+  }
+  if (tid == 0) nused[b] = all;
+}
+
+__global__ __launch_bounds__(256) void rows_in_use_flatten_kernel(const int* __restrict__ rows, const int* __restrict__ nused, int B,
+                                                                  int SP, int* __restrict__ xrow, int* __restrict__ rowbase,
+                                                                  int* __restrict__ total) {
+  __shared__ int part[256];
+  const int b = blockIdx.x, tid = threadIdx.x;
+  int s = 0;
+  for (int i = tid; i < b; i += 256) s += nused[i];
+  part[tid] = s;
+  __syncthreads();
+  for (int o = 128; o > 0; o >>= 1) {
+    if (tid < o) part[tid] += part[tid + o];
+    __syncthreads();
+  }
+  const int base = part[0], n = min(nused[b], SP);
+  for (int r = tid; r < n; r += 256) xrow[base + r] = b * SP + rows[(size_t)b * SP + r];
+  if (tid == 0) {
+    rowbase[b] = base;
+    if (b == B - 1) total[0] = base + n;
+  }
+}
+
+extern "C" hipError_t poem_launch_rows_in_use(const int* idx, int B, int NQ, int K, int ld, int NS, int SP, int* remap, int* rows,
+                                              int* xrow, int* nused, int* rowbase, int* total, hipStream_t s) {
+  if (B < 1 || NQ < 1 || K < 1 || ld < K || NS < 1 || SP < NS || SP > 15360 || (long)NQ * K >= (1l << 31) ||
+      (long)B * SP >= (1l << 31))
+    return hipErrorInvalidValue;
+  hipLaunchKernelGGL(rows_in_use_mark_kernel, dim3((unsigned)B), dim3(1024), (size_t)(SP + 16) * sizeof(int), s, idx, NQ, K, ld, NS, SP,
+                     remap, rows, nused);
+  if (hipError_t e = hipGetLastError(); e != hipSuccess) return e;
+  hipLaunchKernelGGL(rows_in_use_flatten_kernel, dim3((unsigned)B), dim3(256), 0, s, rows, nused, B, SP, xrow, rowbase, total);
+  return hipGetLastError();
+}
diff --git a/poem-v2_amd/csrc/launchers.h b/poem-v2_amd/csrc/launchers.h
--- a/poem-v2_amd/csrc/launchers.h
+++ b/poem-v2_amd/csrc/launchers.h
@@ -68,6 +68,12 @@
 hipError_t poem_launch_knn(const float* qxyz, const float* sxyz, int* idx, int B, int NQ, int NS, int fma, hipStream_t s);
 hipError_t poem_launch_knn_k(const float* qxyz, const float* sxyz, int* idx, int B, int NQ, int NS, int K, int ld, int fma,
                              hipStream_t s);
+hipError_t poem_launch_rows_in_use(const int* idx, int B, int NQ, int K, int ld, int NS, int SP, int* remap, int* rows, int* xrow,
+                                   int* nused, int* rowbase, int* total, hipStream_t s);
+int poem_gemm_segs_rows_applies(const float* X, int ldx, const void* Wp, int M, int K, int seg_cols, int nsegs);
+hipError_t poem_launch_gemm_segs_rows(const float* X, int ldx, const void* Wp, const float* bias, int M, int K, int seg_cols,
+                                      int nsegs, float* const* outs, const int* rows, const int* mrows, hipStream_t s);
+void poem_vecattn_rows_in_use(const int* remap, const int* rowbase);
 hipError_t poem_launch_vector_attention(const float* query_xyz, const float* src_xyz, const float* anchor_xyz,
                                         const int* idx, int shared_idx, const float* q, const float* k, const float* v,
                                         int nsrc, const float* wd1, const float* bd1, const void* wd2, const float* bd2,
diff --git a/poem-v2_amd/csrc/plan.cpp b/poem-v2_amd/csrc/plan.cpp
--- a/poem-v2_amd/csrc/plan.cpp
+++ b/poem-v2_amd/csrc/plan.cpp
@@ -51,6 +51,15 @@
     p.idx_self[i] = a.take<int32_t>(BQ * idx_ld);
     p.idx_cross[i] = a.take<int32_t>(BQ * idx_ld);
     p.y1[i] = a.take<float>(BSP * C * 6);
+    p.riu_remap[i] = p.riu_rows[i] = p.riu_xrow[i] = p.riu_nused[i] = p.riu_rowbase[i] = p.riu_total[i] = nullptr;
+    if (i > 0) {
+      p.riu_remap[i] = a.take<int32_t>(BSP);
+      p.riu_rows[i] = a.take<int32_t>(BSP);
+      p.riu_xrow[i] = a.take<int32_t>(BSP);
+      p.riu_nused[i] = a.take<int32_t>(B);
+      p.riu_rowbase[i] = a.take<int32_t>(B);
+      p.riu_total[i] = a.take<int32_t>(1);
+    }
   }
   p.q3t = a.take<float>((size_t)B * C);
   p.par = a.take<float>((size_t)B * 106);
@@ -108,6 +117,7 @@
     if (i > 0) {
       put(pre + "idx_self", p.idx_self[i], BQ * p.idx_ld);
       put(pre + "idx_cross", p.idx_cross[i], BQ * p.idx_ld);
+      put(pre + "rows_in_use", p.riu_nused[i], B);
     }
   }
 }
diff --git a/poem-v2_amd/csrc/vecattn.hip b/poem-v2_amd/csrc/vecattn.hip
--- a/poem-v2_amd/csrc/vecattn.hip
+++ b/poem-v2_amd/csrc/vecattn.hip
@@ -39,6 +39,8 @@
   float4* tab_p;
   int kvalid;
   int ldidx;
+  const int* remap;
+  const int* rowbase;
 };
 
 __device__ unsigned int va_cu_slot[8 * 256];
@@ -195,8 +197,10 @@
       dl[tid * 3 + 2] = qx[2] - nx[2];
     }
 #endif
-    sidx[tid] = id;
-    voffs[tid] = (int)((unsigned)id * (unsigned)(A.ldv * 4));
+    int rid = id;
+    if ((MODE == 0 || MODE == 3 || WIDE) && A.remap) rid = max(A.remap[(size_t)b * A.NS + id], 0);
+    sidx[tid] = rid;
+    voffs[tid] = (int)((unsigned)rid * (unsigned)(A.ldv * 4));
   }
   if (MODE != 1)
   for (int f = tid; f < P * C / 4; f += NT) {
@@ -240,6 +244,7 @@
   }
 
   f32x16 acc[TPW][P], pos[TPW][P];
+  const size_t kvrow0 = ((MODE == 0 || MODE == 3 || WIDE) && A.remap) ? (size_t)A.rowbase[b] : (size_t)b * A.NS;
 
   if (MODE != 1)
 #pragma unroll
@@ -247,7 +252,7 @@
     const int cbase = (wv * TPW + tp) * 32 + 4 * h;
 #pragma unroll
     for (int p = 0; p < P; ++p) {
-      const float* krow = A.k + ((size_t)b * A.NS + sidx[p * 32 + j]) * A.ldk + cbase;
+      const float* krow = A.k + (kvrow0 + sidx[p * 32 + j]) * A.ldk + cbase;
 #pragma unroll
       for (int g = 0; g < 4; ++g) {
         const float4 kk = *reinterpret_cast<const float4*>(krow + 8 * g);
@@ -422,7 +427,7 @@
 
   float* scr = X + wv * (32 * 33);
   const float k2 = inv_sqrt_c * 1.44269504088896340736f;
-  const __amdgpu_buffer_rsrc_t vrs = frag_rsrc(A.v + (size_t)b * A.NS * A.ldv, 0xffffffffu);
+  const __amdgpu_buffer_rsrc_t vrs = frag_rsrc(A.v + kvrow0 * A.ldv, 0xffffffffu);
   float vgb[2][16];
 #define VA_GATHER(Q)                                                                                          \
   {                                                                                                           \
@@ -529,6 +534,9 @@
 extern "C" void poem_vecattn_valid_neighbours(int k) { g_va_kvalid = k; }
 
 static thread_local int g_va_p1 = 0;
+static thread_local const int* g_va_remap = nullptr;
+static thread_local const int* g_va_rowbase = nullptr;
+extern "C" void poem_vecattn_rows_in_use(const int* remap, const int* rowbase) { g_va_remap = remap; g_va_rowbase = rowbase; }
 extern "C" void poem_vecattn_one_query_blocks(int on) { g_va_p1 = on; }
 
 static int va_group_size(int C) { return C == 128 ? 4 : (C >= 512 ? 1 : 2); }
@@ -586,7 +594,8 @@
                                                    const void* wg2, const float* bg2, float* out, int B, int Q, int C,
                                                    int ldq, int ldk, int ldv, int composed, hipStream_t s) {
   VecAttnArgs a{query_xyz, src_xyz, anchor_xyz, idx, shared_idx, q, k, v, nsrc, wd1, bd1, (const float4*)wd2, bd2,
-                (const float4*)wg1, bg1, (const float4*)wg2, bg2, out, B, Q, ldq, ldk, ldv, 0, composed, nullptr, nullptr, g_va_kvalid, 32};
+                (const float4*)wg1, bg1, (const float4*)wg2, bg2, out, B, Q, ldq, ldk, ldv, 0, composed, nullptr, nullptr, g_va_kvalid, 32,
+                shared_idx ? nullptr : g_va_remap, shared_idx ? nullptr : g_va_rowbase};
 #ifdef POEM_LAB
   static const int stagger_env = getenv("POEM_VA_STAGGER") ? atoi(getenv("POEM_VA_STAGGER")) : 0;
   a.stagger = stagger_env;
@@ -613,6 +622,6 @@
                                                      const float* bg1, const void* wg2, const float* bg2, float* out, int B, int Q,
                                                      int C, int ldq, int ldk, int ldv, int composed, hipStream_t s) {
   VecAttnArgs a{query_xyz, src_xyz, nullptr, idx, 0, q, k, v, nsrc, wd1, bd1, (const float4*)wd2, bd2, (const float4*)wg1, bg1,
-                (const float4*)wg2, bg2, out, B, Q, ldq, ldk, ldv, 0, composed, nullptr, nullptr, K, ld};
+                (const float4*)wg2, bg2, out, B, Q, ldq, ldk, ldv, 0, composed, nullptr, nullptr, K, ld, g_va_remap, g_va_rowbase};
   return dispatch_va(a, C, s, 4);
 }
```

Result: no change. 1484 (median of 6 runs) (+0.6%).
